# computational-cell-analytics/micro-sam

Measured on AMD Instinct MI355X. Metric: 1024^2 tiles/s embed+AMG (vit_b bf16), higher is better.
Workload: dtype bf16 image encoder (patch embedding + neck, 1.2 % of its flops, on hi+lo operand pairs of that type), fp16 mask decoder (16-bit MFMA operands, fp32 accumulation); 1 GPU; configs[1]: vit_b, 1024x1024 uint8 synthetic tiles, batched embedding precompute + AutomaticMaskGenerator (32x32 grid, multimask, default thresholds); encoder_batch=16, distinct_tiles_per_gpu=256, weights=seeded synthetic checkpoint (synthetic.py variant 'cells'), decode_lanes=3

## Files before the change

include/msam_hip.h:

```cpp
#ifndef MSAM_HIP_H
#define MSAM_HIP_H

#include <stdint.h>

#ifdef __cplusplus
extern "C" {
#endif

#define MSAM_MAX_BLOCKS 32
#define MSAM_F32 1
#define MSAM_BF16 2
#define MSAM_FP8 3
#define MSAM_F16 4
#define MSAM_U8 5
#define MSAM_U16 6
#define MSAM_ACT_NONE 0
#define MSAM_ACT_GELU 1
#define MSAM_ACT_RELU 2
#define MSAM_ACT_SIGMOID 3

const char* msam_last_error(void);
int msam_abi_version(void);


// ... 123 lines not shown
                  int32_t W, float thresh, int32_t intersection_over_min, uint64_t* mask_scratch, int32_t* keep_flags,
                  void* stream);

int64_t msam_amg_generate_workspace_bytes(int32_t N, int32_t H, int32_t W);
int msam_amg_generate_labels(const float* iou, const float* stability, const int32_t* boxes, const int32_t* area,
                             const uint32_t* bits, int32_t N, int32_t H, int32_t W, const int32_t* crop_box,
                             float pred_iou_thresh, float stability_score_thresh, float box_nms_thresh,
                             int32_t min_object_size, int32_t with_background, int32_t* labels, int32_t* flag,
                             void* workspace, int64_t workspace_bytes, void* stream);

int64_t msam_labels_from_masks_workspace_bytes(int32_t H, int32_t W);
int msam_labels_from_masks(const uint32_t* bits, const int32_t* order, int32_t K, const int32_t* k_dev, int32_t H, int32_t W,
                           int32_t min_object_size, int32_t with_background, int32_t* labels, int32_t* flag,
                           void* workspace, int64_t workspace_bytes, void* stream);

int msam_layernorm_backward(const float* x, const float* weight, const float* dy, float eps, int64_t rows, int32_t dim,
                            float* dx, float* dweight, float* dbias, void* stream);
int msam_attention_forward(const float* q, const float* k, const float* v, int32_t BH, int32_t Nq, int32_t Nk, int32_t D,
                           float scale, float* out, float* lse, void* stream);
int msam_attention_backward(const float* q, const float* k, const float* v, const float* out, const float* dout,
                            const float* lse, int32_t BH, int32_t Nq, int32_t Nk, int32_t D, float scale, float* dq, float* dk,
                            float* dv, float* delta, void* stream);

int msam_relpos_attention_forward(const float* q, const float* k, const float* v, const float* bias_h, const float* bias_w,
                                  int32_t BH, int32_t Gh, int32_t Gw, int32_t D, float scale, float* out, float* lse,
                                  void* stream);
int msam_relpos_attention_backward(const float* q, const float* k, const float* v, const float* bias_h, const float* bias_w,
                                   const float* out, const float* dout, const float* lse, int32_t BH, int32_t Gh, int32_t Gw,
                                   int32_t D, float scale, float* dq, float* dk, float* dv, float* dbias_h, float* dbias_w,
                                   float* delta, void* stream);

int msam_cast_transpose(const void* x, int32_t x_dtype, int64_t M, int32_t K, int64_t ldx, void* out16, void* outT, float* colsum,
                        void* stream);

int msam_layernorm(const float* x, const float* weight, const float* bias, float eps, int64_t rows, int32_t dim,
                   void* out, int32_t out_dtype, int32_t gelu, int32_t out_nchw_hw, void* stream);

int msam_layernorm_fp8(const float* x, const float* weight, const float* bias, float eps, int64_t rows, int32_t dim,
                       void* out_fp8, float* row_scale, void* stream);
int msam_quant_rows_fp8(const void* x_bf16, int64_t rows, int32_t dim, void* out_fp8, float* row_scale, void* stream);
int msam_patchify(const float* img, int32_t B, void* out_bf16, void* stream);
int msam_patchify16(const float* img, int32_t B, int32_t dtype16, void* out16, void* stream);
int msam_patchify_u8(const uint8_t* img, int32_t B, int32_t h, int32_t w, void* out_bf16, void* stream);
int msam_patchify_u8_16(const uint8_t* img, int32_t B, int32_t h, int32_t w, int32_t dtype16, void* out16, void* stream);
int msam_im2col3x3(const void* x_bf16, int32_t B, int32_t C, void* out_bf16, void* stream);
int msam_cast_f32_to_bf16(const float* x, void* out_bf16, int64_t n, void* stream);
int msam_cast_f32_to_16(const float* x, int32_t dtype16, void* out16, int64_t n, void* stream);
int msam_resample_u8(const uint8_t* in, int32_t B, int32_t H, int32_t W, int32_t C, int32_t axis, int32_t n_out,
                     const int32_t* bounds, const int32_t* coefs, int32_t ksize, uint8_t* out, void* stream);
int msam_patchify_split16(const float* img, int32_t B, int32_t dtype16, void* out16, void* stream);
int msam_patchify_u8_split16(const uint8_t* img, int32_t B, int32_t h, int32_t w, int32_t dtype16, void* out16, void* stream);
int msam_im2col3x3_split16(const float* x_f32, int32_t B, int32_t C, int32_t dtype16, void* out16, void* stream);
int msam_cast_f32_split16(const float* x, int32_t dtype16, void* out16, int64_t rows, int32_t dim, void* stream);

int msam_window_attention(const void* q, const void* k, const void* v, const void* rel_h, const void* rel_w,
                          const float* qkv_bias, int32_t B, int32_t heads, int32_t head_dim, float scale, void* out,
                          void* stream);
int msam_window_attention16(const void* q, const void* k, const void* v, const void* rel_h, const void* rel_w,
                            const float* qkv_bias, int32_t B, int32_t heads, int32_t head_dim, float scale, int32_t dtype16,
                            void* out, void* stream);
int msam_global_attention(const void* q, const void* k, const void* v, const void* rel_h, const void* rel_w,
                          int32_t B, int32_t heads, int32_t head_dim, float scale, void* out, void* stream);
int msam_global_attention16(const void* q, const void* k, const void* v, const void* rel_h, const void* rel_w, int32_t B,
                            int32_t heads, int32_t head_dim, float scale, int32_t dtype16, void* out, void* stream);

typedef struct {
    int32_t embed_dim, depth, heads;
    int32_t is_global[MSAM_MAX_BLOCKS];
    const void* patch_w; const float* patch_b;
    const float* pos_embed;
    const float* ln1_w[MSAM_MAX_BLOCKS]; const float* ln1_b[MSAM_MAX_BLOCKS];
    const void* qkv_w[MSAM_MAX_BLOCKS]; const float* qkv_b[MSAM_MAX_BLOCKS];
    const void* rel_h[MSAM_MAX_BLOCKS]; const void* rel_w[MSAM_MAX_BLOCKS];
    const void* proj_w[MSAM_MAX_BLOCKS]; const float* proj_b[MSAM_MAX_BLOCKS];
    const float* ln2_w[MSAM_MAX_BLOCKS]; const float* ln2_b[MSAM_MAX_BLOCKS];
    const void* lin1_w[MSAM_MAX_BLOCKS]; const float* lin1_b[MSAM_MAX_BLOCKS];
    const void* lin2_w[MSAM_MAX_BLOCKS]; const float* lin2_b[MSAM_MAX_BLOCKS];
    const void* neck0_w;
    const float* neck1_w; const float* neck1_b;
    const void* neck2_w;
    const float* neck3_w; const float* neck3_b;
    int32_t use_glds;
    int32_t head_dim_stored;
    int32_t fp8;
    const void* qkv_w8[MSAM_MAX_BLOCKS]; const float* qkv_cs[MSAM_MAX_BLOCKS];
    const void* proj_w8[MSAM_MAX_BLOCKS]; const float* proj_cs[MSAM_MAX_BLOCKS];
    const void* lin1_w8[MSAM_MAX_BLOCKS]; const float* lin1_cs[MSAM_MAX_BLOCKS];
    const void* lin2_w8[MSAM_MAX_BLOCKS]; const float* lin2_cs[MSAM_MAX_BLOCKS];
    int32_t dtype16;
    int32_t split_io;
    const void* adapter_wd[MSAM_MAX_BLOCKS]; const float* adapter_bd[MSAM_MAX_BLOCKS];
    const void* adapter_wu[MSAM_MAX_BLOCKS]; const float* adapter_bu[MSAM_MAX_BLOCKS];
    const float* adapter_alpha[MSAM_MAX_BLOCKS];
    int32_t adapter_dim;
} msam_encoder_t;

int64_t msam_encoder_workspace_bytes(const msam_encoder_t* enc, int32_t B);
int msam_encoder_forward(const msam_encoder_t* enc, const float* img_f32, const uint8_t* img_u8, int32_t h, int32_t w,
                         int32_t B, float* out, void* workspace, int64_t workspace_bytes,
                         float* tap, int32_t tap_block, void* stream);

int msam_adapter_bf16(const void* y16, int64_t ldy, const void* wd16, const float* bd, const void* wu16, const float* bu,
                      const float* alpha, float* x, int64_t ldx, int32_t R, int32_t D, int32_t P, int32_t dtype16, void* stream);

typedef struct {
    const void* q_w; const float* q_b; const void* k_w; const float* k_b;
    const void* v_w; const float* v_b; const void* o_w; const float* o_b;
} msam_attn_w_t;
typedef struct {
    msam_attn_w_t self_attn, t2i, i2t;
    const float *n1_w, *n1_b, *n2_w, *n2_b, *n3_w, *n3_b, *n4_w, *n4_b;
    const void* mlp1_w; const float* mlp1_b; const void* mlp2_w; const float* mlp2_b;
    const void* mlp1_ws; const void* mlp2_ws;
} msam_twoway_layer_t;
typedef struct {
    const float* pe_gauss;
    const float* point_embed;
    const float* not_a_point;
    const float* no_mask;
    const float* out_tokens;
    msam_twoway_layer_t layer[2];
    msam_attn_w_t final_attn; const float *nf_w, *nf_b;
    const void* up1_w; const float* up1_b;
    const float* up_ln_w; const float* up_ln_b;
    const void* up2_w; const float* up2_b;
    const void* hyp_w[4][3]; const float* hyp_b[4][3];
    const void* iou_w[3]; const float* iou_b[3];
    int32_t use_glds;
    int32_t low_res_dtype;
    int32_t up1_centred;
    float* low_res_range;
} msam_decoder_t;

int msam_decoder_dtype(void);
int64_t msam_decoder_const_bytes(void);
int msam_decoder_prepare_const(const msam_decoder_t* dec, void* consts, void* stream);
int64_t msam_decoder_image_bytes(void);
int msam_decoder_prepare_image(const msam_decoder_t* dec, const void* consts, const float* embedding ,
                               void* image_state, void* workspace, int64_t workspace_bytes, void* stream);
int64_t msam_decoder_workspace_bytes(int32_t P);
int msam_decoder_forward(const msam_decoder_t* dec, const void* consts, const void* image_state,
                         const float* points, const int32_t* labels, int32_t Np, const float* boxes, int32_t P,
                         int32_t multimask, float* low_res, float* iou,
                         void* workspace, int64_t workspace_bytes, void* stream);

typedef struct {
    const float *c1_w, *c1_b, *ln1_w, *ln1_b, *c2_w, *c2_b, *ln2_w, *ln2_b, *c3_w, *c3_b;
    int32_t exact_gelu;
} msam_mask_prompt_t;
int msam_decoder_forward_masks(const msam_decoder_t* dec, const msam_mask_prompt_t* mask_w, const void* consts,
                               const void* image_state, const float* points, const int32_t* labels, int32_t Np,
                               const float* boxes, const float* mask_input, int32_t P, int32_t multimask, float* low_res,
                               float* iou, void* workspace, int64_t workspace_bytes, void* stream);

int msam_prompt_encode(const msam_decoder_t* dec, const msam_mask_prompt_t* mask_w, const float* points,
                       const int32_t* labels, int32_t Np, const float* boxes, const float* mask_input, int32_t P,
                       float* sparse, float* dense, void* stream);
int msam_decoder_forward_embeddings(const msam_decoder_t* dec, const void* consts, const void* image_state,
                                    const float* sparse, int32_t Ns, const float* dense, const float* embedding,
                                    int32_t P, int32_t multimask, float* low_res, float* iou, void* workspace,
                                    int64_t workspace_bytes, void* stream);

int msam_postprocess_masks(const float* low_res, int32_t N, int32_t in_h, int32_t in_w, int32_t out_h, int32_t out_w,
                           float thr, float off, int32_t* counts, int32_t* boxes, uint32_t* bits, float* logits,
                           void* stream);
int msam_postprocess_masks16(const void* low_res, int32_t low_res_dtype, int32_t N, int32_t in_h, int32_t in_w, int32_t out_h,
                             int32_t out_w, float thr, float off, int32_t* counts, int32_t* boxes, uint32_t* bits, float* logits,
                             void* stream);
int msam_postprocess_masks_range(const float* low_res, const float* range, int32_t N, int32_t in_h, int32_t in_w, int32_t out_h,
                                 int32_t out_w, float thr, float off, int32_t* counts, int32_t* boxes, uint32_t* bits,
                                 void* stream);
int msam_uncrop_bits(const uint32_t* bits_crop, int32_t N, int32_t crop_h, int32_t crop_w, int32_t x0, int32_t y0,
                     int32_t out_h, int32_t out_w, uint32_t* bits_out, void* stream);

int msam_rle_run_counts(const uint32_t* bits, int32_t N, int32_t out_h, int32_t out_w, int32_t* n_runs, void* stream);
int msam_rle_encode(const uint32_t* bits, int32_t N, int32_t out_h, int32_t out_w, const int64_t* offsets,
                    int32_t* counts_out, void* stream);

int msam_box_nms(const float* boxes_sorted, int32_t K, float iou_threshold, uint64_t* mask_scratch, int32_t* keep_flags,
                 void* stream);

int msam_box_nms_valid(const float* boxes_sorted, const int32_t* valid_sorted, int32_t K, float iou_threshold,
                       uint64_t* mask_scratch, int32_t* keep_flags, void* stream);

int msam_paint_label_image(const uint32_t* bits, const int32_t* order, int32_t K, int32_t H, int32_t W, int32_t* label,
                           void* stream);
int msam_paint_label_image_dev(const uint32_t* bits, const int32_t* order, const int32_t* k_dev, int32_t H, int32_t W,
                               int32_t* label, void* stream);
int msam_label_components(const int32_t* seg, int32_t H, int32_t W, int32_t* roots, int32_t* changed_flag,
                          int32_t max_iters, int32_t* iters_done, void* stream);

int msam_component_sizes(const int32_t* roots, int32_t n, int32_t* sizes, int32_t* bg_count, void* stream);
int msam_label_components_async(const int32_t* seg, int32_t H, int32_t W, int32_t* roots, int32_t* changed_flag,
                                int32_t passes, void* stream);

#define MSAM_MATCH_MAX_THRESHOLDS 16
#define MSAM_MATCH_MAX_BATCH 65535
#define MSAM_MATCH_HEADER 4
#define MSAM_MATCH_ITEM 20
#define MSAM_MATCH_EDGE 6
int64_t msam_label_matching_workspace_bytes(int32_t B, int32_t capacity);
int msam_label_matching(const int32_t* pred, const int32_t* gt, int32_t B, int32_t G, int32_t H, int32_t W,
                        const double* thresholds, int32_t T, void* workspace, int64_t workspace_bytes, int32_t capacity,
                        int32_t* result, int32_t max_edges, void* stream);

int msam_slice_overlaps(const int32_t* labels, int32_t Z, int32_t H, int32_t W, uint64_t* table_keys, int32_t* table_counts,
                        int32_t capacity, int32_t* edges, int32_t max_edges, int32_t* n_edges, void* stream);

int msam_host_seeded_watershed(const float* image, const int32_t* markers, const uint8_t* mask, int32_t H, int32_t W, int32_t* out);

typedef struct {
    const float* A; int64_t lda;
    const float* A2; int64_t lda2; int64_t a2_rows;
    const float* W; int64_t ldw;
    int64_t M; int32_t N, K;
    const float* bias; int32_t act;
    const float* res; int64_t ldr; int64_t res_rows;
    float* out; int64_t ldc;
    const float* col_scale; const float* col_shift;
    int32_t conv_h, conv_w, conv_c;
    int32_t shuffle_h, shuffle_w, shuffle_c;
    int32_t a2_cols;
    int32_t split16;
    float a_scale, w_scale;
    const void* w_pairs;
} msam_sgemm_t;
int msam_strict_gemm(const msam_sgemm_t* p, void* stream);
int msam_strict_layernorm(const float* x, const float* weight, const float* bias, float eps, int64_t rows, int32_t dim, float* out,
                          int32_t gelu, int32_t out_nchw_hw, void* stream);
int msam_strict_relpos_attention(const float* qkv, const float* qkv_bias, const float* rel_h, const float* rel_w, int32_t B, int32_t heads,
                                 int32_t head_dim, int32_t grid, int32_t window, float scale, float* out, void* stream);
int msam_split16_relpos_attention(const float* qkv, const float* qkv_bias, const float* rel_h, const float* rel_w, int32_t B, int32_t heads,
                                  int32_t head_dim, int32_t grid, int32_t window, float scale, float* out, void* stream);
typedef struct msam_si2t {
    const float* keys; int64_t key_batch_stride;
    const float* pos;
    const float* wq; const float* bq;
    const float* tok_k; const float* tok_v; int64_t ld_tok, tok_batch_stride;
    const float* wo; const float* bo;
    const float* ln_weight; const float* ln_bias; float ln_eps; float denom;
    float* out;
    int32_t B, Tk;
    int32_t split16;
    float wq_scale, wo_scale;
    const void* wq_pairs; const void* wo_pairs;
} msam_si2t_t;
int msam_strict_i2t_block(const msam_si2t_t* p, void* stream);
int msam_strict_attention(const float* q, int64_t ldq, int64_t q_batch_stride, const float* k, int64_t ldk, int64_t k_batch_stride,
                          const float* v, int64_t ldv, int64_t v_batch_stride, int32_t B, int32_t H, int32_t Nq, int32_t Nk, int32_t D,
                          float denom, float* out, int64_t ldo, int64_t out_batch_stride, void* stream);
int msam_strict_patchify(const float* img, const uint8_t* img_u8, int32_t B, int32_t h, int32_t w, float* out, void* stream);
int msam_strict_im2col3x3(const float* x, int32_t B, int32_t C, float* out, void* stream);
int msam_strict_source(const float* embedding, const float* dense, int64_t dense_stride, int32_t P, float* src, void* stream);
int msam_strict_hyper_masks(const float* up, const float* hyper, int32_t hyper_ld, int32_t mask0, int32_t nmask, int64_t P, float* low_res,
                            void* stream);
int msam_split16_i2t_block(const msam_si2t_t* p, void* workspace, int64_t workspace_bytes, void* stream);
int msam_split16_prepare_pairs(const float* w, int64_t N, int32_t K, float scale, int32_t permute, void* out, void* stream);
typedef struct {
    const float* keys; int64_t key_batch_stride;
    const float* pos;
    const float* q; int64_t ldq;
    const float* wk; const float* wv; const float* bv;
    float denom;
    float* out; int64_t ldo;
    int32_t B, Tk;
    void* workspace; int64_t workspace_bytes;
} msam_st2i_t;
int msam_split16_t2i_attention(const msam_st2i_t* p, void* stream);
typedef struct {
    const float* u1;
    const float* ln_weight; const float* ln_bias; float ln_eps;
    const float* w2; const float* b2; float w_scale;
    const float* hyper; int32_t hyper_ld, mask0, nmask;
    float* low_res;
    int64_t P;
} msam_sup2_t;
int msam_strict_upscale2(const msam_sup2_t* p, void* stream);
int msam_strict_instance_norm(const float* x, int64_t ldx, int32_t B, int64_t HW, int32_t C, float eps, float* out, float* workspace,
                              int64_t workspace_floats, void* stream);
int msam_strict_resize_bilinear(const float* in, int32_t B, int32_t h, int32_t w, int32_t pitch_h, int32_t pitch_w, int64_t pixel_pitch, int32_t C,
                                int32_t H2, int32_t W2, float scale_h, float scale_w, int32_t out_nchw, float* out, void* stream);

#define MSAM_OBJFEAT_DESC 12
int msam_objfeat_gather(const int64_t* labels, const int64_t* desc, int32_t U, int32_t max_pixels, const int32_t* itab,
                        const int64_t* ids, int32_t n_ids, int64_t* keys, int32_t* area, void* stream);
int msam_objfeat_accumulate(const float* emb, const int64_t* desc, int32_t U, const int32_t* itab, const float* ftab,
                            const int64_t* sorted_keys, const int64_t* perm, const int32_t* chunk_start, const int64_t* pix_start,
                            const int32_t* area, int32_t n_ids, int32_t K, int32_t max_chunks, double* partial, void* stream);
int msam_objfeat_finish(const double* partial, const int32_t* chunk_start, const int32_t* area, int32_t n_ids, double* sums,
                        int64_t* area_total, int32_t out_f64, void* out, void* stream);
int msam_objfeat_project(const int64_t* labels, int64_t n, const int64_t* ids, int32_t n_ids, int32_t* index, void* stream);

#define MSAM_EDT_MAX_SIDE 32767
int64_t msam_edt_squared_workspace_bytes(int32_t H, int32_t W);
int msam_edt_squared(const void* mask, int32_t mask_is_int32, int32_t H, int32_t W, int32_t* out, void* workspace,
                     int64_t workspace_bytes, void* stream);
int64_t msam_label_props_workspace_bytes(int32_t H, int32_t W, int32_t N);
int msam_label_props(const int32_t* labels, int32_t H, int32_t W, const int32_t* ids, int32_t N, int32_t* area, int32_t* bbox,
                     int64_t* coord_sum, int32_t* center, void* workspace, int64_t workspace_bytes, void* stream);
int64_t msam_distance_targets_workspace_bytes(int32_t H, int32_t W, int32_t N);
int msam_distance_targets(const int32_t* labels, int32_t H, int32_t W, int32_t N, int32_t correct_centers, float fill, float* out,
                          int32_t* center, int32_t* dmax2, int32_t* bbox, void* workspace, int64_t workspace_bytes, void* stream);

#define MSAM_MASK_MAX_SIDE 32767
#define MSAM_MASK_MAX_OBJECTS 65535
int msam_mask_pack(const uint8_t* masks, int32_t P, int32_t H, int32_t W, uint32_t* bits, void* stream);
// ... 63 lines not shown
```

micro_sam_amd/_lib.py:

```python
from __future__ import annotations

import ctypes as C
import os
from typing import Optional

import torch

from . import build as _build

MSAM_MAX_BLOCKS = 32
F32, BF16, FP8, F16, U8, U16 = 1, 2, 3, 4, 5, 6
ACT_NONE, ACT_GELU, ACT_RELU, ACT_SIGMOID = 0, 1, 2, 3

_vp, _i32, _i64, _f32 = C.c_void_p, C.c_int32, C.c_int64, C.c_float
PROFILE_FAMILIES = 8


class GemmParams(C.Structure):
    _fields_ = [
        ("A", _vp), ("lda", _i64), ("W", _vp), ("ldw", _i64), ("M", _i32), ("N", _i32), ("K", _i32),
        ("bias", _vp), ("table", _vp), ("table_rows", _i32), ("table_cols", _i32), ("table_ld", _i64),
        ("resid", _vp), ("resid_dtype", _i32), ("resid_rows", _i32), ("ldr", _i64), ("act", _i32),
        ("out", _vp), ("out_dtype", _i32), ("ldc", _i64), ("out_mode", _i32),
        ("q", _vp), ("k", _vp), ("v", _vp), ("heads", _i32), ("head_dim", _i32), ("tokens", _i32),
        ("use_glds", _i32), ("ln_mode", _i32), ("ln_w", _vp), ("ln_b", _vp), ("ln_eps", _f32),
        ("a_dtype", _i32), ("row_scale", _vp), ("col_scale", _vp), ("split_k", _i32),
        ("ln_add", _vp), ("ln_out_a", _vp), ("ln_out_b", _vp),
    ]


class WsGemmParams(C.Structure):
    _fields_ = [
        ("A", _vp), ("W", _vp), ("M", _i32), ("N", _i32), ("K", _i32), ("bias", _vp),
        ("table", _vp), ("table_rows", _i32), ("table_cols", _i32), ("table_ld", _i64),
        ("resid", _vp), ("resid_rows", _i32), ("ldr", _i64),
        ("ln_mode", _i32), ("ln_w", _vp), ("ln_b", _vp), ("ln_eps", _f32),
        ("out", _vp), ("ldc", _i64), ("kv_split", _i32), ("k_out", _vp), ("vT_out", _vp), ("tokens", _i32),
        ("head_major", _i32),
    ]


class ImageLayerParams(C.Structure):
    _fields_ = [
        ("xin", _vp), ("q_shared", _vp), ("wq", _vp), ("bq", _vp), ("peq", _vp),
        ("wo", _vp), ("bo", _vp), ("ln_w", _vp), ("ln_b", _vp), ("ln_eps", _f32),
        ("ktok", _vp), ("vtok", _vp), ("Nt", _i32), ("out", _vp), ("rows", _i32),
    ]


_blk = _vp * MSAM_MAX_BLOCKS


class EncoderParams(C.Structure):
    _fields_ = [
        ("embed_dim", _i32), ("depth", _i32), ("heads", _i32), ("is_global", _i32 * MSAM_MAX_BLOCKS),
        ("patch_w", _vp), ("patch_b", _vp), ("pos_embed", _vp),
        ("ln1_w", _blk), ("ln1_b", _blk), ("qkv_w", _blk), ("qkv_b", _blk), ("rel_h", _blk), ("rel_w", _blk),
        ("proj_w", _blk), ("proj_b", _blk), ("ln2_w", _blk), ("ln2_b", _blk),
        ("lin1_w", _blk), ("lin1_b", _blk), ("lin2_w", _blk), ("lin2_b", _blk),
        ("neck0_w", _vp), ("neck1_w", _vp), ("neck1_b", _vp), ("neck2_w", _vp), ("neck3_w", _vp), ("neck3_b", _vp),
        ("use_glds", _i32), ("head_dim_stored", _i32), ("fp8", _i32),
        ("qkv_w8", _blk), ("qkv_cs", _blk), ("proj_w8", _blk), ("proj_cs", _blk),
        ("lin1_w8", _blk), ("lin1_cs", _blk), ("lin2_w8", _blk), ("lin2_cs", _blk),
        ("dtype16", _i32), ("split_io", _i32),
        ("adapter_wd", _blk), ("adapter_bd", _blk), ("adapter_wu", _blk), ("adapter_bu", _blk), ("adapter_alpha", _blk),
        ("adapter_dim", _i32),
    ]


class AttnW(C.Structure):
    _fields_ = [("q_w", _vp), ("q_b", _vp), ("k_w", _vp), ("k_b", _vp), ("v_w", _vp), ("v_b", _vp),
                ("o_w", _vp), ("o_b", _vp)]


class TwoWayLayer(C.Structure):
    _fields_ = [("self_attn", AttnW), ("t2i", AttnW), ("i2t", AttnW),
                ("n1_w", _vp), ("n1_b", _vp), ("n2_w", _vp), ("n2_b", _vp), ("n3_w", _vp), ("n3_b", _vp),
                ("n4_w", _vp), ("n4_b", _vp),
                ("mlp1_w", _vp), ("mlp1_b", _vp), ("mlp2_w", _vp), ("mlp2_b", _vp), ("mlp1_ws", _vp), ("mlp2_ws", _vp)]


class DecoderParams(C.Structure):
    _fields_ = [
        ("pe_gauss", _vp), ("point_embed", _vp), ("not_a_point", _vp), ("no_mask", _vp), ("out_tokens", _vp),
        ("layer", TwoWayLayer * 2), ("final_attn", AttnW), ("nf_w", _vp), ("nf_b", _vp),
        ("up1_w", _vp), ("up1_b", _vp), ("up_ln_w", _vp), ("up_ln_b", _vp), ("up2_w", _vp), ("up2_b", _vp),
        ("hyp_w", (_vp * 3) * 4), ("hyp_b", (_vp * 3) * 4), ("iou_w", _vp * 3), ("iou_b", _vp * 3),
        ("use_glds", _i32), ("low_res_dtype", _i32), ("up1_centred", _i32), ("low_res_range", _vp),
    ]


class SGemmParams(C.Structure):
    _fields_ = [("A", _vp), ("lda", _i64), ("A2", _vp), ("lda2", _i64), ("a2_rows", _i64), ("W", _vp), ("ldw", _i64),
                ("M", _i64), ("N", _i32), ("K", _i32), ("bias", _vp), ("act", _i32), ("res", _vp), ("ldr", _i64), ("res_rows", _i64),
                ("out", _vp), ("ldc", _i64), ("col_scale", _vp), ("col_shift", _vp), ("conv_h", _i32), ("conv_w", _i32), ("conv_c", _i32),
                ("shuffle_h", _i32), ("shuffle_w", _i32), ("shuffle_c", _i32), ("a2_cols", _i32), ("split16", _i32), ("a_scale", _f32), ("w_scale", _f32), ("w_pairs", _vp)]


class SI2TParams(C.Structure):
    _fields_ = [("keys", _vp), ("key_batch_stride", _i64), ("pos", _vp), ("wq", _vp), ("bq", _vp), ("tok_k", _vp), ("tok_v", _vp),
                ("ld_tok", _i64), ("tok_batch_stride", _i64), ("wo", _vp), ("bo", _vp), ("ln_weight", _vp), ("ln_bias", _vp),
                ("ln_eps", _f32), ("denom", _f32), ("out", _vp), ("B", _i32), ("Tk", _i32), ("split16", _i32), ("wq_scale", _f32), ("wo_scale", _f32), ("wq_pairs", _vp), ("wo_pairs", _vp)]


class ST2IParams(C.Structure):
    _fields_ = [("keys", _vp), ("key_batch_stride", _i64), ("pos", _vp), ("q", _vp), ("ldq", _i64), ("wk", _vp), ("wv", _vp), ("bv", _vp),
                ("denom", _f32), ("out", _vp), ("ldo", _i64), ("B", _i32), ("Tk", _i32), ("workspace", _vp), ("workspace_bytes", _i64)]


class SUp2Params(C.Structure):
    _fields_ = [("u1", _vp), ("ln_weight", _vp), ("ln_bias", _vp), ("ln_eps", _f32), ("w2", _vp), ("b2", _vp), ("w_scale", _f32),
                ("hyper", _vp), ("hyper_ld", _i32), ("mask0", _i32), ("nmask", _i32), ("low_res", _vp), ("P", _i64)]


class MaskPromptParams(C.Structure):
    _fields_ = [(n, _vp) for n in ("c1_w", "c1_b", "ln1_w", "ln1_b", "c2_w", "c2_b", "ln2_w", "ln2_b", "c3_w", "c3_b")] + [("exact_gelu", _i32)]


_PROTOS = {
    "msam_last_error": (C.c_char_p, []),
    "msam_abi_version": (_i32, []),
    "msam_gemm_bf16": (_i32, [C.POINTER(GemmParams), _vp]),
    "msam_wsgemm_bf16": (_i32, [C.POINTER(WsGemmParams), _vp]),
    "msam_decoder_image_layer": (_i32, [C.POINTER(ImageLayerParams), _vp]),
    "msam_t2i_fold_workspace_bytes": (_i64, [_i32]),
    "msam_t2i_fold_attention": (_i32, [_vp, _i32, _vp, _i32, _i32, _vp, _vp, _vp, _vp, _vp, _vp, _i64, _vp]),
    "msam_upscale_fused": (_i32, [_vp, _i32, _vp, _vp, _vp, _vp, _f32, _vp, _vp, _vp, _i32, _i32, _i32, _vp, _vp]),
    "msam_uncrop_bits": (_i32, [_vp, _i32, _i32, _i32, _i32, _i32, _i32, _i32, _vp, _vp]),
    "msam_decoder_forward_masks": (_i32, [C.POINTER(DecoderParams), C.POINTER(MaskPromptParams), _vp, _vp, _vp, _vp, _i32, _vp, _vp,
                                          _i32, _i32, _vp, _vp, _vp, _i64, _vp]),
    "msam_i2t_fold_workspace_bytes": (_i64, [_i32]),
    "msam_i2t_fold_layer": (_i32, [_vp, _i32, _vp, _vp, _i32, _i32, _vp, _vp, _vp, _vp, _vp, _vp, _f32, _vp, _vp, _i64, _vp]),
    "msam_profile_enable": (_i32, [_i32]),
    "msam_profile_collect": (_i32, [C.POINTER(_i32), C.POINTER(C.c_double), C.POINTER(C.c_double)]),
    "msam_profile_collect_family": (_i32, [_i32 * PROFILE_FAMILIES, C.c_double * PROFILE_FAMILIES, C.c_double * PROFILE_FAMILIES,
                                          C.c_double * PROFILE_FAMILIES]),
    "msam_layernorm": (_i32, [_vp, _vp, _vp, _f32, _i64, _i32, _vp, _i32, _i32, _i32, _vp]),
    "msam_layernorm_backward": (_i32, [_vp, _vp, _vp, _f32, _i64, _i32, _vp, _vp, _vp, _vp]),
    "msam_attention_forward": (_i32, [_vp, _vp, _vp, _i32, _i32, _i32, _i32, _f32, _vp, _vp, _vp]),
    "msam_attention_backward": (_i32, [_vp, _vp, _vp, _vp, _vp, _vp, _i32, _i32, _i32, _i32, _f32, _vp, _vp, _vp, _vp, _vp]),
    "msam_relpos_attention_forward": (_i32, [_vp, _vp, _vp, _vp, _vp, _i32, _i32, _i32, _i32, _f32, _vp, _vp, _vp]),
    "msam_relpos_attention_backward": (_i32, [_vp, _vp, _vp, _vp, _vp, _vp, _vp, _vp, _i32, _i32, _i32, _i32, _f32, _vp, _vp, _vp,
                                              _vp, _vp, _vp, _vp]),
    "msam_amg_generate_workspace_bytes": (_i64, [_i32, _i32, _i32]),
    "msam_amg_generate_labels": (_i32, [_vp, _vp, _vp, _vp, _vp, _i32, _i32, _i32, C.POINTER(_i32), _f32, _f32, _f32, _i32, _i32,
                                        _vp, _vp, _vp, _i64, _vp]),
    "msam_to_image": (_i32, [_vp, _i32, _i32, _i32, _i32, _vp, _vp, _vp]),
    "msam_patchify": (_i32, [_vp, _i32, _vp, _vp]),
    "msam_patchify_u8": (_i32, [_vp, _i32, _i32, _i32, _vp, _vp]),
    "msam_im2col3x3": (_i32, [_vp, _i32, _i32, _vp, _vp]),
    "msam_cast_f32_to_bf16": (_i32, [_vp, _vp, _i64, _vp]),
    "msam_cast_transpose": (_i32, [_vp, _i32, _i64, _i32, _i64, _vp, _vp, _vp, _vp]),
    "msam_gemm256_set_staging": (_i32, [_i32]),
    "msam_gemm_set_trace": (_i32, [_vp]),
    "msam_gemm_group_bf16": (_i32, [_vp, _i32, _vp]),
    "msam_fold_attn_set_dma": (_i32, [_i32]),
    "msam_tune_set": (_i32, [C.c_char_p, _i32]),
    "msam_tune_get": (_i32, [C.c_char_p, C.POINTER(_i32)]),
    "msam_i2t_fold_operand_bytes": (_i64, [_i32]),
    "msam_i2t_fold_operands": (_i32, [_vp, _vp, _i32, _i32, _vp, _vp, _vp, _i32, _vp, _vp]),
    "msam_i2t0_t2i_workspace_bytes": (_i64, [_i32]),
    "msam_i2t0_t2i_fused": (_i32, [_vp, _vp, _vp, _vp, _f32, _vp, _i32, _i32, _vp, _vp, _vp, _vp, _vp, _i64, _vp]),
    "msam_i2t01_fused": (_i32, [_vp, _vp, _vp, _vp, _vp, _vp, _vp, _f32, _i32, _i32, _vp, _vp]),
    "msam_chain_tables2_bytes": (_i64, []),
    "msam_chain_prepare_tables2": (_i32, [_vp, _vp, _vp, _vp, _vp, _vp, _vp, _vp, _vp, _vp]),
    "msam_chain_const2_bytes": (_i64, []),
    "msam_chain_prepare_const2": (_i32, [_vp, _vp, _vp, _vp, _vp, _vp, _vp, _vp, _vp]),
    "msam_chain_prepare_tables2_c": (_i32, [_vp, _vp, _vp, _vp]),
    "msam_t2i_fold_values_bytes": (_i64, [_i32]),
    "msam_t2i_fold_values": (_i32, [_vp, _i32, _i32, _vp, _vp, _vp]),
    "msam_i2t_fold_operands_values": (_i32, [_vp, _vp, _i32, _i32, _vp, _vp, _vp, _i32, _vp, _vp, _vp, _vp]),
    "msam_i2t0_t2i_v2_workspace_bytes": (_i64, [_i32]),
    "msam_i2t0_t2i_fused_v2": (_i32, [_vp, _vp, _vp, _vp, _vp, _f32, _vp, _i32, _i32, _vp, _vp, _vp, _i64, _vp]),
    "msam_chain_handover_bytes": (_i64, [_i32]),
    "msam_i2t0_t2i_fused_v2_handover": (_i32, [_vp, _vp, _vp, _vp, _vp, _f32, _vp, _i32, _i32, _vp, _vp, _vp, _i64, _vp, _vp]),
    "msam_i2t01_fused_handover": (_i32, [_vp, _vp, _vp, _vp, _vp, _vp, _vp, _f32, _i32, _i32, _vp, _vp, _vp]),
    "msam_chain_tables_bytes": (_i64, []),
    "msam_chain_prepare_tables": (_i32, [_vp, _vp, _vp, _vp, _vp, _vp]),
    "msam_upscale_fused_layout": (_i32, [_vp, _i32, _i32, _vp, _vp, _vp, _vp, _f32, _vp, _vp, _vp, _i32, _i32, _i32, _vp, _vp]),
    "msam_upscale_fused_out": (_i32, [_vp, _i32, _i32, _vp, _vp, _vp, _vp, _f32, _vp, _vp, _vp, _i32, _i32, _i32, _vp, _i32, _vp]),
    "msam_upscale_fused_range": (_i32, [_vp, _i32, _i32, _vp, _vp, _vp, _vp, _f32, _vp, _vp, _vp, _i32, _i32, _i32, _vp, _i32, _vp, _vp]),
    "msam_upscale_set_prio": (_i32, [_i32]),
    "msam_layernorm_fp8": (_i32, [_vp, _vp, _vp, _f32, _i64, _i32, _vp, _vp, _vp]),
    "msam_quant_rows_fp8": (_i32, [_vp, _i64, _i32, _vp, _vp, _vp]),
    "msam_debug_i2t_timing": (_i32, [_i32, _vp]),
    "msam_window_attention": (_i32, [_vp, _vp, _vp, _vp, _vp, _vp, _i32, _i32, _i32, C.c_float, _vp, _vp]),
    "msam_global_attention": (_i32, [_vp, _vp, _vp, _vp, _vp, _i32, _i32, _i32, C.c_float, _vp, _vp]),
    "msam_window_attention16": (_i32, [_vp, _vp, _vp, _vp, _vp, _vp, _i32, _i32, _i32, C.c_float, _i32, _vp, _vp]),
    "msam_global_attention16": (_i32, [_vp, _vp, _vp, _vp, _vp, _i32, _i32, _i32, C.c_float, _i32, _vp, _vp]),
    "msam_patchify16": (_i32, [_vp, _i32, _i32, _vp, _vp]),
    "msam_patchify_u8_16": (_i32, [_vp, _i32, _i32, _i32, _i32, _vp, _vp]),
    "msam_cast_f32_to_16": (_i32, [_vp, _i32, _vp, _i64, _vp]),
    "msam_resample_u8": (_i32, [_vp, _i32, _i32, _i32, _i32, _i32, _i32, _vp, _vp, _i32, _vp, _vp]),
    "msam_patchify_split16": (_i32, [_vp, _i32, _i32, _vp, _vp]),
    "msam_patchify_u8_split16": (_i32, [_vp, _i32, _i32, _i32, _i32, _vp, _vp]),
    "msam_im2col3x3_split16": (_i32, [_vp, _i32, _i32, _i32, _vp, _vp]),
    "msam_cast_f32_split16": (_i32, [_vp, _i32, _vp, _i64, _i32, _vp]),
    "msam_encoder_workspace_bytes": (_i64, [C.POINTER(EncoderParams), _i32]),
    "msam_encoder_forward": (_i32, [C.POINTER(EncoderParams), _vp, _vp, _i32, _i32, _i32, _vp, _vp, _i64, _vp, _i32, _vp]),
    "msam_decoder_dtype": (_i32, []),
    "msam_decoder_const_bytes": (_i64, []),
    "msam_decoder_prepare_const": (_i32, [C.POINTER(DecoderParams), _vp, _vp]),
    "msam_decoder_image_bytes": (_i64, []),
    "msam_decoder_prepare_image": (_i32, [C.POINTER(DecoderParams), _vp, _vp, _vp, _vp, _i64, _vp]),
    "msam_decoder_workspace_bytes": (_i64, [_i32]),
    "msam_prompt_encode": (_i32, [C.POINTER(DecoderParams), C.POINTER(MaskPromptParams), _vp, _vp, _i32, _vp, _vp, _i32, _vp, _vp, _vp]),
    "msam_decoder_forward_embeddings": (_i32, [C.POINTER(DecoderParams), _vp, _vp, _vp, _i32, _vp, _vp, _i32, _i32, _vp, _vp, _vp,
                                               _i64, _vp]),
    "msam_decoder_forward": (_i32, [C.POINTER(DecoderParams), _vp, _vp, _vp, _vp, _i32, _vp, _i32, _i32, _vp, _vp, _vp,
                                    _i64, _vp]),
    "msam_postprocess_masks": (_i32, [_vp, _i32, _i32, _i32, _i32, _i32, _f32, _f32, _vp, _vp, _vp, _vp, _vp]),
    "msam_postprocess_masks16": (_i32, [_vp, _i32, _i32, _i32, _i32, _i32, _i32, _f32, _f32, _vp, _vp, _vp, _vp, _vp]),
    "msam_postprocess_masks_range": (_i32, [_vp, _vp, _i32, _i32, _i32, _i32, _i32, _f32, _f32, _vp, _vp, _vp, _vp]),
    "msam_rle_run_counts": (_i32, [_vp, _i32, _i32, _i32, _vp, _vp]),
    "msam_rle_encode": (_i32, [_vp, _i32, _i32, _i32, _vp, _vp, _vp]),
    "msam_mask_nms": (_i32, [_vp, _vp, _vp, _vp, _i32, _i32, _i32, _f32, _i32, _vp, _vp, _vp]),
    "msam_box_nms": (_i32, [_vp, _i32, _f32, _vp, _vp, _vp]),
    "msam_box_nms_valid": (_i32, [_vp, _vp, _i32, _f32, _vp, _vp, _vp]),
    "msam_paint_label_image_dev": (_i32, [_vp, _vp, _vp, _i32, _i32, _vp, _vp]),
    "msam_label_components_async": (_i32, [_vp, _i32, _i32, _vp, _vp, _i32, _vp]),
    "msam_component_sizes": (_i32, [_vp, _i32, _vp, _vp, _vp]),
    "msam_labels_from_masks_workspace_bytes": (_i64, [_i32, _i32]),
    "msam_labels_from_masks": (_i32, [_vp, _vp, _i32, _vp, _i32, _i32, _i32, _i32, _vp, _vp, _vp, _i64, _vp]),
    "msam_host_seeded_watershed": (_i32, [_vp, _vp, _vp, _i32, _i32, _vp]),
    "msam_slice_overlaps": (_i32, [_vp, _i32, _i32, _i32, _vp, _vp, _i32, _vp, _i32, _vp, _vp]),
    "msam_paint_label_image": (_i32, [_vp, _vp, _i32, _i32, _i32, _vp, _vp]),
    "msam_label_components": (_i32, [_vp, _i32, _i32, _vp, _vp, _i32, C.POINTER(_i32), _vp]),
    "msam_strict_gemm": (_i32, [C.POINTER(SGemmParams), _vp]),
    "msam_strict_i2t_block": (_i32, [C.POINTER(SI2TParams), _vp]),
    "msam_strict_layernorm": (_i32, [_vp, _vp, _vp, _f32, _i64, _i32, _vp, _i32, _i32, _vp]),
    "msam_strict_relpos_attention": (_i32, [_vp, _vp, _vp, _vp, _i32, _i32, _i32, _i32, _i32, _f32, _vp, _vp]),
    "msam_split16_relpos_attention": (_i32, [_vp, _vp, _vp, _vp, _i32, _i32, _i32, _i32, _i32, _f32, _vp, _vp]),
    "msam_strict_attention": (_i32, [_vp, _i64, _i64, _vp, _i64, _i64, _vp, _i64, _i64, _i32, _i32, _i32, _i32, _i32, _f32, _vp, _i64,
                                     _i64, _vp]),
    "msam_strict_patchify": (_i32, [_vp, _vp, _i32, _i32, _i32, _vp, _vp]),
    "msam_strict_im2col3x3": (_i32, [_vp, _i32, _i32, _vp, _vp]),
    "msam_strict_source": (_i32, [_vp, _vp, _i64, _i32, _vp, _vp]),
    "msam_strict_hyper_masks": (_i32, [_vp, _vp, _i32, _i32, _i32, _i64, _vp, _vp]),
    "msam_strict_upscale2": (_i32, [C.POINTER(SUp2Params), _vp]),
    "msam_split16_t2i_attention": (_i32, [C.POINTER(ST2IParams), _vp]),
    "msam_split16_prepare_pairs": (_i32, [_vp, _i64, _i32, _f32, _i32, _vp, _vp]),
    "msam_split16_i2t_block": (_i32, [C.POINTER(SI2TParams), _vp, _i64, _vp]),
    "msam_strict_instance_norm": (_i32, [_vp, _i64, _i32, _i64, _i32, _f32, _vp, _vp, _i64, _vp]),
    "msam_strict_resize_bilinear": (_i32, [_vp, _i32, _i32, _i32, _i32, _i32, _i64, _i32, _i32, _i32, _f32, _f32, _i32, _vp, _vp]),
    "msam_objfeat_gather": (_i32, [_vp, _vp, _i32, _i32, _vp, _vp, _i32, _vp, _vp, _vp]),
    "msam_objfeat_accumulate": (_i32, [_vp, _vp, _i32, _vp, _vp, _vp, _vp, _vp, _vp, _vp, _i32, _i32, _i32, _vp, _vp]),
    "msam_objfeat_finish": (_i32, [_vp, _vp, _vp, _i32, _vp, _vp, _i32, _vp, _vp]),
    "msam_objfeat_project": (_i32, [_vp, _i64, _vp, _i32, _vp, _vp]),
    "msam_label_matching_workspace_bytes": (_i64, [_i32, _i32]),
    "msam_label_matching": (_i32, [_vp, _vp, _i32, _i32, _i32, _i32, C.POINTER(C.c_double), _i32, _vp, _i64, _i32, _vp, _i32, _vp]),
    "msam_edt_squared_workspace_bytes": (_i64, [_i32, _i32]),
    "msam_edt_squared": (_i32, [_vp, _i32, _i32, _i32, _vp, _vp, _i64, _vp]),
    "msam_label_props_workspace_bytes": (_i64, [_i32, _i32, _i32]),
    "msam_label_props": (_i32, [_vp, _i32, _i32, _vp, _i32, _vp, _vp, _vp, _vp, _vp, _i64, _vp]),
    "msam_distance_targets_workspace_bytes": (_i64, [_i32, _i32, _i32]),
    "msam_distance_targets": (_i32, [_vp, _i32, _i32, _i32, _i32, _f32, _vp, _vp, _vp, _vp, _vp, _i64, _vp]),
    "msam_mask_pack": (_i32, [_vp, _i32, _i32, _i32, _vp, _vp]),
    "msam_mask_iou_counts": (_i32, [_vp, _vp, _i32, _i32, _i32, C.c_double, _vp, _vp, _vp]),
    "msam_mask_box_prompts": (_i32, [_vp, _i32, _i32, _i32, C.c_double, _i32, _i32, _vp, _vp, _vp]),
    "msam_mask_logits": (_i32, [_vp, _i32, _i32, _i32, _vp, _vp]),
    "msam_paint_max": (_i32, [_vp, _vp, _vp, _i32, _i32, _i32, _vp, _vp]),
    "msam_pca_moments_workspace_bytes": (_i64, [_i32, _i32, _i32]),
    "msam_pca_moments": (_i32, [_vp, _i32, _i32, _i32, _vp, _vp, _vp, _i64, _vp]),
    "msam_pca_project": (_i32, [_vp, _vp, _vp, _i32, _i32, _i32, _i32, _vp, _vp, _vp]),
    "msam_pca_to_rgb": (_i32, [_vp, _vp, _i32, _i32, _vp, _vp]),
    "msam_semantic_loss_workspace_bytes": (_i64, [_i32, _i32, _i32]),
    "msam_semantic_loss_forward": (_i32, [_vp, _vp, _i32, _i32, _i32, _f32, _f32, _i32, C.c_double, _vp, _i64, _vp, _vp, _vp]),
    "msam_semantic_loss_backward": (_i32, [_vp, _vp, _i32, _i32, _i32, _f32, _f32, _i32, C.c_double, _vp, _vp, _vp, _vp]),
    "msam_depth_conv3_bf16": (_i32, [_vp, _i64, _vp, _vp, _vp, _i64, _i32, _i32, _i32, _i32, _i32, _vp]),
    "msam_conv3d_k3_bf16": (_i32, [_vp, _i64, _vp, _vp, _vp, _i64, _i32, _i32, _i32, _i32, _i32, _i32, _vp]),
    "msam_conv3d_k3_wgrad_workspace_bytes": (_i64, [_i32, _i32, _i32, _i32, _i32, _i32]),
    "msam_conv3d_k3_wgrad_bf16": (_i32, [_vp, _i64, _vp, _i64, _vp, _vp, _i64, _i32, _i32, _i32, _i32, _i32, _i32, _vp]),
    "msam_instance_norm_workspace_bytes": (_i64, [_i32, _i64, _i32]),
    "msam_instance_norm_stats": (_i32, [_vp, _i64, _i32, _i64, _i32, _vp, _vp, _i64, _vp]),
    "msam_instance_norm_apply": (_i32, [_vp, _i64, _vp, _vp, _i64, _vp, _i32, _i64, _i32, _f32, _f32, _i32, _vp, _i64, _vp, _i64, _vp]),
    "msam_instance_norm_backward": (_i32, [_vp, _i64, _vp, _i64, _vp, _vp, _i64, _vp, _i32, _i64, _i32, _f32, _f32, _i32, _vp, _i64, _vp, _i64,
                                           _vp, _vp, _i64, _vp]),
    "msam_column_sums_f32": (_i32, [_vp, _i64, _i64, _i32, _vp, _vp, _i64, _vp]),
    "msam_adapter_bf16": (_i32, [_vp, _i64, _vp, _vp, _vp, _vp, _vp, _vp, _i64, _i32, _i32, _i32, _i32, _vp]),
    "msam_tiled_mask_overlaps": (_i32, [_vp, _vp, _vp, _i32, _vp, _i32, _vp, _vp]),
    "msam_paint_tiled": (_i32, [_vp, _vp, _vp, _vp, _i32, _i32, _i32, _vp, _vp]),
    "msam_mask_moments": (_i32, [_vp, _i32, _i32, _i32, _vp, _vp]),
    "msam_mask_shift": (_i32, [_vp, _i32, _i32, _i32, _vp, _vp, _vp]),
# ... 76 lines not shown
```

micro_sam_amd/csrc/decfold.hip:

```cpp
#include "common.h"
#include "../../include/msam_hip.h"
#include <string>

void msam_set_error(const char* msg);
int msam_check_launch(const char* what);
void msam_profile_mark2(void* stream, int begin, double flops, double bytes, int family);

namespace {

constexpr int T = 4096, C = 256, CI = 128, TK = 32, NTHR = 256;
constexpr int SUBT = 1024 + 32;
constexpr int KEYS_BYTES = 16 * SUBT, TAB_BYTES = TK * CI * 2, BUF_BYTES = KEYS_BYTES + TAB_BYTES;
constexpr float NEG_BIG = -1.0e30f;
#ifndef FOLD_ATTN_DMA_DEFAULT
#define FOLD_ATTN_DMA_DEFAULT 0
#endif

typedef short s16x4_t __attribute__((ext_vector_type(4)));

MSAM_DEVINL uint2 lds_tr16(const unsigned char* p) {
    s16x4_t v = __builtin_amdgcn_ds_read_tr16_b64_v4i16((s16x4_t __attribute__((address_space(3)))*)p);
    return __builtin_bit_cast(uint2, v);
}

// ... 527 lines not shown
__global__ __launch_bounds__(256) void fold_v_kernel(const u16* __restrict__ vtok, const u16* __restrict__ wo, int Nt,
                                                     u16* __restrict__ vfoldT) {
    __shared__ float v[8][CI];
    const int p = blockIdx.x, c = threadIdx.x;
    for (int i = c; i < 8 * CI; i += 256) {
        const int t = i >> 7, d = i & (CI - 1);
        v[t][d] = t < Nt ? d2f(vtok[((long)p * Nt + t) * CI + d]) : 0.f;
    }
    __syncthreads();
    u16* dst = vfoldT + ((long)p * C + c) * 64;
    for (int h = 0; h < 8; ++h) {
        const uint4 w0 = *(const uint4*)(wo + (long)c * CI + h * 16), w1 = *(const uint4*)(wo + (long)c * CI + h * 16 + 8);
        const uint32_t ww[8] = {w0.x, w0.y, w0.z, w0.w, w1.x, w1.y, w1.z, w1.w};
        float wf[16];
#pragma unroll
        for (int x = 0; x < 8; ++x) { wf[2 * x] = d2f((u16)(ww[x] & 0xffff)); wf[2 * x + 1] = d2f((u16)(ww[x] >> 16)); }
        uint32_t pk[4];
#pragma unroll
        for (int t2 = 0; t2 < 4; ++t2) {
            float a0 = 0.f, a1 = 0.f;
#pragma unroll
            for (int d = 0; d < 16; ++d) { a0 = fmaf(wf[d], v[2 * t2][h * 16 + d], a0); a1 = fmaf(wf[d], v[2 * t2 + 1][h * 16 + d], a1); }
            pk[t2] = pack2d(a0, a1);
        }
        *(uint4*)(dst + h * 8) = make_uint4(pk[0], pk[1], pk[2], pk[3]);
    }
}

int key_splits(int P) {
    int ks = 1;
    while (P * ks < 512 && ks < 16) ks *= 2;
    return ks;
}

}

extern "C" int64_t msam_t2i_fold_workspace_bytes(int32_t P) {
    const long ks = key_splits(P);
    return (long)P * 64 * C * 2 + (long)P * ks * 64 * C * 4 + (long)P * ks * 64 * 2 * 4;
}

extern "C" int msam_t2i_fold_attention(const void* keys, int32_t kv_shared, const void* qtok, int32_t P, int32_t Nt,
                                       const void* wk, const void* tabk, const void* wv, const float* bv, void* out,
                                       void* workspace, int64_t workspace_bytes, void* stream) {
    if (!keys || !qtok || !wk || !tabk || !wv || !bv || !out || !workspace || P <= 0) {
        msam_set_error("msam_t2i_fold_attention: null argument");
        return 1;
    }
    if (Nt < 1 || Nt > 8) { msam_set_error("msam_t2i_fold_attention: 1 <= Nt <= 8 tokens per prompt"); return 1; }
    if (workspace_bytes < msam_t2i_fold_workspace_bytes(P)) { msam_set_error("msam_t2i_fold_attention: workspace too small"); return 1; }
    hipStream_t s = (hipStream_t)stream;
    const int KS = key_splits(P);
    char* wp = (char*)workspace;
    u16* qprime = (u16*)wp; wp += (long)P * 64 * C * 2;
    float* opart = (float*)wp; wp += (long)P * KS * 64 * C * 4;
    float* stats = (float*)wp;
    hipLaunchKernelGGL(fold_q_kernel, dim3(P * 8), dim3(256), 0, s, (const u16*)qtok, (const u16*)wk, Nt, qprime);
    if (int e = msam_check_launch("fold_q")) return e;
    FoldArgs a{};
    a.keys = (const u16*)keys; a.kv_shared = kv_shared & 1; a.blocked = (kv_shared >> 1) & 1; a.qprime = qprime; a.qtok = (const u16*)qtok; a.Nt = Nt;
    a.tabk = (const u16*)tabk; a.nitems = P * KS; a.KS = KS; a.opart = opart; a.stats = stats;
    a.wv = (const u16*)wv; a.bv = bv; a.out = (u16*)out;
    int dev = 0, cus = 256;
    (void)hipGetDevice(&dev);
    (void)hipDeviceGetAttribute(&cus, hipDeviceAttributeMultiprocessorCount, dev);
    const int grid = a.nitems < 2 * cus ? a.nitems : 2 * cus;
    const double flops = (double)P * T * (2.0 * 64 * C * 2 + 2.0 * 64 * 32);
    const double bytes = (double)((kv_shared & 1) ? 1 : P) * T * C * 2 + (KS > 1 ? (double)P * KS * 64 * C * 4 : 0.0);
    msam_profile_mark2(stream, 1, flops, bytes, 3);
    if (g_fold_attn_dma && !a.blocked) {
        const int grid3 = a.nitems < 3 * cus ? a.nitems : 3 * cus;
        hipLaunchKernelGGL(fold_attn_kernel<true>, dim3(grid3), dim3(NTHR), 0, s, a);
    } else {
        hipLaunchKernelGGL(fold_attn_kernel<false>, dim3(grid), dim3(NTHR), 0, s, a);
    }
    msam_profile_mark2(stream, 0, flops, bytes, 3);
    if (int e = msam_check_launch("fold_attn")) return e;
    if (KS == 1) return 0;
    hipLaunchKernelGGL(fold_finish_kernel, dim3(P * 8), dim3(128), 0, s, opart, stats, KS, Nt, (const u16*)wv, bv, (u16*)out);
    return msam_check_launch("fold_finish");
}

int64_t msam_i2t_tok_workspace_bytes(int32_t P);
int msam_i2t_tok_layer(const void* xin, int32_t x_shared, const void* ktok, const void* vtok, int32_t P, int32_t Nt,
                       const void* wq, const void* tabq, const void* wo, const float* bo, const float* ln_w,
                       const float* ln_b, float ln_eps, void* out, void* workspace, int KS, void* stream);
extern int g_tune_i2t_variant;

extern "C" int64_t msam_i2t_fold_workspace_bytes(int32_t P) {
    const int64_t a = (int64_t)P * 64 * C * 2 * 2, b = msam_i2t_tok_workspace_bytes(P);
    return a > b ? a : b;
}

extern "C" int msam_i2t_fold_layer(const void* xin, int32_t x_shared, const void* ktok, const void* vtok, int32_t P,
                                   int32_t Nt, const void* wq, const void* tabq, const void* wo, const float* bo,
                                   const float* ln_w, const float* ln_b, float ln_eps, void* out, void* workspace,
                                   int64_t workspace_bytes, void* stream) {
    if (!xin || !ktok || !vtok || !wq || !tabq || !wo || !bo || !ln_w || !ln_b || !out || !workspace || P <= 0) {
        msam_set_error("msam_i2t_fold_layer: null argument");
        return 1;
    }
    if (Nt < 1 || Nt > 8) { msam_set_error("msam_i2t_fold_layer: 1 <= Nt <= 8 tokens per prompt"); return 1; }
    if (workspace_bytes < msam_i2t_fold_workspace_bytes(P)) { msam_set_error("msam_i2t_fold_layer: workspace too small"); return 1; }
    if (g_tune_i2t_variant == 1)
        return msam_i2t_tok_layer(xin, x_shared, ktok, vtok, P, Nt, wq, tabq, wo, bo, ln_w, ln_b, ln_eps, out, workspace,
                                  key_splits(P), stream);
    hipStream_t s = (hipStream_t)stream;
    u16* kfold = (u16*)workspace;
    u16* vfoldT = kfold + (long)P * 64 * C;
    hipLaunchKernelGGL(fold_q_kernel, dim3(P * 8), dim3(256), 0, s, (const u16*)ktok, (const u16*)wq, Nt, kfold);
    if (int e = msam_check_launch("fold_k")) return e;
    hipLaunchKernelGGL(fold_v_kernel, dim3(P), dim3(256), 0, s, (const u16*)vtok, (const u16*)wo, Nt, vfoldT);
    if (int e = msam_check_launch("fold_v")) return e;
    I2tArgs a{};
    a.xin = (const u16*)xin; a.x_shared = x_shared; a.kfold = kfold; a.vfoldT = vfoldT; a.ktok = (const u16*)ktok; a.Nt = Nt;
    a.tabq = (const u16*)tabq; a.bo = bo; a.ln_w = ln_w; a.ln_b = ln_b; a.eps = ln_eps;
    a.KS = key_splits(P); a.nitems = P * a.KS; a.out = (u16*)out;
    int dev = 0, cus = 256;
    (void)hipGetDevice(&dev);
    (void)hipDeviceGetAttribute(&cus, hipDeviceAttributeMultiprocessorCount, dev);
    const int grid = a.nitems < 2 * cus ? a.nitems : 2 * cus;
    const double flops = (double)P * T * (2.0 * 64 * C * 2 + 2.0 * 64 * 32);
    const double bytes = (double)(x_shared ? 1 : P) * T * C * 2 + (double)P * T * C * 2;
    msam_profile_mark2(stream, 1, flops, bytes, 2);
    if (g_i2t_timing) hipLaunchKernelGGL(fold_i2t_kernel<true>, dim3(grid), dim3(NTHR), 0, s, a);
    else hipLaunchKernelGGL(fold_i2t_kernel<false>, dim3(grid), dim3(NTHR), 0, s, a);
    msam_profile_mark2(stream, 0, flops, bytes, 2);
    return msam_check_launch("fold_i2t");
}

extern "C" int msam_debug_i2t_timing(int32_t enable, uint64_t* host_out) {
    g_i2t_timing = enable;
    if (host_out) {
        if (hipDeviceSynchronize() != hipSuccess ||
            hipMemcpyFromSymbol(host_out, HIP_SYMBOL(g_i2t_stamps), sizeof(unsigned long long) * 64 * 12) != hipSuccess) {
            msam_set_error("msam_debug_i2t_timing: copy failed");
            return 2;
        }
    }
    return 0;
}

extern "C" int msam_fold_attn_set_dma(int32_t on) { g_fold_attn_dma = on; return 0; }

extern int g_tune_i2t_wg_per_cu, g_tune_chain_variant, g_tune_chain_tmask, g_tune_up_gelu16, g_tune_up_ln_two_pass, g_tune_up_centred;
void msam_gemm_set_dbg(int v);
void msam_gemm_set_gw(int delay, int cls);
void msam_gemm_set_g3(int delay);
void msam_gemm_set_g3_epi(int v);
extern int g_tune_tok_fuse;
extern int g_tune_chain_handover, g_tune_chain_handover_ring;
extern int g_tune_mlp_split_fused;
extern int g_tune_amg_range_map;
extern int g_tune_sgemm_bufs, g_tune_srel_mfma, g_tune_sgemm_small_below, g_tune_si2t_dbg, g_tune_si2t_late_us, g_tune_sattn_allh;
int g_tune_dec_chain = 1, g_tune_dec_chain_min_p = 128;
extern "C" int msam_tune_set(const char* key, int32_t value) {
    const std::string k = key ? key : "";
    if (k == "i2t_variant") g_tune_i2t_variant = value;
    else if (k == "i2t_wg_per_cu") g_tune_i2t_wg_per_cu = value;
    else if (k == "dec_chain") g_tune_dec_chain = value;
    else if (k == "chain_variant") g_tune_chain_variant = value;
    else if (k == "chain_tmask") g_tune_chain_tmask = value;
    else if (k == "chain_handover") g_tune_chain_handover = value;
    else if (k == "chain_handover_ring") g_tune_chain_handover_ring = value;
    else if (k == "up_gelu16") g_tune_up_gelu16 = value;
    else if (k == "up_ln_two_pass") g_tune_up_ln_two_pass = value;
    else if (k == "up_centred") g_tune_up_centred = value;
    else if (k == "amg_range_map") g_tune_amg_range_map = value;
    else if (k == "gemm_dbg") msam_gemm_set_dbg(value);
    else if (k == "gw_delay") msam_gemm_set_gw(value, -1);
    else if (k == "gw_class") msam_gemm_set_gw(-2, value);
    else if (k == "g3_delay") msam_gemm_set_g3(value);
    else if (k == "g3_epi") msam_gemm_set_g3_epi(value);
    else if (k == "tok_fuse") g_tune_tok_fuse = value;
    else if (k == "mlp_split_fused") g_tune_mlp_split_fused = value;
    else if (k == "dec_chain_min_p") g_tune_dec_chain_min_p = value;
    else if (k == "sgemm_bufs") g_tune_sgemm_bufs = value;
    else if (k == "srel_mfma") g_tune_srel_mfma = value;
    else if (k == "sattn_allh") g_tune_sattn_allh = value;
    else if (k == "sgemm_small_below") g_tune_sgemm_small_below = value;
    else if (k == "si2t_dbg") g_tune_si2t_dbg = value;
    else if (k == "si2t_late_us") g_tune_si2t_late_us = value;
    else { msam_set_error("msam_tune_set: unknown key"); return 1; }
    return 0;
}
extern "C" int msam_tune_get(const char* key, int32_t* value) {
    const std::string k = key ? key : "";
    if (!value || k != "amg_range_map") { msam_set_error("msam_tune_get: unknown key"); return 1; }
    *value = g_tune_amg_range_map;
    return 0;
}
```

micro_sam_amd/csrc/decoder.hip:

```cpp
#include <stdlib.h>
#include "common.h"
#include "../../include/msam_hip.h"

void msam_set_error(const char* msg);
int msam_check_launch(const char* what);

namespace {

constexpr int T = 4096;
constexpr int C = 256;
constexpr int CI = 128;
constexpr float NEG_BIG = -1.0e30f;
constexpr float TWO_PI = 6.283185307179586f;


MSAM_DEVINL void pe_encode(const float* __restrict__ G, float cx, float cy, int j, float& s, float& c) {
    const float x = 2.f * cx - 1.f, y = 2.f * cy - 1.f;
    const float v = TWO_PI * (x * G[j] + y * G[128 + j]);
    s = sinf(v); c = cosf(v);
}

__global__ __launch_bounds__(256) void dense_pe_kernel(const float* __restrict__ G, float* __restrict__ pos_f32,
                                                       u16* __restrict__ pos_bf16) {
    const int idx = blockIdx.x * 256 + threadIdx.x;
// ... 183 lines not shown
            float s, co;
            pe_encode(G, bx / 1024.f, by / 1024.f, j, s, co);
            tp[row * C + c] = (c < 128 ? s : co) + point_embed[(2 + k) * C + c];
        }
    }
}

__global__ __launch_bounds__(256) void add_cast_kernel(const float* __restrict__ a, const float* __restrict__ b,
                                                       u16* __restrict__ out, long n4) {
    for (long i = (long)blockIdx.x * 256 + threadIdx.x; i < n4; i += (long)gridDim.x * 256) {
        float4 x = *(const float4*)(a + i * 4);
        if (b) { float4 y = *(const float4*)(b + i * 4); x.x += y.x; x.y += y.y; x.z += y.z; x.w += y.w; }
        uint2 pk; pk.x = pack2d(x.x, x.y); pk.y = pack2d(x.z, x.w);
        *(uint2*)(out + i * 4) = pk;
    }
}

__global__ __launch_bounds__(256) void add_cast2_kernel(const float* __restrict__ a, const float* __restrict__ b,
                                                        u16* __restrict__ out_a, u16* __restrict__ out_b, long n4) {
    for (long i = (long)blockIdx.x * 256 + threadIdx.x; i < n4; i += (long)gridDim.x * 256) {
        const float4 x = *(const float4*)(a + i * 4), y = *(const float4*)(b + i * 4);
        uint2 pa, pb;
        pa.x = pack2d(x.x + y.x, x.y + y.y); pa.y = pack2d(x.z + y.z, x.w + y.w);
        pb.x = pack2d(x.x, x.y); pb.y = pack2d(x.z, x.w);
        *(uint2*)(out_a + i * 4) = pa;
        *(uint2*)(out_b + i * 4) = pb;
    }
}

__global__ __launch_bounds__(128) void token_self_attn_kernel(const u16* __restrict__ q, const u16* __restrict__ k,
                                                              const u16* __restrict__ v, int Nt, u16* __restrict__ out) {
    const int p = blockIdx.x, head = threadIdx.x >> 4, i = threadIdx.x & 15;
    if (i >= Nt) return;
    const long base = (long)p * Nt * C + head * 32;
    float qv[32];
#pragma unroll
    for (int c4 = 0; c4 < 4; ++c4) {
        uint4 w = *(const uint4*)(q + base + (long)i * C + c4 * 8);
        const uint32_t ww[4] = {w.x, w.y, w.z, w.w};
#pragma unroll
        for (int x = 0; x < 4; ++x) { qv[c4 * 8 + 2 * x] = d2f((u16)(ww[x] & 0xffff)); qv[c4 * 8 + 2 * x + 1] = d2f((u16)(ww[x] >> 16)); }
    }
    float s[16];
    float m = NEG_BIG;
#pragma unroll
    for (int j = 0; j < 16; ++j) {
        float acc = 0.f;
        if (j < Nt) {
#pragma unroll
            for (int c4 = 0; c4 < 4; ++c4) {
                uint4 w = *(const uint4*)(k + base + (long)j * C + c4 * 8);
                const uint32_t ww[4] = {w.x, w.y, w.z, w.w};
#pragma unroll
                for (int x = 0; x < 4; ++x) {
                    acc += qv[c4 * 8 + 2 * x] * d2f((u16)(ww[x] & 0xffff));
                    acc += qv[c4 * 8 + 2 * x + 1] * d2f((u16)(ww[x] >> 16));
                }
            }
            acc *= 0.17677669529663687f;
        } else acc = NEG_BIG;
        s[j] = acc; m = fmaxf(m, acc);
    }
    float l = 0.f;
#pragma unroll
    for (int j = 0; j < 16; ++j) { s[j] = __expf(s[j] - m); l += s[j]; }
    float o[32];
#pragma unroll
    for (int d = 0; d < 32; ++d) o[d] = 0.f;
#pragma unroll
    for (int j = 0; j < 16; ++j) {
        if (j < Nt) {
#pragma unroll
            for (int c4 = 0; c4 < 4; ++c4) {
                uint4 w = *(const uint4*)(v + base + (long)j * C + c4 * 8);
                const uint32_t ww[4] = {w.x, w.y, w.z, w.w};
#pragma unroll
                for (int x = 0; x < 4; ++x) {
                    o[c4 * 8 + 2 * x] += s[j] * d2f((u16)(ww[x] & 0xffff));
                    o[c4 * 8 + 2 * x + 1] += s[j] * d2f((u16)(ww[x] >> 16));
                }
            }
        }
    }
    const float inv = 1.f / l;
#pragma unroll
    for (int c4 = 0; c4 < 4; ++c4) {
        uint4 pk;
        pk.x = pack2d(o[c4 * 8 + 0] * inv, o[c4 * 8 + 1] * inv); pk.y = pack2d(o[c4 * 8 + 2] * inv, o[c4 * 8 + 3] * inv);
        pk.z = pack2d(o[c4 * 8 + 4] * inv, o[c4 * 8 + 5] * inv); pk.w = pack2d(o[c4 * 8 + 6] * inv, o[c4 * 8 + 7] * inv);
        *(uint4*)(out + base + (long)i * C + c4 * 8) = pk;
    }
}

__global__ __launch_bounds__(256) void t2i_attn_kernel(const u16* __restrict__ qtok, const u16* __restrict__ kimg,
                                                       const u16* __restrict__ vT, int kv_shared, int Nt,
                                                       u16* __restrict__ out) {
    __shared__ float red[4][16][20];
    const int p = blockIdx.x >> 3, head = blockIdx.x & 7;
    const int tid = threadIdx.x, lane = tid & 63, wave = tid >> 6, fr = lane & 15, fg = lane >> 4;
    const int pk = kv_shared ? 0 : p;
    const u16* kb = kimg + ((long)pk * 8 + head) * T * 16;
    const u16* vb = vT + ((long)pk * CI + head * 16 + fr) * T;
    uint4 qf = make_uint4(0, 0, 0, 0);
    if (fg < 2 && fr < Nt) qf = *(const uint4*)(qtok + ((long)p * Nt + fr) * CI + head * 16 + fg * 8);
    f32x4_t o = {0.f, 0.f, 0.f, 0.f};
    float m = NEG_BIG, l = 0.f;
    const int t_begin = wave * (T / 4), t_end = t_begin + T / 4;
    for (int t0 = t_begin; t0 < t_end; t0 += 32) {
        uint4 ka0 = make_uint4(0, 0, 0, 0), ka1 = ka0;
        if (fg < 2) {
            ka0 = *(const uint4*)(kb + (long)(t0 + fr) * 16 + fg * 8);
            ka1 = *(const uint4*)(kb + (long)(t0 + 16 + fr) * 16 + fg * 8);
        }
        const uint2 v0 = *(const uint2*)(vb + t0 + fg * 4), v1 = *(const uint2*)(vb + t0 + 16 + fg * 4);
        f32x4_t s0 = {0.f, 0.f, 0.f, 0.f}, s1 = s0;
        s0 = mfma16d(ka0, qf, s0);
        s1 = mfma16d(ka1, qf, s1);
        float mt = NEG_BIG;
#pragma unroll
        for (int r = 0; r < 4; ++r) { s0[r] *= 0.25f; s1[r] *= 0.25f; mt = fmaxf(mt, fmaxf(s0[r], s1[r])); }
        mt = fmaxf(mt, __shfl_xor(mt, 16)); mt = fmaxf(mt, __shfl_xor(mt, 32));
        const float mn = fmaxf(m, mt), alpha = __expf(m - mn);
        m = mn;
        float ps = 0.f;
#pragma unroll
        for (int r = 0; r < 4; ++r) { s0[r] = __expf(s0[r] - mn); s1[r] = __expf(s1[r] - mn); ps += s0[r] + s1[r]; }
        l = l * alpha + ps;
        uint4 pb;
        pb.x = pack2d(s0[0], s0[1]); pb.y = pack2d(s0[2], s0[3]); pb.z = pack2d(s1[0], s1[1]); pb.w = pack2d(s1[2], s1[3]);
        o[0] *= alpha; o[1] *= alpha; o[2] *= alpha; o[3] *= alpha;
        o = mfma16d(make_uint4(v0.x, v0.y, v1.x, v1.y), pb, o);
    }
    l += __shfl_xor(l, 16); l += __shfl_xor(l, 32);
    if (fg == 0) { red[wave][fr][0] = m; red[wave][fr][1] = l; }
#pragma unroll
    for (int r = 0; r < 4; ++r) red[wave][fr][2 + fg * 4 + r] = o[r];
    __syncthreads();
    if (wave == 0 && fr < Nt) {
        float mm = fmaxf(fmaxf(red[0][fr][0], red[1][fr][0]), fmaxf(red[2][fr][0], red[3][fr][0]));
        float ll = 0.f, oo[4] = {0.f, 0.f, 0.f, 0.f};
#pragma unroll
        for (int w = 0; w < 4; ++w) {
            const float a = __expf(red[w][fr][0] - mm);
            ll += a * red[w][fr][1];
#pragma unroll
            for (int r = 0; r < 4; ++r) oo[r] += a * red[w][fr][2 + fg * 4 + r];
        }
        const float inv = 1.f / ll;
        uint2 pkd; pkd.x = pack2d(oo[0] * inv, oo[1] * inv); pkd.y = pack2d(oo[2] * inv, oo[3] * inv);
        *(uint2*)(out + ((long)p * Nt + fr) * CI + head * 16 + fg * 4) = pkd;
    }
}

__global__ __launch_bounds__(256) void t2i_shared4_kernel(const u16* __restrict__ qtok, const u16* __restrict__ kimg,
                                                          const u16* __restrict__ vT, int P, int Nt, u16* __restrict__ out) {
    __shared__ float red[4][32][20];
    const int pg = blockIdx.x >> 3, head = blockIdx.x & 7;
    const int tid = threadIdx.x, lane = tid & 63, wave = tid >> 6, fr = lane & 15, fg = lane >> 4;
    const u16* kb = kimg + (long)head * T * 16;
    const u16* vb = vT + ((long)head * 16 + fr) * T;
    const int tk = fr & 7;
    uint4 qf[2];
#pragma unroll
    for (int n = 0; n < 2; ++n) {
        const int p = pg * 4 + n * 2 + (fr >> 3);
        qf[n] = make_uint4(0, 0, 0, 0);
        if (fg < 2 && tk < Nt && p < P) qf[n] = *(const uint4*)(qtok + ((long)p * Nt + tk) * CI + head * 16 + fg * 8);
    }
    f32x4_t o[2] = {{0.f, 0.f, 0.f, 0.f}, {0.f, 0.f, 0.f, 0.f}};
    float m[2] = {NEG_BIG, NEG_BIG}, l[2] = {0.f, 0.f};
    const int t_begin = wave * (T / 4), t_end = t_begin + T / 4;
    for (int t0 = t_begin; t0 < t_end; t0 += 32) {
        uint4 ka0 = make_uint4(0, 0, 0, 0), ka1 = ka0;
        if (fg < 2) {
            ka0 = *(const uint4*)(kb + (long)(t0 + fr) * 16 + fg * 8);
            ka1 = *(const uint4*)(kb + (long)(t0 + 16 + fr) * 16 + fg * 8);
        }
        const uint2 v0 = *(const uint2*)(vb + t0 + fg * 4), v1 = *(const uint2*)(vb + t0 + 16 + fg * 4);
        const uint4 va = make_uint4(v0.x, v0.y, v1.x, v1.y);
#pragma unroll
        for (int n = 0; n < 2; ++n) {
            f32x4_t s0 = {0.f, 0.f, 0.f, 0.f}, s1 = s0;
            s0 = mfma16d(ka0, qf[n], s0);
            s1 = mfma16d(ka1, qf[n], s1);
            float mt = NEG_BIG;
#pragma unroll
            for (int r = 0; r < 4; ++r) { s0[r] *= 0.25f; s1[r] *= 0.25f; mt = fmaxf(mt, fmaxf(s0[r], s1[r])); }
            mt = fmaxf(mt, __shfl_xor(mt, 16)); mt = fmaxf(mt, __shfl_xor(mt, 32));
            const float mn = fmaxf(m[n], mt), alpha = __expf(m[n] - mn);
            m[n] = mn;
            float ps = 0.f;
#pragma unroll
            for (int r = 0; r < 4; ++r) { s0[r] = __expf(s0[r] - mn); s1[r] = __expf(s1[r] - mn); ps += s0[r] + s1[r]; }
            l[n] = l[n] * alpha + ps;
            uint4 pb;
            pb.x = pack2d(s0[0], s0[1]); pb.y = pack2d(s0[2], s0[3]); pb.z = pack2d(s1[0], s1[1]); pb.w = pack2d(s1[2], s1[3]);
            o[n][0] *= alpha; o[n][1] *= alpha; o[n][2] *= alpha; o[n][3] *= alpha;
            o[n] = mfma16d(va, pb, o[n]);
        }
    }
#pragma unroll
    for (int n = 0; n < 2; ++n) {
        float ln = l[n];
        ln += __shfl_xor(ln, 16); ln += __shfl_xor(ln, 32);
        if (fg == 0) { red[wave][n * 16 + fr][0] = m[n]; red[wave][n * 16 + fr][1] = ln; }
#pragma unroll
        for (int r = 0; r < 4; ++r) red[wave][n * 16 + fr][2 + fg * 4 + r] = o[n][r];
    }
    __syncthreads();
    if (wave < 2) {
        const int n = wave, c = n * 16 + fr, p = pg * 4 + n * 2 + (fr >> 3);
        if (tk < Nt && p < P) {
            const float mm = fmaxf(fmaxf(red[0][c][0], red[1][c][0]), fmaxf(red[2][c][0], red[3][c][0]));
            float ll = 0.f, oo[4] = {0.f, 0.f, 0.f, 0.f};
#pragma unroll
            for (int w = 0; w < 4; ++w) {
                const float a = __expf(red[w][c][0] - mm);
                ll += a * red[w][c][1];
#pragma unroll
                for (int r = 0; r < 4; ++r) oo[r] += a * red[w][c][2 + fg * 4 + r];
            }
            const float inv = 1.f / ll;
            uint2 pkd; pkd.x = pack2d(oo[0] * inv, oo[1] * inv); pkd.y = pack2d(oo[2] * inv, oo[3] * inv);
            *(uint2*)(out + ((long)p * Nt + tk) * CI + head * 16 + fg * 4) = pkd;
        }
    }
}

inline int grid_for(long items) { long g = (items + 255) / 256; return (int)(g < 1 ? 1 : (g > 8192 ? 8192 : g)); }


struct Ctx { hipStream_t s; int use_glds; };

msam_gemm_t mk_gemm(const void* A, long lda, const void* W, int M, int N, int K, const float* bias, void* out, int out_dtype,
                    long ldc, int act = 0) {
    msam_gemm_t g{};
    g.A = A; g.lda = lda; g.W = W; g.ldw = K; g.M = M; g.N = N; g.K = K; g.bias = bias;
    g.act = act; g.out = out; g.out_dtype = out_dtype; g.ldc = ldc; g.a_dtype = MSAM_D16;
    return g;
}

int gemm(const Ctx& cx, const void* A, long lda, const void* W, int M, int N, int K, const float* bias, void* out,
         int out_dtype, long ldc, int act = 0, const void* resid = nullptr, int resid_dtype = 0, long ldr = 0,
         int resid_rows = 0, const float* table = nullptr, int table_cols = 0, int ln_mode = 0,
         const float* ln_w = nullptr, const float* ln_b = nullptr, float ln_eps = 1e-5f) {
    msam_gemm_t g{};
    g.ln_mode = ln_mode; g.ln_w = ln_w; g.ln_b = ln_b; g.ln_eps = ln_eps;
    g.A = A; g.lda = lda; g.W = W; g.ldw = K; g.M = M; g.N = N; g.K = K; g.bias = bias;
    g.table = table; g.table_rows = T; g.table_cols = table_cols; g.table_ld = CI;
    g.resid = resid; g.resid_dtype = resid_dtype; g.resid_rows = resid_rows; g.ldr = ldr;
    g.act = act; g.out = out; g.out_dtype = out_dtype; g.ldc = ldc; g.out_mode = 0; g.a_dtype = MSAM_D16;
    g.use_glds = MSAM_DEC_F16 ? 0 : cx.use_glds;
    return msam_gemm_bf16(&g, cx.s);
}

int gemm_ln_tok(const Ctx& cx, const void* A, long lda, const void* W, int M, int K, const float* bias, const float* resid,
                const float* ln_w, const float* ln_b, float* queries, const float* add, void* out_a, void* out_b) {
    msam_gemm_t g{};
    g.A = A; g.lda = lda; g.W = W; g.ldw = K; g.M = M; g.N = C; g.K = K; g.bias = bias;
    g.resid = resid; g.resid_dtype = resid ? MSAM_F32 : 0; g.ldr = C;
    g.out = queries; g.out_dtype = MSAM_F32; g.ldc = C; g.a_dtype = MSAM_D16;
    g.ln_mode = 1; g.ln_w = ln_w; g.ln_b = ln_b; g.ln_eps = 1e-5f;
    g.ln_add = add; g.ln_out_a = out_a; g.ln_out_b = out_b;
    return msam_gemm_bf16(&g, cx.s);
}

int wsgemm_kv(const Ctx& cx, const void* x, const u16* wkv, const float* bkv, const float* pek, int rows, void* k_out,
              void* vT_out) {
    {
        msam_wsgemm_t k{};
        k.A = x; k.W = wkv; k.M = rows; k.N = CI; k.K = C; k.bias = bkv;
        k.table = pek; k.table_rows = T; k.table_cols = CI; k.table_ld = CI;
        k.out = k_out; k.ldc = CI; k.head_major = 1; k.tokens = T;
        if (int e = msam_wsgemm_bf16(&k, cx.s)) return e;
    }
    msam_wsgemm_t g{};
    g.A = x; g.W = wkv + (long)CI * C; g.M = rows; g.N = CI; g.K = C; g.bias = bkv + CI;
    g.kv_split = 1; g.vT_out = vT_out; g.tokens = T;
    return msam_wsgemm_bf16(&g, cx.s);
}

struct Consts {
    float* pos_f32; u16* pos_bf16; float* pe_k[3]; float* pe_q[2]; u16* wkv[3]; float* bkv[3];
    u16* tab_k[3];
    u16* tab_q[2];
    void* chain2;
};
constexpr long CONST2_BYTES = 128L * 128 * 4 + 4 * 512 + (long)CI * C * 2;
constexpr long CONST_BYTES = (long)T * C * 4 + (long)T * C * 2 + 5L * T * CI * 4 + 3L * C * C * 2 + 3L * C * 4 + 5L * T * CI * 2 + CONST2_BYTES;

Consts carve_consts(void* base) {
    Consts c; char* p = (char*)base;
    c.pos_f32 = (float*)p; p += (long)T * C * 4;
    c.pos_bf16 = (u16*)p; p += (long)T * C * 2;
    for (int i = 0; i < 3; ++i) { c.pe_k[i] = (float*)p; p += (long)T * CI * 4; }
    for (int i = 0; i < 2; ++i) { c.pe_q[i] = (float*)p; p += (long)T * CI * 4; }
    for (int i = 0; i < 3; ++i) { c.wkv[i] = (u16*)p; p += (long)C * C * 2; }
    for (int i = 0; i < 3; ++i) { c.bkv[i] = (float*)p; p += (long)C * 4; }
    for (int i = 0; i < 3; ++i) { c.tab_k[i] = (u16*)p; p += (long)T * CI * 2; }
    for (int i = 0; i < 2; ++i) { c.tab_q[i] = (u16*)p; p += (long)T * CI * 2; }
    c.chain2 = p;
    return c;
}

struct ImageState { float* src_f32; u16* src_bf16; u16* k0; u16* vT0; u16* q0; };
constexpr long IMAGE_BYTES = (long)T * C * 4 + (long)T * C * 2 + 3L * T * CI * 2;

ImageState carve_image(void* base) {
    ImageState s; char* p = (char*)base;
    s.src_f32 = (float*)p; p += (long)T * C * 4;
    s.src_bf16 = (u16*)p; p += (long)T * C * 2;
    s.k0 = (u16*)p; p += (long)T * CI * 2;
    s.vT0 = (u16*)p; p += (long)T * CI * 2;
    s.q0 = (u16*)p; p += (long)T * CI * 2;
    return s;
}

inline long align256(long x) { return (x + 255) & ~255L; }

}

extern "C" int64_t msam_decoder_const_bytes(void) { return CONST_BYTES; }
extern "C" int msam_decoder_dtype(void) { return MSAM_D16; }
extern "C" int64_t msam_decoder_image_bytes(void) { return IMAGE_BYTES; }

extern "C" int msam_decoder_prepare_const(const msam_decoder_t* dec, void* consts, void* stream) {
    if (!dec || !consts) { msam_set_error("msam_decoder_prepare_const: null argument"); return 1; }
    Ctx cx{(hipStream_t)stream, dec->use_glds};
    Consts c = carve_consts(consts);
    hipLaunchKernelGGL(dense_pe_kernel, dim3(T * 128 / 256), dim3(256), 0, cx.s, dec->pe_gauss, c.pos_f32, c.pos_bf16);
    if (int e = msam_check_launch("dense_pe")) return e;
    const msam_attn_w_t* t2i[3] = {&dec->layer[0].t2i, &dec->layer[1].t2i, &dec->final_attn};
    for (int i = 0; i < 3; ++i) {
        hipMemcpyAsync(c.wkv[i], t2i[i]->k_w, (size_t)CI * C * 2, hipMemcpyDeviceToDevice, cx.s);
        hipMemcpyAsync(c.wkv[i] + (long)CI * C, t2i[i]->v_w, (size_t)CI * C * 2, hipMemcpyDeviceToDevice, cx.s);
        hipMemcpyAsync(c.bkv[i], t2i[i]->k_b, CI * 4, hipMemcpyDeviceToDevice, cx.s);
        hipMemcpyAsync(c.bkv[i] + CI, t2i[i]->v_b, CI * 4, hipMemcpyDeviceToDevice, cx.s);
        if (int e = gemm(cx, c.pos_bf16, C, t2i[i]->k_w, T, CI, C, nullptr, c.pe_k[i], MSAM_F32, CI)) return e;
        if (int e = gemm(cx, c.pos_bf16, C, t2i[i]->k_w, T, CI, C, t2i[i]->k_b, c.tab_k[i], MSAM_D16, CI)) return e;
    }
    for (int i = 0; i < 2; ++i) {
        if (int e = gemm(cx, c.pos_bf16, C, dec->layer[i].i2t.q_w, T, CI, C, nullptr, c.pe_q[i], MSAM_F32, CI)) return e;
        if (int e = gemm(cx, c.pos_bf16, C, dec->layer[i].i2t.q_w, T, CI, C, dec->layer[i].i2t.q_b, c.tab_q[i], MSAM_D16, CI))
            return e;
    }
    if (msam_chain_const2_bytes() != CONST2_BYTES) { msam_set_error("msam_decoder_prepare_const: const2 size mismatch"); return 2; }
    return msam_chain_prepare_const2(dec->layer[1].t2i.v_w, dec->layer[1].t2i.v_b, dec->layer[1].t2i.k_w, dec->layer[0].n4_w,
                                     dec->layer[0].n4_b, dec->layer[0].i2t.o_w, dec->layer[0].i2t.o_b, c.chain2, stream);
}

extern "C" int msam_decoder_prepare_image(const msam_decoder_t* dec, const void* consts, const float* embedding,
                                          void* image_state, void* workspace, int64_t workspace_bytes, void* stream) {
    (void)workspace; (void)workspace_bytes;
    if (!dec || !consts || !embedding || !image_state) { msam_set_error("msam_decoder_prepare_image: null argument"); return 1; }
    Ctx cx{(hipStream_t)stream, dec->use_glds};
    Consts c = carve_consts((void*)consts);
    ImageState im = carve_image(image_state);
    hipLaunchKernelGGL(src_prepare_kernel, dim3(T / 32, C / 32), dim3(256), 0, cx.s, embedding, dec->no_mask, im.src_f32,
                       im.src_bf16);
    if (int e = msam_check_launch("src_prepare")) return e;
    if (int e = wsgemm_kv(cx, im.src_bf16, c.wkv[0], c.bkv[0], c.pe_k[0], T, im.k0, im.vT0)) return e;
    return gemm(cx, im.src_bf16, C, dec->layer[0].i2t.q_w, T, CI, C, dec->layer[0].i2t.q_b, im.q0, MSAM_D16, CI, 0,
                nullptr, 0, 0, 0, c.pe_q[0], CI);
}

extern int g_tune_dec_chain, g_tune_dec_chain_min_p, g_tune_chain_variant, g_tune_chain_handover;
int g_tune_tok_fuse = 0;
int g_tune_mlp_split_fused = 1;
namespace {
struct Work {
    float *qpe, *queries, *tmp; u16 *a, *b, *qs, *ks, *vs, *attn_tok, *mlp_h;
    u16 *keys, *kimg, *vT, *qimg, *attn_img, *up1; float* pre;
    u16 *hh0, *hh1; float *hyper, *iou_full;
    void* hand;
};
long work_bytes(int P, int Nt) {
    const long M = (long)P * Nt, R = (long)P * T;
    long b = 0;
    b += 3 * align256(M * C * 4);
    b += 6 * align256(M * C * 2);
    b += align256(M * 2048 * 2);
    b += align256(R * C * 2);
    b += 4 * align256(R * CI * 2);
    b += align256(R * C * 2);
    b += align256(R * C * 4);
    b += 2 * align256(5L * P * C * 2);
    b += align256((long)P * 4 * 128 * 4) + align256((long)P * 128 * 4);
    b += align256(msam_chain_handover_bytes(P));
    return b;
}
Work carve_work(void* base, int P, int Nt) {
    const long M = (long)P * Nt, R = (long)P * T;
    Work w; char* p = (char*)base;
    auto take = [&](long bytes) { char* r = p; p += align256(bytes); return r; };
    w.qpe = (float*)take(M * C * 4); w.queries = (float*)take(M * C * 4); w.tmp = (float*)take(M * C * 4);
    w.a = (u16*)take(M * C * 2); w.b = (u16*)take(M * C * 2); w.qs = (u16*)take(M * C * 2); w.ks = (u16*)take(M * C * 2);
    w.vs = (u16*)take(M * C * 2); w.attn_tok = (u16*)take(M * C * 2);
    w.mlp_h = (u16*)take(M * 2048 * 2);
    w.keys = (u16*)take(R * C * 2);
    w.kimg = (u16*)take(R * CI * 2); w.vT = (u16*)take(R * CI * 2); w.qimg = (u16*)take(R * CI * 2);
    w.attn_img = (u16*)take(R * CI * 2);
    w.up1 = (u16*)take(R * C * 2);
    w.pre = (float*)take(R * C * 4);
    w.hh0 = (u16*)take(5L * P * C * 2); w.hh1 = (u16*)take(5L * P * C * 2);
    w.hyper = (float*)take((long)P * 4 * 128 * 4); w.iou_full = (float*)take((long)P * 128 * 4);
    w.hand = take(msam_chain_handover_bytes(P));
    return w;
}

int t2i_stream(const Ctx& cx, const Work& w, const Consts& c, int idx, const msam_attn_w_t& aw, int P, int Nt, bool blocked = false) {
    const long R = (long)P * T;
    if (Nt <= 8) {
        const int64_t avail = (int64_t)((char*)w.up1 - (char*)w.kimg);
        return msam_t2i_fold_attention(w.keys, blocked ? 2 : 0, w.qs, P, Nt, aw.k_w, c.tab_k[idx], aw.v_w, aw.v_b, w.attn_tok, w.kimg,
                                       avail, cx.s);
    }
    if (int e = wsgemm_kv(cx, w.keys, c.wkv[idx], c.bkv[idx], c.pe_k[idx], (int)R, w.kimg, w.vT)) return e;
    hipLaunchKernelGGL(t2i_attn_kernel, dim3(P * 8), dim3(256), 0, cx.s, w.qs, w.kimg, w.vT, 0, Nt, w.attn_tok);
    return msam_check_launch("t2i_attn");
}

__global__ void gather_iou_kernel(const float* __restrict__ iou_full, int P, int c0, int nc, float* __restrict__ iou) {
    const int i = blockIdx.x * 256 + threadIdx.x;
    if (i < P * nc) iou[i] = iou_full[(long)(i / nc) * 128 + c0 + (i % nc)];
}
}

extern "C" int64_t msam_decoder_workspace_bytes(int32_t P) { return work_bytes(P, 16); }

extern "C" int msam_decoder_forward(const msam_decoder_t* dec, const void* consts, const void* image_state,
                                    const float* points, const int32_t* labels, int32_t Np, const float* boxes, int32_t P,
                                    int32_t multimask, float* low_res, float* iou, void* workspace, int64_t workspace_bytes,
                                    void* stream) {
    return msam_decoder_forward_masks(dec, nullptr, consts, image_state, points, labels, Np, boxes, nullptr, P, multimask,
                                      low_res, iou, workspace, workspace_bytes, stream);
}

namespace {
int decoder_run(const msam_decoder_t* dec, const msam_mask_prompt_t* mask_w, const void* consts,
                const void* image_state, const float* points, const int32_t* labels, int32_t Np,
                const float* boxes, const float* mask_input, const float* sparse, int32_t Ns, const float* dense,
                const float* embedding, int32_t P, int32_t multimask,
                float* low_res, float* iou, void* workspace, int64_t workspace_bytes, void* stream);
}

extern "C" int msam_decoder_forward_masks(const msam_decoder_t* dec, const msam_mask_prompt_t* mask_w, const void* consts,
                                          const void* image_state, const float* points, const int32_t* labels, int32_t Np,
                                          const float* boxes, const float* mask_input, int32_t P, int32_t multimask,
                                          float* low_res, float* iou, void* workspace, int64_t workspace_bytes, void* stream) {
    return decoder_run(dec, mask_w, consts, image_state, points, labels, Np, boxes, mask_input, nullptr, 0, nullptr, nullptr, P,
                       multimask, low_res, iou, workspace, workspace_bytes, stream);
}

extern "C" int msam_decoder_forward_embeddings(const msam_decoder_t* dec, const void* consts, const void* image_state,
                                               const float* sparse, int32_t Ns, const float* dense, const float* embedding,
                                               int32_t P, int32_t multimask, float* low_res, float* iou, void* workspace,
                                               int64_t workspace_bytes, void* stream) {
    if (!sparse && Ns != 0) { msam_set_error("msam_decoder_forward_embeddings: Ns > 0 needs the sparse embeddings"); return 1; }
    if (Ns < 0 || Ns > 11) { msam_set_error("msam_decoder_forward_embeddings: 0 .. 11 sparse tokens per prompt"); return 1; }
    if (dense && !embedding) { msam_set_error("msam_decoder_forward_embeddings: a dense embedding needs the image embedding"); return 1; }
    return decoder_run(dec, nullptr, consts, image_state, nullptr, nullptr, 0, nullptr, nullptr, sparse ? sparse : (const float*)consts,
                       Ns, dense, embedding, P, multimask, low_res, iou, workspace, workspace_bytes, stream);
}

extern "C" int msam_prompt_encode(const msam_decoder_t* dec, const msam_mask_prompt_t* mask_w, const float* points,
                                  const int32_t* labels, int32_t Np, const float* boxes, const float* mask_input, int32_t P,
                                  float* sparse, float* dense, void* stream) {
    if (!dec || P <= 0) { msam_set_error("msam_prompt_encode: null argument"); return 1; }
    if (!points) Np = 0;
    const int Ns = Np + (boxes ? 2 : (Np > 0 ? 1 : 0));
    if (Ns > 0) {
        if (!sparse) { msam_set_error("msam_prompt_encode: null sparse output"); return 1; }
        hipLaunchKernelGGL(sparse_embed_kernel, dim3(P), dim3(256), 0, (hipStream_t)stream, dec->pe_gauss, dec->point_embed,
                           dec->not_a_point, points, labels, Np, boxes, P, Ns, sparse);
        if (int e = msam_check_launch("sparse_embed")) return e;
    }
    if (mask_input) {
        if (!mask_w || !dense) { msam_set_error("msam_prompt_encode: mask prompts need the mask_downscaling weights and a dense output"); return 1; }
        hipLaunchKernelGGL(mask_src_kernel, dim3(64, P), dim3(256), 0, (hipStream_t)stream, mask_input, *mask_w, (const float*)nullptr,
                           dec->no_mask, (u16*)nullptr, dense);
        if (int e = msam_check_launch("mask_dense")) return e;
    }
    return 0;
}

namespace {
int decoder_run(const msam_decoder_t* dec, const msam_mask_prompt_t* mask_w, const void* consts,
                const void* image_state, const float* points, const int32_t* labels, int32_t Np,
                const float* boxes, const float* mask_input, const float* sparse, int32_t Ns, const float* dense,
                const float* embedding, int32_t P, int32_t multimask,
                float* low_res, float* iou, void* workspace, int64_t workspace_bytes, void* stream) {
    if (!dec || !consts || !image_state || !low_res || !iou || !workspace || P <= 0) {
        msam_set_error("msam_decoder_forward: null argument");
        return 1;
    }
    if (!sparse && (!points || Np <= 0) && !boxes && !mask_input && !dense) {
        msam_set_error("msam_decoder_forward: need points, boxes and / or a mask prompt");
        return 1;
    }
    if (mask_input && !mask_w) { msam_set_error("msam_decoder_forward: mask prompts need the mask_downscaling weights"); return 1; }
    const bool own_src = mask_input != nullptr || dense != nullptr;
    if (!points) Np = 0;
    const int Nt = sparse ? 5 + Ns : 5 + Np + (boxes ? 2 : (Np > 0 ? 1 : 0));
    if (Nt > 16) { msam_set_error("msam_decoder_forward: at most 16 tokens per prompt (<= 10 points)"); return 1; }
    if (workspace_bytes < work_bytes(P, Nt)) { msam_set_error("msam_decoder_forward: workspace too small"); return 1; }
    Ctx cx{(hipStream_t)stream, dec->use_glds};
    Consts c = carve_consts((void*)consts);
    ImageState im = carve_image((void*)image_state);
    Work w = carve_work(workspace, P, Nt);
    const int M = P * Nt;
    const long R = (long)P * T;
    const long n4 = (long)M * C / 4;
    int e;
#define CHECK(x) do { if ((e = (x))) return e; } while (0)
#define ADD_CAST(a_, b_, out_) do { hipLaunchKernelGGL(add_cast_kernel, dim3(grid_for(n4)), dim3(256), 0, cx.s, a_, b_, out_, n4); \
                                     CHECK(msam_check_launch("add_cast")); } while (0)
#define ADD_CAST2(a_, b_, outa_, outb_) do { hipLaunchKernelGGL(add_cast2_kernel, dim3(grid_for(n4)), dim3(256), 0, cx.s, a_, b_, outa_, \
                                                                 outb_, n4); CHECK(msam_check_launch("add_cast2")); } while (0)
#define LN(x_, w_, b_, rows_, out_, dt_) CHECK(msam_layernorm(x_, w_, b_, 1e-5f, rows_, C, out_, dt_, 0, 0, cx.s))

    if (dense) {
        hipLaunchKernelGGL(dense_src_kernel, dim3(T / 32, C / 32, P), dim3(256), 0, cx.s, embedding, dense, w.keys);
        CHECK(msam_check_launch("dense_src"));
    } else if (own_src) {
        hipLaunchKernelGGL(mask_src_kernel, dim3(64, P), dim3(256), 0, cx.s, mask_input, *mask_w, im.src_f32, dec->no_mask, w.keys,
                           (float*)nullptr);
        CHECK(msam_check_launch("mask_src"));
    }
    if (sparse) {
        hipLaunchKernelGGL(tokens_from_sparse_kernel, dim3(P), dim3(256), 0, cx.s, dec->out_tokens, sparse, Ns, P, Nt, w.qpe,
                           w.queries, w.a);
        CHECK(msam_check_launch("tokens_from_sparse"));
    } else {
        hipLaunchKernelGGL(prompt_tokens_kernel, dim3(P), dim3(256), 0, cx.s, dec->pe_gauss, dec->point_embed, dec->not_a_point,
                           dec->out_tokens, points, labels, Np, boxes, P, Nt, w.qpe, w.queries, w.a);
        CHECK(msam_check_launch("prompt_tokens"));
    }

    const char* dbg = getenv("MSAM_DEBUG_DEC_LAYERS");
    const int nlayers = dbg ? atoi(dbg) : 2;
    const bool chain = g_tune_dec_chain && !own_src && !dbg && Nt <= 8 && P >= g_tune_dec_chain_min_p;
    const bool fuse_tok = g_tune_tok_fuse != 0 && !dbg;
    void* const oper0 = w.qimg; void* const oper1 = w.attn_img;
    void* const tables = (char*)w.vT + (int64_t)R * CI * 2 - msam_chain_tables_bytes();
    if (chain) CHECK(msam_chain_prepare_tables(im.src_bf16, im.q0, c.tab_k[1], c.tab_q[1], tables, cx.s));
    const bool chain2 = chain && g_tune_chain_variant == 9;
    void* const tables2 = (char*)tables - msam_chain_tables2_bytes();
    void* const mfrag = (char*)oper0 + msam_i2t_fold_operand_bytes(P);
    if (chain2) CHECK(msam_chain_prepare_tables2_c(im.src_bf16, c.chain2, tables2, cx.s));
    const bool handover = chain2 && g_tune_chain_handover != 0;
    for (int li = 0; li < nlayers && li < 2; ++li) {
        const msam_twoway_layer_t& L = dec->layer[li];
        const u16* sv = w.a;
        if (li > 0) {
            if (!fuse_tok) ADD_CAST2(w.queries, w.qpe, w.a, w.b);
            sv = w.b;
        }
        {
            const msam_gemm_t qkv[3] = {mk_gemm(w.a, C, L.self_attn.q_w, M, C, C, L.self_attn.q_b, w.qs, MSAM_D16, C),
                                        mk_gemm(w.a, C, L.self_attn.k_w, M, C, C, L.self_attn.k_b, w.ks, MSAM_D16, C),
                                        mk_gemm(sv, C, L.self_attn.v_w, M, C, C, L.self_attn.v_b, w.vs, MSAM_D16, C)};
            CHECK(msam_gemm_group_bf16(qkv, 3, cx.s));
        }
        hipLaunchKernelGGL(token_self_attn_kernel, dim3(P), dim3(128), 0, cx.s, w.qs, w.ks, w.vs, Nt, w.attn_tok);
        CHECK(msam_check_launch("token_self_attn"));
        if (fuse_tok) {
            CHECK(gemm_ln_tok(cx, w.attn_tok, C, L.self_attn.o_w, M, C, L.self_attn.o_b, li == 0 ? nullptr : w.queries, L.n1_w, L.n1_b,
                              w.queries, w.qpe, w.a, nullptr));
        } else {
        CHECK(gemm(cx, w.attn_tok, C, L.self_attn.o_w, M, C, C, L.self_attn.o_b, w.tmp, MSAM_F32, C, 0,
                   li == 0 ? nullptr : w.queries, li == 0 ? 0 : MSAM_F32, C));
        LN(w.tmp, L.n1_w, L.n1_b, M, w.queries, MSAM_F32);
        ADD_CAST(w.queries, w.qpe, w.a);
        }
        CHECK(gemm(cx, w.a, C, L.t2i.q_w, M, CI, C, L.t2i.q_b, w.qs, MSAM_D16, CI));
        if (li == 0 && !own_src) {
            if (Nt <= 8)
                hipLaunchKernelGGL(t2i_shared4_kernel, dim3(((P + 3) / 4) * 8), dim3(256), 0, cx.s, w.qs, im.k0, im.vT0, P, Nt,
                                   w.attn_tok);
            else
                hipLaunchKernelGGL(t2i_attn_kernel, dim3(P * 8), dim3(256), 0, cx.s, w.qs, im.k0, im.vT0, 1, Nt, w.attn_tok);
            CHECK(msam_check_launch("t2i_attn"));
        } else if (chain) {
            const msam_twoway_layer_t& L0 = dec->layer[0];
            const int64_t avail = (int64_t)R * CI * 2 - msam_chain_tables_bytes() - msam_chain_tables2_bytes();
            if (handover)
                CHECK(msam_i2t0_t2i_fused_v2_handover(tables, tables2, oper0, mfrag, L0.n4_w, 1e-5f, w.qs, P, Nt, L.t2i.k_w, w.attn_tok,
                                                      w.vT, avail, w.hand, cx.s));
            else if (chain2)
                CHECK(msam_i2t0_t2i_fused_v2(tables, tables2, oper0, mfrag, L0.n4_w, 1e-5f, w.qs, P, Nt, L.t2i.k_w, w.attn_tok, w.vT,
                                             avail, cx.s));
            else
                CHECK(msam_i2t0_t2i_fused(tables, oper0, L0.n4_w, L0.n4_b, 1e-5f, w.qs, P, Nt, L.t2i.k_w, L.t2i.v_w, L.t2i.v_b,
                                          w.attn_tok, w.vT, avail, cx.s));
        } else {
            CHECK(t2i_stream(cx, w, c, li, L.t2i, P, Nt));
        }
        if (fuse_tok) {
            CHECK(gemm_ln_tok(cx, w.attn_tok, CI, L.t2i.o_w, M, CI, L.t2i.o_b, w.queries, L.n2_w, L.n2_b, w.queries, nullptr, w.a, nullptr));
        } else {
        CHECK(gemm(cx, w.attn_tok, CI, L.t2i.o_w, M, C, CI, L.t2i.o_b, w.tmp, MSAM_F32, C, 0, w.queries, MSAM_F32, C));
        LN(w.tmp, L.n2_w, L.n2_b, M, w.queries, MSAM_F32);
        if (!(L.mlp1_ws != nullptr && L.mlp2_ws != nullptr)) ADD_CAST(w.queries, nullptr, w.a);
        }
        const bool mlp_split = L.mlp1_ws != nullptr && L.mlp2_ws != nullptr;
        const void* mlp_h = w.mlp_h; const void* mlp2_w = L.mlp2_w; int mlp2_k = 2048;
        if (mlp_split) {
            u16* a3 = (u16*)w.pre;
            float* h32 = (float*)((char*)a3 + align256((long)M * 3 * C * 2));
            u16* h3 = (u16*)((char*)h32 + align256((long)M * 2048 * 4));
            CHECK(msam_cast_f32_split16(w.queries, MSAM_D16, a3, M, C, cx.s));
            if (g_tune_mlp_split_fused) {
                msam_gemm_t g1 = mk_gemm(a3, 3 * C, L.mlp1_ws, M, 2048, 3 * C, L.mlp1_b, h3, MSAM_D16, 3 * 2048, MSAM_ACT_RELU);
                g1.out_mode = 3;
                CHECK(msam_gemm_bf16(&g1, cx.s));
            } else {
                CHECK(gemm(cx, a3, 3 * C, L.mlp1_ws, M, 2048, 3 * C, L.mlp1_b, h32, MSAM_F32, 2048, MSAM_ACT_RELU));
                CHECK(msam_cast_f32_split16(h32, MSAM_D16, h3, M, 2048, cx.s));
            }
            mlp_h = h3; mlp2_w = L.mlp2_ws; mlp2_k = 3 * 2048;
        } else {
        CHECK(gemm(cx, w.a, C, L.mlp1_w, M, 2048, C, L.mlp1_b, w.mlp_h, MSAM_D16, 2048, MSAM_ACT_RELU));
        }
        if (fuse_tok) {
            CHECK(gemm_ln_tok(cx, mlp_h, mlp2_k, mlp2_w, M, mlp2_k, L.mlp2_b, w.queries, L.n3_w, L.n3_b, w.queries, w.qpe, w.a, w.b));
        } else {
        CHECK(gemm(cx, mlp_h, mlp2_k, mlp2_w, M, C, mlp2_k, L.mlp2_b, w.tmp, MSAM_F32, C, 0, w.queries, MSAM_F32, C));
        LN(w.tmp, L.n3_w, L.n3_b, M, w.queries, MSAM_F32);
        ADD_CAST2(w.queries, w.qpe, w.a, w.b);
        }
        {
            const msam_gemm_t kv[2] = {mk_gemm(w.a, C, L.i2t.k_w, M, CI, C, L.i2t.k_b, w.ks, MSAM_D16, CI),
                                       mk_gemm(w.b, C, L.i2t.v_w, M, CI, C, L.i2t.v_b, w.vs, MSAM_D16, CI)};
            CHECK(msam_gemm_group_bf16(kv, 2, cx.s));
        }
        if (chain) {
            if (li == 0 && chain2)
                CHECK(msam_i2t_fold_operands_values(w.ks, w.vs, P, Nt, L.i2t.q_w, L.i2t.o_w, L.i2t.o_b, 0, tables2, oper0, mfrag, cx.s));
            else
                CHECK(msam_i2t_fold_operands(w.ks, w.vs, P, Nt, L.i2t.q_w, L.i2t.o_w, L.i2t.o_b, li, li == 0 ? oper0 : oper1, cx.s));
            if (li == 1) {
                const msam_twoway_layer_t& L0 = dec->layer[0];
                if (handover)
                    CHECK(msam_i2t01_fused_handover(tables, oper0, L0.n4_w, L0.n4_b, oper1, L.n4_w, L.n4_b, 1e-5f, P, Nt, w.hand, w.keys, cx.s));
                else
                    CHECK(msam_i2t01_fused(tables, oper0, L0.n4_w, L0.n4_b, oper1, L.n4_w, L.n4_b, 1e-5f, P, Nt, w.keys, cx.s));
            }
        } else if (Nt <= 8) {
            const bool shared = li == 0 && !own_src;
            CHECK(msam_i2t_fold_layer(shared ? (const void*)im.src_bf16 : (const void*)w.keys, shared, w.ks, w.vs, P, Nt,
                                      L.i2t.q_w, c.tab_q[li], L.i2t.o_w, L.i2t.o_b, L.n4_w, L.n4_b, 1e-5f, w.keys, w.qimg,
                                      (int64_t)((char*)w.up1 - (char*)w.qimg), cx.s));
        } else {
            msam_image_layer_t g{};
            g.wo = L.i2t.o_w; g.bo = L.i2t.o_b; g.ln_w = L.n4_w; g.ln_b = L.n4_b; g.ln_eps = 1e-5f;
            g.ktok = w.ks; g.vtok = w.vs; g.Nt = Nt; g.out = w.keys; g.rows = (int)R;
            if (li == 0 && !own_src) { g.xin = im.src_bf16; g.q_shared = im.q0; }
            else { g.xin = w.keys; g.wq = L.i2t.q_w; g.bq = L.i2t.q_b; g.peq = c.pe_q[li]; }
            CHECK(msam_decoder_image_layer(&g, cx.s));
        }
    }
    if (dbg) return 0;
    if (!fuse_tok) ADD_CAST(w.queries, w.qpe, w.a);
    CHECK(gemm(cx, w.a, C, dec->final_attn.q_w, M, CI, C, dec->final_attn.q_b, w.qs, MSAM_D16, CI));
    CHECK(t2i_stream(cx, w, c, 2, dec->final_attn, P, Nt, chain));
    if (fuse_tok) {
        CHECK(gemm_ln_tok(cx, w.attn_tok, CI, dec->final_attn.o_w, M, CI, dec->final_attn.o_b, w.queries, dec->nf_w, dec->nf_b, w.queries,
                          nullptr, w.a, nullptr));
    } else {
    CHECK(gemm(cx, w.attn_tok, CI, dec->final_attn.o_w, M, C, CI, dec->final_attn.o_b, w.tmp, MSAM_F32, C, 0, w.queries,
               MSAM_F32, C));
    LN(w.tmp, dec->nf_w, dec->nf_b, M, w.queries, MSAM_F32);

    ADD_CAST(w.queries, nullptr, w.a);
    }
    {
        msam_gemm_t h[5];
        const long PC = (long)P * C;
        for (int i = 0; i < 5; ++i) {
            const void* wt = i == 0 ? dec->iou_w[0] : dec->hyp_w[i - 1][0];
            const float* bs = i == 0 ? dec->iou_b[0] : dec->hyp_b[i - 1][0];
            h[i] = mk_gemm(w.a + (long)i * C, (long)Nt * C, wt, P, C, C, bs, w.hh0 + i * PC, MSAM_D16, C, MSAM_ACT_RELU);
        }
        CHECK(msam_gemm_group_bf16(h, 5, cx.s));
        for (int i = 0; i < 5; ++i) {
            const void* wt = i == 0 ? dec->iou_w[1] : dec->hyp_w[i - 1][1];
            const float* bs = i == 0 ? dec->iou_b[1] : dec->hyp_b[i - 1][1];
            h[i] = mk_gemm(w.hh0 + i * PC, C, wt, P, C, C, bs, w.hh1 + i * PC, MSAM_D16, C, MSAM_ACT_RELU);
        }
        CHECK(msam_gemm_group_bf16(h, 5, cx.s));
        h[0] = mk_gemm(w.hh1, C, dec->iou_w[2], P, 128, C, dec->iou_b[2], w.iou_full, MSAM_F32, 128);
        for (int i = 1; i < 5; ++i)
            h[i] = mk_gemm(w.hh1 + i * PC, C, dec->hyp_w[i - 1][2], P, 128, C, dec->hyp_b[i - 1][2], w.hyper + (long)(i - 1) * 128,
                           MSAM_F32, 4 * 128);
        CHECK(msam_gemm_group_bf16(h, 5, cx.s));
    }
    const int mask0 = multimask ? 1 : 0, nmask = multimask ? 3 : 1;
    hipLaunchKernelGGL(gather_iou_kernel, dim3((P * nmask + 255) / 256), dim3(256), 0, cx.s, w.iou_full, P, mask0, nmask, iou);
    CHECK(msam_check_launch("gather_iou"));

    CHECK(msam_upscale_fused_range(w.keys, (chain ? 1 : 0) | (dec->up1_centred ? 2 : 0), P, dec->up1_w, dec->up1_b, dec->up_ln_w, dec->up_ln_b, 1e-6f, dec->up2_w,
                                   dec->up2_b, w.hyper, 128, mask0, nmask, low_res, dec->low_res_dtype == MSAM_F16 ? MSAM_F16 : MSAM_F32,
                                   dec->low_res_range, cx.s));
#undef CHECK
#undef ADD_CAST
#undef ADD_CAST2
#undef LN
    return 0;
}
}
```

micro_sam_amd/instance_segmentation.py:

```python
from __future__ import annotations

from abc import ABC
from copy import deepcopy
from typing import Any, Dict, List, Optional, Union

import numpy as np
import torch

from . import amg_utils, ops, util
from .predictor import SamPredictor


class DeviceMaskData(amg_utils.MaskData):

    def __init__(self, mask_size=None, crop_box=None, full_size=None, **kwargs) -> None:
        super().__init__(**kwargs)
        self.mask_size = mask_size
        self.crop_box = crop_box
        self.full_size = full_size

    def _is_cropped(self) -> bool:
        return self.crop_box is not None and self.full_size is not None and tuple(self.mask_size) != tuple(self.full_size)

    def full_bits(self, bits: Optional[torch.Tensor] = None) -> torch.Tensor:
        bits = self._stats["bits"] if bits is None else bits
        if not self._is_cropped():
            return bits
        return ops.uncrop_bits(bits.contiguous(), self.crop_box, self.full_size[0], self.full_size[1])

    def __getitem__(self, key: str):
        if key == "rles" and "rles" not in self._stats and "bits" in self._stats:
            self._stats["rles"] = self._encode_rles()
        return self._stats[key]

    def _encode_rles(self):
        bits = self._stats["bits"]
        if bits.shape[0] == 0:
            return []
        if not self._is_cropped():
            h, w = self.mask_size
            counts, offsets = ops.rle_encode(bits.contiguous(), h, w)
            return ops.rles_to_list(counts, offsets, h, w, as_list=False)
        h, w = self.full_size
        out = []
        for s in range(0, bits.shape[0], 256):
            counts, offsets = ops.rle_encode(self.full_bits(bits[s:s + 256]), h, w)
            out.extend(ops.rles_to_list(counts, offsets, h, w, as_list=False))
        return out

    def shallow_copy(self) -> "DeviceMaskData":
        out = DeviceMaskData(mask_size=self.mask_size, crop_box=self.crop_box, full_size=self.full_size)
        out._stats = dict(self._stats)
        return out

    def cat(self, new_stats) -> None:
        new_cropped = isinstance(new_stats, DeviceMaskData) and new_stats._is_cropped()
        same_crop = new_cropped and self.crop_box is not None and list(self.crop_box) == list(new_stats.crop_box)
        if "rles" in self._stats and "rles" not in new_stats._stats and "bits" in new_stats._stats:
            new_stats["rles"]
        if new_cropped and not same_crop:
            items = dict(new_stats.items())
            if "bits" in items:
                items["bits"] = new_stats.full_bits()
            self.mask_size, self.crop_box = tuple(new_stats.full_size), None
            self.full_size = tuple(new_stats.full_size)
        else:
            items = dict(new_stats.items())
            if getattr(new_stats, "mask_size", None) is not None:
                self.mask_size = new_stats.mask_size
                if same_crop or (isinstance(new_stats, DeviceMaskData) and "bits" not in self._stats):
                    self.crop_box, self.full_size = new_stats.crop_box, new_stats.full_size
        for k, v in items.items():
            cur = self._stats.get(k)
            if cur is None:
                self._stats[k] = v
            elif isinstance(v, torch.Tensor):
                self._stats[k] = torch.cat([cur, v.to(cur.device)], dim=0)
            elif isinstance(v, np.ndarray):
                self._stats[k] = np.concatenate([cur, v], axis=0)
            else:
                self._stats[k] = cur + list(v)

    def __len__(self) -> int:
        return int(self._stats["iou_preds"].shape[0]) if "iou_preds" in self._stats else 0

    def __getstate__(self):
        stats = {}
        for k, v in self._stats.items():
            if k == "bits":
                continue
            stats[k] = v.cpu() if torch.is_tensor(v) else v
        if "bits" in self._stats:
            stats["rles"] = self["rles"]
        size = self.full_size if self._is_cropped() else self.mask_size
        return {"_stats": stats, "mask_size": size}

    def __setstate__(self, state):
        self._stats = state["_stats"]
        self.mask_size = state["mask_size"]
        self.crop_box = None
        self.full_size = state["mask_size"]


DEFAULT_SEGMENTATION_MODE_WITH_DECODER = "ais"


class AMGBase(ABC):
    def __init__(self):
        self._is_initialized = False
        self._crop_list = None
        self._crop_boxes = None
        self._original_size = None

    @property
    def is_initialized(self):
        return self._is_initialized

    @property
    def crop_list(self):
        return self._crop_list

    @property
    def crop_boxes(self):
        return self._crop_boxes

    @property
    def original_size(self):
        return self._original_size

    def _postprocess_batch(self, data, crop_box, original_size, pred_iou_thresh, stability_score_thresh, box_nms_thresh):
        orig_h, orig_w = original_size
        keep = ~amg_utils.is_box_near_crop_edge(data["boxes"], crop_box, [0, 0, orig_w, orig_h])
        if pred_iou_thresh > 0.0:
            keep = keep & (data["iou_preds"] > pred_iou_thresh).to(keep.device)
        if stability_score_thresh > 0.0:
            keep = keep & (data["stability_score"] >= stability_score_thresh).to(keep.device)
        idx = torch.nonzero(keep).squeeze(1)
        boxes, scores = data["boxes"][idx], data["iou_preds"][idx]
        if boxes.is_cuda:
            keep_by_nms = ops.box_nms(boxes, scores, box_nms_thresh)
        else:
            keep_by_nms = amg_utils.batched_nms(boxes.float(), scores, torch.zeros_like(boxes[:, 0]), iou_threshold=box_nms_thresh)
        data.filter(idx[keep_by_nms.to(idx.device)])
        data["boxes"] = amg_utils.uncrop_boxes_xyxy(data["boxes"], crop_box)
        data["crop_boxes"] = torch.tensor([crop_box for _ in range(int(data["iou_preds"].shape[0]))])
        try:
            data["points"] = amg_utils.uncrop_points(data["points"], crop_box)
        except KeyError:
            pass
        return data

    def _postprocess_batch_prepare(self, data, crop_box, original_size, pred_iou_thresh, stability_score_thresh, box_nms_thresh):
        orig_h, orig_w = original_size
        keep = ~amg_utils.is_box_near_crop_edge(data["boxes"], crop_box, [0, 0, orig_w, orig_h])
        if pred_iou_thresh > 0.0:
            keep = keep & (data["iou_preds"] > pred_iou_thresh)
        if stability_score_thresh > 0.0:
            keep = keep & (data["stability_score"] >= stability_score_thresh)
        scores = data["iou_preds"].float()
        flags = ops.box_nms_flags(data["boxes"], scores, keep, box_nms_thresh)
        order = torch.sort(torch.where(flags, scores, torch.full_like(scores, float("-inf"))), descending=True, stable=True).indices
        return order, flags.sum()

    def _postprocess_batch_finish(self, data, crop_box, order, count: int):
        data.filter(order[:count])
        data["boxes"] = amg_utils.uncrop_boxes_xyxy(data["boxes"], crop_box)
        data["crop_boxes"] = torch.tensor([crop_box for _ in range(int(data["iou_preds"].shape[0]))])
        try:
            data["points"] = amg_utils.uncrop_points(data["points"], crop_box)
        except KeyError:
            pass
        return data

    def _postprocess_small_regions(self, mask_data, min_area, nms_thresh):
        from ._vendored import batched_mask_to_box
        rles = list(mask_data["rles"])
        if len(rles) == 0:
            return mask_data
        for k in ("bits", "area"):
            if k in mask_data:
                del mask_data[k]
        mask_data["rles"] = rles
        new_masks, scores = [], []
        for rle in rles:
            mask = amg_utils.rle_to_mask(rle)
            mask, changed = amg_utils.remove_small_regions(mask, min_area, mode="holes")
            unchanged = not changed
            mask, changed = amg_utils.remove_small_regions(mask, min_area, mode="islands")
            unchanged = unchanged and not changed
            new_masks.append(torch.as_tensor(mask, dtype=torch.int).unsqueeze(0))
            scores.append(float(unchanged))
        masks = torch.cat(new_masks, dim=0)
        boxes = batched_mask_to_box(masks.to(torch.bool))
        keep_by_nms = amg_utils.batched_nms(boxes.float(), torch.as_tensor(scores, dtype=torch.float),
                                            torch.zeros_like(boxes[:, 0]), iou_threshold=nms_thresh)
        box_col = torch.as_tensor(mask_data["boxes"]).clone()
        for i_mask in keep_by_nms.tolist():
            if scores[i_mask] == 0.0:
                mask_data["rles"][i_mask] = amg_utils.mask_to_rle_numpy(masks[i_mask].numpy().astype(bool))
                box_col[i_mask] = boxes[i_mask].to(box_col.dtype)
        mask_data["boxes"] = box_col.numpy() if isinstance(mask_data["boxes"], np.ndarray) else box_col
        mask_data.filter(keep_by_nms)
        return mask_data

    def _postprocess_masks(self, mask_data, min_mask_region_area, box_nms_thresh, crop_nms_thresh, output_mode):
        if min_mask_region_area > 0:
            mask_data = self._postprocess_small_regions(mask_data, min_mask_region_area, max(box_nms_thresh, crop_nms_thresh))
        if output_mode == "coco_rle":
            mask_data["segmentations"] = [amg_utils.coco_encode_rle(rle) for rle in mask_data["rles"]]
        elif output_mode in ("binary_mask", "instance_segmentation"):
            if "bits" in mask_data:
                h, w = mask_data.mask_size
                dense = ops.unpack_bits(torch.as_tensor(mask_data["bits"]), h).cpu().numpy()
                mask_data["segmentations"] = [m for m in dense]
            else:
                mask_data["segmentations"] = [amg_utils.rle_to_mask(rle) for rle in mask_data["rles"]]
        elif output_mode == "rle":
            mask_data["segmentations"] = [{"size": r["size"], "counts": np.asarray(r["counts"]).tolist()}
                                          for r in mask_data["rles"]]
        else:
            raise ValueError(f"Invalid output mode {output_mode}.")
        curr_anns = []
        for idx in range(len(mask_data["segmentations"])):
            ann = {
                "segmentation": mask_data["segmentations"][idx],
                "area": int(mask_data["area"][idx]) if "area" in mask_data else amg_utils.area_from_rle(mask_data["rles"][idx]),
                "bbox": amg_utils.box_xyxy_to_xywh(mask_data["boxes"][idx]).tolist(),
                "predicted_iou": mask_data["iou_preds"][idx].item(),
                "stability_score": mask_data["stability_score"][idx].item(),
                "crop_box": amg_utils.box_xyxy_to_xywh(mask_data["crop_boxes"][idx]).tolist(),
            }
            try:
                ann["point_coords"] = [mask_data["points"][idx].tolist()]
            except KeyError:
                pass
            curr_anns.append(ann)
        return curr_anns

    def _to_mask_data_device(self, iou_preds, post, crop_box, original_size, points=None):
        orig_h, orig_w = original_size
        x0, y0, x1, y1 = crop_box
        full_image = (x0 == 0 and y0 == 0 and x1 == orig_w and y1 == orig_h)
        n_masks_per_prompt = iou_preds.shape[1]
        data = DeviceMaskData(mask_size=(orig_h, orig_w) if full_image else (y1 - y0, x1 - x0),
                              crop_box=None if full_image else list(crop_box), full_size=(orig_h, orig_w),
                              iou_preds=iou_preds.flatten(0, 1))
        if points is not None:
            data["points"] = torch.as_tensor(points.repeat(n_masks_per_prompt, axis=0), dtype=torch.float)
        counts = post["counts"]
        data["stability_score"] = counts[:, 0] / counts[:, 1]
        data["boxes"] = post["boxes"]
        data["area"] = counts[:, 2]
        data["bits"] = post["bits"]
        return data

    def get_state(self) -> Dict[str, Any]:
        if not self.is_initialized:
            raise RuntimeError("The state has not been computed yet. Call initialize first.")
        return {"crop_list": self.crop_list, "crop_boxes": self.crop_boxes, "original_size": self.original_size}

    def set_state(self, state: Dict[str, Any]) -> None:
        self._crop_list = state["crop_list"]
        self._crop_boxes = state["crop_boxes"]
        self._original_size = state["original_size"]
        self._is_initialized = True

    def clear_state(self):
        self._crop_list = None
        self._crop_boxes = None
        self._original_size = None
        self._is_initialized = False


class AutomaticMaskGenerator(AMGBase):

    def __init__(self, predictor: SamPredictor, points_per_side: Optional[int] = 32, points_per_batch: Optional[int] = None,
                 crop_n_layers: int = 0, crop_overlap_ratio: float = 512 / 1500, crop_n_points_downscale_factor: int = 1,
                 point_grids: Optional[List[np.ndarray]] = None, stability_score_offset: float = 1.0,
                 device_chunk: int = 1024):
        super().__init__()
        self._device_chunk = int(device_chunk)
        if points_per_side is not None:
            self.point_grids = amg_utils.build_all_layer_point_grids(points_per_side, crop_n_layers,
                                                                     crop_n_points_downscale_factor)
        elif point_grids is not None:
            self.point_grids = point_grids
        else:
            raise ValueError("Can't have both points_per_side and point_grid be None or not None.")
        self._predictor = predictor
        self._points_per_side = points_per_side
        self._points_per_batch = 64 if points_per_batch is None else points_per_batch
        self._crop_n_layers = crop_n_layers
        self._crop_overlap_ratio = crop_overlap_ratio
        self._crop_n_points_downscale_factor = crop_n_points_downscale_factor
        self._stability_score_offset = stability_score_offset

    def _lane_clone(self, lane_predictor: Optional[SamPredictor] = None) -> "AutomaticMaskGenerator":
        import copy
        clone = copy.copy(self)
        clone._predictor = lane_predictor if lane_predictor is not None else SamPredictor(self._predictor.model.lane_view())
        clone._prompt_cache = {}
        clone._lanes = clone._post_stream = None
        clone.clear_state()
        return clone

    def _decode_lanes(self, n: int):
        dev = self._predictor.device
        pool = getattr(self._predictor, "_lane_pool", None) or []
        if pool and (pool[0][0].device != dev or pool[0][0].model.mask_decoder is not self._predictor.model.mask_decoder):
            pool = []
        while len(pool) < n:
            pool.append((SamPredictor(self._predictor.model.lane_view()), torch.cuda.Stream(device=dev)))
        self._predictor._lane_pool = pool
        main = self._predictor.model
        for lp, _ in pool[:n]:
            lm, stale = lp.model, False
            for k in ("precision", "split_token_mlp", "use_glds", "amg_low_res_dtype"):
                if getattr(lm, k, None) != getattr(main, k, None):
                    setattr(lm, k, getattr(main, k))
                    stale = stale or k in ("split_token_mlp", "use_glds")
            if stale:
                lm._dec = None
                lm._img_state = None
        lanes = getattr(self, "_lanes", None) or []
        if lanes and any(l[0]._predictor is not p for l, (p, _) in zip(lanes, pool)):
            lanes = []
        while len(lanes) < n:
            lp, st = pool[len(lanes)]
            lanes.append((self._lane_clone(lp), st))
        self._lanes = lanes
        for clone, _ in lanes[:n]:
            for k in ("point_grids", "_points_per_side", "_points_per_batch", "_crop_n_layers", "_crop_overlap_ratio",
                      "_crop_n_points_downscale_factor", "_stability_score_offset", "_device_chunk"):
                setattr(clone, k, getattr(self, k))
        return lanes[:n]

    def _process_batch(self, points, im_size, crop_box, original_size):
        key = (points.shape, tuple(im_size), float(points[0, 0]), float(points[-1, -1]))
        cached = self._prompt_cache.get(key) if hasattr(self, "_prompt_cache") else None
        if cached is None or cached[0].device != self._predictor.device or not np.array_equal(cached[2], points):
            transformed_points = self._predictor.transform.apply_coords(points, im_size)
            in_points = torch.as_tensor(transformed_points, device=self._predictor.device, dtype=torch.float)
            in_labels = torch.ones(in_points.shape[0], dtype=torch.int, device=in_points.device)
            if not hasattr(self, "_prompt_cache"):
                self._prompt_cache = {}
            if len(self._prompt_cache) > 64:
                self._prompt_cache.clear()
            self._prompt_cache[key] = (in_points, in_labels, np.array(points, copy=True))
        else:
            in_points, in_labels = cached[0], cached[1]
        iou_preds, post = self._predictor.predict_masks_device(
            in_points[:, None, :], in_labels[:, None], multimask_output=True,
            stability_score_offset=self._stability_score_offset)
        return self._to_mask_data_device(iou_preds, post, crop_box, original_size, points=points)

    def _process_crop(self, image, crop_box, crop_layer_idx, precomputed_embeddings, pbar_init=None, pbar_update=None):
        x0, y0, x1, y1 = crop_box
        cropped_im = image[y0:y1, x0:x1, :]
        cropped_im_size = cropped_im.shape[:2]
        if not precomputed_embeddings:
            self._predictor.set_image(cropped_im)
        points_scale = np.array(cropped_im_size)[None, ::-1]
        points_for_image = self.point_grids[crop_layer_idx] * points_scale
        full_image = (x0 == 0 and y0 == 0 and (y1, x1) == tuple(self.original_size))
        data = DeviceMaskData(mask_size=tuple(self.original_size) if full_image else tuple(cropped_im_size),
                              crop_box=None if full_image else list(crop_box), full_size=tuple(self.original_size))
        n_batches = len(points_for_image) // self._points_per_batch + \
            int(len(points_for_image) % self._points_per_batch != 0)
        if pbar_init is not None:
            pbar_init(n_batches, "Predict masks for point grid prompts")
        chunk = max(self._device_chunk, self._points_per_batch)
        for (points,) in amg_utils.batch_iterator(chunk, points_for_image):
            batch_data = self._process_batch(points, cropped_im_size, crop_box, self.original_size)
            data.cat(batch_data)
            del batch_data
            if pbar_update is not None:
                pbar_update(int(np.ceil(len(points) / self._points_per_batch)))
        if not precomputed_embeddings:
            self._predictor.reset_image()
        return data

    @torch.no_grad()
    def initialize(self, image: np.ndarray, image_embeddings=None, i: Optional[int] = None, verbose: bool = False,
                   pbar_init: Optional[callable] = None, pbar_update: Optional[callable] = None) -> None:
        original_size = image.shape[:2]
        self._original_size = original_size
        crop_boxes, layer_idxs = amg_utils.generate_crop_boxes(original_size, self._crop_n_layers,
                                                               self._crop_overlap_ratio)
        if len(crop_boxes) == 1:
            if image_embeddings is None:
                image_embeddings = util.precompute_image_embeddings(self._predictor, image, verbose=verbose)
            util.set_precomputed(self._predictor, image_embeddings, i=i)
            precomputed_embeddings = True
        else:
            precomputed_embeddings = False
        if precomputed_embeddings:
            image = np.broadcast_to(np.zeros((1, 1, 1), dtype=np.uint8), tuple(original_size) + (3,))
        else:
            image = util._to_image(image)
        _, pbar_init, pbar_update, pbar_close = util.handle_pbar(verbose, pbar_init, pbar_update)
        crop_list = []
        for crop_box, layer_idx in zip(crop_boxes, layer_idxs):
            crop_list.append(self._process_crop(image, crop_box, layer_idx, precomputed_embeddings=precomputed_embeddings,
                                                pbar_init=pbar_init, pbar_update=pbar_update))
        pbar_close()
        self._is_initialized = True
        self._crop_list = crop_list
        self._crop_boxes = crop_boxes

    @torch.no_grad()
    def generate_device(self, pred_iou_thresh: float = 0.88, stability_score_thresh: float = 0.95,
                        box_nms_thresh: float = 0.7, with_background: bool = True, min_object_size: int = 0,
                        stream: Optional["torch.cuda.Stream"] = None):
        if not self.is_initialized:
            raise RuntimeError("AutomaticMaskGenerator has not been initialized. Call initialize first.")
        if len(self.crop_list) != 1 or "bits" not in self.crop_list[0]:
            raise RuntimeError("generate_device needs the single-crop device state produced by initialize()")
        if stream is not None:
            stream.wait_stream(torch.cuda.current_stream(stream.device))
            for k in ("iou_preds", "stability_score", "boxes", "area", "bits"):
                self.crop_list[0][k].record_stream(stream)
            with torch.cuda.stream(stream):
                return self.generate_device(pred_iou_thresh, stability_score_thresh, box_nms_thresh, with_background,
                                            min_object_size)
        data, crop_box = self.crop_list[0], self.crop_boxes[0]
        orig_h, orig_w = self.original_size
        if 0 < len(data) <= 4096 and tuple(crop_box) == (0, 0, orig_w, orig_h) and not getattr(self, "_torch_glue_generate", False):
            return ops.amg_generate_labels(data["iou_preds"], data["stability_score"], data["boxes"], data["area"], data["bits"],
                                           self.original_size, crop_box, pred_iou_thresh, stability_score_thresh, box_nms_thresh,
                                           min_object_size=min_object_size, with_background=with_background)
        valid = torch.ones_like(data["iou_preds"], dtype=torch.bool)
        if pred_iou_thresh > 0.0:
            valid &= data["iou_preds"] > pred_iou_thresh
        if stability_score_thresh > 0.0:
            valid &= data["stability_score"] >= stability_score_thresh
        valid &= ~amg_utils.is_box_near_crop_edge(data["boxes"], crop_box, [0, 0, orig_w, orig_h])
        keep = ops.box_nms_flags(data["boxes"], data["iou_preds"], valid, box_nms_thresh)
        return util.masks_to_segmentation_device(data["bits"], data["area"], keep, self.original_size,
                                                 min_object_size=min_object_size, with_background=with_background)

    @torch.no_grad()
    def generate(self, pred_iou_thresh: float = 0.88, stability_score_thresh: float = 0.95, box_nms_thresh: float = 0.7,
                 crop_nms_thresh: float = 0.7, min_mask_region_area: int = 0, output_mode: str = "instance_segmentation",
                 with_background: bool = True) -> Union[List[Dict[str, Any]], np.ndarray]:
        if not self.is_initialized:
            raise RuntimeError("AutomaticMaskGenerator has not been initialized. Call initialize first.")
        if (output_mode == "instance_segmentation" and min_mask_region_area == 0 and len(self.crop_list) == 1
                and isinstance(self.crop_list[0], DeviceMaskData) and "bits" in self.crop_list[0]
                and 0 < len(self.crop_list[0]) <= 4096
                and tuple(self.crop_boxes[0]) == (0, 0, self.original_size[1], self.original_size[0])
                and not getattr(self, "_general_generate", False)):
            labels, flag = self.generate_device(pred_iou_thresh, stability_score_thresh, box_nms_thresh, with_background)
            out = util.fetch_to_host(torch.cat([labels.reshape(-1), flag]), tag="labels")
            if out[-1] == 0:
                return out[:-1].reshape(self.original_size).view(np.uint32)
        data = DeviceMaskData()
        on_device = len(self.crop_list) > 1 and all(
            isinstance(d, DeviceMaskData) and len(d) > 0 and all(torch.is_tensor(d[k]) and d[k].is_cuda for k in ("boxes", "iou_preds", "stability_score"))
            for d in self.crop_list)
        if on_device:
            prepared = [self._postprocess_batch_prepare(d, cb, self.original_size, pred_iou_thresh, stability_score_thresh, box_nms_thresh)
                        for d, cb in zip(self.crop_list, self.crop_boxes)]
            counts = torch.stack([c for _, c in prepared]).tolist()
            for data_, crop_box, (order, _), n in zip(self.crop_list, self.crop_boxes, prepared, counts):
                data.cat(self._postprocess_batch_finish(data_.shallow_copy(), crop_box, order, int(n)))
        else:
            for data_, crop_box in zip(self.crop_list, self.crop_boxes):
                crop_data = self._postprocess_batch(
                    data=data_.shallow_copy() if isinstance(data_, DeviceMaskData) else deepcopy(data_),
                    crop_box=crop_box, original_size=self.original_size,
                    pred_iou_thresh=pred_iou_thresh, stability_score_thresh=stability_score_thresh,
                    box_nms_thresh=box_nms_thresh)
                data.cat(crop_data)
        if len(self.crop_boxes) > 1 and len(data["crop_boxes"]) > 0:
            scores = 1 / amg_utils.box_area(data["crop_boxes"])
            scores = scores.to(data["boxes"].device)
            keep_by_nms = amg_utils.batched_nms(data["boxes"].float(), scores, torch.zeros_like(data["boxes"][:, 0]),
                                                iou_threshold=crop_nms_thresh)
            data.filter(keep_by_nms)
        if output_mode == "instance_segmentation" and min_mask_region_area == 0 and "bits" in data:
            return util.mask_data_to_segmentation_device(data["bits"], data["area"], self.original_size,
                                                         with_background=with_background)
        bits = data["bits"] if "bits" in data else None
        if bits is not None:
            del data["bits"]
        data.to_numpy()
        if bits is not None:
            data["bits"] = bits
        masks = self._postprocess_masks(data, min_mask_region_area, box_nms_thresh, crop_nms_thresh, output_mode)
        if output_mode == "instance_segmentation":
            shape = next(iter(masks))["segmentation"].shape if len(masks) > 0 else self.original_size
            masks = util.mask_data_to_segmentation(masks, shape=shape, with_background=with_background,
                                                   merge_exclusively=False)
        return masks


def _process_tiled_embeddings(predictor, image, image_embeddings, tile_shape, halo, verbose, batch_size, mask, i):
    if image_embeddings is None:
        if tile_shape is None or halo is None:
            raise ValueError("To compute tiled embeddings the parameters tile_shape and halo have to be passed.")
        image_embeddings = util.precompute_image_embeddings(predictor, image, tile_shape=tile_shape, halo=halo,
                                                            verbose=verbose, batch_size=batch_size, mask=mask)
    feats = image_embeddings["features"]
    tile_shape_, halo_ = tuple(feats.attrs["tile_shape"]), tuple(feats.attrs["halo"])
    if tile_shape is None:
        tile_shape = tile_shape_
# ... 367 lines not shown
```

micro_sam_amd/modeling.py:

```python
from __future__ import annotations

import ctypes as C
import os
from typing import List, Optional, Tuple, Union

import torch
import torch.nn as nn
import torch.nn.functional as F

from . import _lib

VIT_CONFIGS = {
    "vit_b": dict(embed_dim=768, depth=12, num_heads=12, global_attn_indexes=(2, 5, 8, 11)),
    "vit_l": dict(embed_dim=1024, depth=24, num_heads=16, global_attn_indexes=(5, 11, 17, 23)),
    "vit_h": dict(embed_dim=1280, depth=32, num_heads=16, global_attn_indexes=(7, 15, 23, 31)),
}
IMG_SIZE, PATCH, GRID, WINDOW, PROMPT_DIM = 1024, 16, 64, 14, 256


def _bf16(t: torch.Tensor) -> torch.Tensor:
    return t.detach().to(torch.bfloat16).contiguous()


def _d16(t: torch.Tensor) -> torch.Tensor:
# ... 515 lines not shown
        up = md.output_upscaling
        w1 = up[0].weight.detach().float().permute(2, 3, 1, 0).reshape(4, 64, PROMPT_DIM)
        b1 = up[0].bias.detach().float()
        centred = os.environ.get("MSAM_UP_CENTRED", "1") != "0"
        if centred:
            w1 = w1 - w1.mean(dim=1, keepdim=True)
            b1 = b1 - b1.mean()
        p.up1_w = k(_d16(w1.reshape(4 * 64, PROMPT_DIM)))
        p.up1_b = k(_f32(b1.repeat(4)))
        p.up1_centred = 1 if centred else 0
        p.up_ln_w, p.up_ln_b = k(_f32(up[1].weight)), k(_f32(up[1].bias))
        p.up2_w = k(_d16(up[3].weight.permute(2, 3, 1, 0).reshape(4 * 32, 64)))
        p.up2_b = k(_f32(up[3].bias))

        def pad_rows(wt, bs, rows=128):
            wp = torch.zeros((rows, wt.shape[1]), dtype=wt.dtype, device=wt.device)
            wp[: wt.shape[0]] = wt
            bp = torch.zeros((rows,), dtype=bs.dtype, device=bs.device)
            bp[: bs.shape[0]] = bs
            return wp, bp

        for i, mlp in enumerate(md.output_hypernetworks_mlps):
            for j, lin in enumerate(mlp.layers):
                wt, bs = lin.weight.detach(), lin.bias.detach()
                if j == 2:
                    wt, bs = pad_rows(wt, bs)
                p.hyp_w[i][j], p.hyp_b[i][j] = k(_d16(wt)), k(_f32(bs))
        for j, lin in enumerate(md.iou_prediction_head.layers):
            wt, bs = lin.weight.detach(), lin.bias.detach()
            if j == 2:
                wt, bs = pad_rows(wt, bs)
            p.iou_w[j], p.iou_b[j] = k(_d16(wt)), k(_f32(bs))
        p.use_glds = int(self.use_glds)
        ds = pe.mask_downscaling
        mp = _lib.MaskPromptParams()
        mp.c1_w, mp.c1_b = k(_f32(ds[0].weight.reshape(-1))), k(_f32(ds[0].bias))
        mp.ln1_w, mp.ln1_b = k(_f32(ds[1].weight)), k(_f32(ds[1].bias))
        mp.c2_w, mp.c2_b = k(_f32(ds[3].weight.reshape(-1))), k(_f32(ds[3].bias))
        mp.ln2_w, mp.ln2_b = k(_f32(ds[4].weight)), k(_f32(ds[4].bias))
        mp.c3_w, mp.c3_b = k(_f32(ds[6].weight.reshape(PROMPT_DIM, 16))), k(_f32(ds[6].bias))
        mp.exact_gelu = 1 if self.reference_formulation else 0
        self._mask_params = mp
        lib = _lib.load()
        consts = torch.empty(lib.msam_decoder_const_bytes(), dtype=torch.uint8, device=dev)
        _lib.check(lib.msam_decoder_prepare_const(C.byref(p), consts.data_ptr(), _lib.stream_ptr()),
                   "msam_decoder_prepare_const")
        self._dec = (p, keep, consts)
        self._dec_versions = self._watch.key()
        return self._dec

    def _dense_pe(self) -> torch.Tensor:
        _, _, consts = self._prepare_decoder()
        pos = consts[: GRID * GRID * PROMPT_DIM * 4].view(torch.float32).reshape(GRID * GRID, PROMPT_DIM)
        return pos.t().reshape(1, PROMPT_DIM, GRID, GRID).contiguous()

    def _image_state(self, features: torch.Tensor, prepared=None) -> torch.Tensor:
        key = (features.data_ptr(), features._version, tuple(features.shape))
        p, _, consts = prepared if prepared is not None else self._prepare_decoder()
        if self._img_state is not None and self._img_state[0] == key and self._img_state[3] is features:
            return self._img_state[1]
        lib = _lib.load()
        feats = features.to(device=self.device, dtype=torch.float32).reshape(PROMPT_DIM, GRID * GRID).contiguous()
        state = torch.empty(lib.msam_decoder_image_bytes(), dtype=torch.uint8, device=self.device)
        _lib.check(lib.msam_decoder_prepare_image(C.byref(p), consts.data_ptr(), feats.data_ptr(), state.data_ptr(),
                                                  None, 0, _lib.stream_ptr()), "msam_decoder_prepare_image")
        self._img_state = (key, state, feats, features)
        return state

    def _workspace(self, P: int) -> torch.Tensor:
        need = _lib.load().msam_decoder_workspace_bytes(P)
        if self._dec_ws is None or self._dec_ws.numel() < need or self._dec_ws.device != self.device:
            self._dec_ws = None
            self._dec_ws = torch.empty(need, dtype=torch.uint8, device=self.device)
        return self._dec_ws

    @torch.no_grad()
    def _prompt_encode(self, points, boxes, masks):
        p, _, _ = self._prepare_decoder()
        dev = self.device
        pts = lbl = bx = msk = None
        if points is not None:
            pts = points[0].to(device=dev, dtype=torch.float32).contiguous()
            lbl = points[1].to(device=dev, dtype=torch.int32).contiguous()
            B, Np = pts.shape[0], pts.shape[1]
        else:
            Np = 0
            B = boxes.shape[0] if boxes is not None else (masks.shape[0] if masks is not None else 1)
        if boxes is not None:
            bx = boxes.to(device=dev, dtype=torch.float32).reshape(-1, 4).contiguous()
        if masks is not None:
            msk = masks.to(device=dev, dtype=torch.float32).reshape(-1, 4 * GRID, 4 * GRID).contiguous()
            if msk.shape[0] != B:
                raise ValueError(f"masks holds {msk.shape[0]} masks for {B} prompts")
        Ns = Np + (2 if boxes is not None else (1 if Np > 0 else 0))
        sparse = torch.empty((B, Ns, PROMPT_DIM), dtype=torch.float32, device=dev)
        dense = torch.empty((B, PROMPT_DIM, GRID, GRID), dtype=torch.float32, device=dev) if msk is not None else None
        if Ns > 0 or msk is not None:
            self._mask_params.exact_gelu = 1 if self.reference_formulation else 0
            _lib.check(_lib.load().msam_prompt_encode(
                C.byref(p), C.byref(self._mask_params), _lib.ptr(pts), _lib.ptr(lbl), Np, _lib.ptr(bx), _lib.ptr(msk), B,
                _lib.ptr(sparse) if Ns > 0 else None, _lib.ptr(dense), _lib.stream_ptr()), "msam_prompt_encode")
        if dense is None:
            dense = self.prompt_encoder.no_mask_embed.weight.detach().to(dev).reshape(1, -1, 1, 1).expand(B, -1, GRID, GRID)
        return sparse, dense

    @torch.no_grad()
    def _decode_embeddings(self, image_embeddings, image_pe, sparse, dense, multimask_output: bool):
        if image_embeddings.numel() != PROMPT_DIM * GRID * GRID:
            raise NotImplementedError("micro_sam_amd: mask_decoder takes ONE image embedding [1,256,64,64] per call "
                                      f"(got {tuple(image_embeddings.shape)})")
        p, _, consts = self._prepare_decoder()
        dev = self.device
        if self.reference_formulation:
            nm = self.prompt_encoder.no_mask_embed.weight.detach().to(dev).reshape(1, -1, 1, 1)
            dn = dense.to(device=dev, dtype=torch.float32)
            no_mask = (dn.stride(-1) == 0 and dn.stride(-2) == 0 and torch.equal(dn[:, :, :1, :1], nm.expand(dn.shape[0], -1, 1, 1))) \
                or bool(torch.equal(dn, nm.expand_as(dn)))
            return self._decode_strict(image_embeddings, sparse.to(device=dev, dtype=torch.float32), None if no_mask else dn,
                                       multimask_output)
        own_pe = self._dense_pe()
        if image_pe is not None and (tuple(image_pe.shape) != tuple(own_pe.shape) or
                                     not torch.allclose(image_pe.to(device=dev, dtype=torch.float32), own_pe, atol=1e-5)):
            raise NotImplementedError("micro_sam_amd: mask_decoder needs image_pe == prompt_encoder.get_dense_pe() "
                                      "(the positional projections are precomputed tables)")
        state = self._image_state(image_embeddings)
        sp = sparse.to(device=dev, dtype=torch.float32).contiguous()
        P, Ns = sp.shape[0], sp.shape[1]
        if Ns > 11:
            raise ValueError(f"at most 11 sparse prompt tokens per prompt, got {Ns}")
        nm = self.prompt_encoder.no_mask_embed.weight.detach().to(dev).reshape(1, -1, 1, 1)
        dn = dense.to(device=dev, dtype=torch.float32)
        is_no_mask = (dn.stride(-1) == 0 and dn.stride(-2) == 0 and torch.equal(dn[:, :, :1, :1], nm.expand(dn.shape[0], -1, 1, 1))) \
            or bool(torch.equal(dn, nm.expand_as(dn)))
        dptr = eptr = None
        if not is_no_mask:
            if dn.shape[0] != P:
                raise ValueError(f"dense_prompt_embeddings holds {dn.shape[0]} entries for {P} prompts")
            dn = dn.contiguous()
            emb = image_embeddings.to(device=dev, dtype=torch.float32).reshape(PROMPT_DIM, GRID * GRID).contiguous()
            dptr, eptr = dn.data_ptr(), emb.data_ptr()
        nc = 3 if multimask_output else 1
        low = torch.empty((P, nc, 256, 256), dtype=torch.float32, device=dev)
        iou = torch.empty((P, nc), dtype=torch.float32, device=dev)
        ws = self._workspace(P)
        p.low_res_dtype = _lib.F32
        p.low_res_range = None
        _lib.check(_lib.load().msam_decoder_forward_embeddings(
            C.byref(p), consts.data_ptr(), state.data_ptr(), sp.data_ptr() if Ns > 0 else None, Ns, dptr, eptr, P,
            1 if multimask_output else 0, low.data_ptr(), iou.data_ptr(), ws.data_ptr(), ws.numel(), _lib.stream_ptr()),
            "msam_decoder_forward_embeddings")
        return low, iou

    @torch.no_grad()
    def decode(self, features: torch.Tensor, point_coords: Optional[torch.Tensor], point_labels: Optional[torch.Tensor],
               boxes: Optional[torch.Tensor] = None, mask_input: Optional[torch.Tensor] = None,
               multimask_output: bool = True, low_res_dtype: torch.dtype = torch.float32,
               range_map: Union[bool, torch.Tensor] = False) -> Tuple[torch.Tensor, ...]:
        want_range = range_map is not False and range_map is not None
        if want_range and (low_res_dtype != torch.float32 or self.reference_formulation or mask_input is not None):
            raise ValueError("range_map goes with float32 low-res logits of the kernel path, without a mask prompt")
        if low_res_dtype not in (torch.float32, torch.float16):
            raise ValueError("low_res_dtype is torch.float32 or torch.float16")
        if features.numel() != PROMPT_DIM * GRID * GRID:
            raise ValueError(f"expected one image embedding [1,256,64,64], got {tuple(features.shape)}")
        if self.reference_formulation:
            if point_coords is None and boxes is None and mask_input is None:
                raise ValueError("micro_sam_amd: a prompt needs points, a box and / or a mask input")
            pts = None if point_coords is None else (point_coords, point_labels)
            msk = None if mask_input is None else mask_input.reshape(-1, 1, 4 * GRID, 4 * GRID)
            sparse, dense = self._prompt_encode(pts, None if boxes is None else boxes.reshape(-1, 4), msk)
            low, iou = self._decode_strict(features, sparse, dense if mask_input is not None else None, multimask_output)
            return (low if low_res_dtype == torch.float32 else low.to(low_res_dtype)), iou
        prepared = self._prepare_decoder()
        p, _, consts = prepared
        state = self._image_state(features, prepared)
        lib = _lib.load()
        dev = self.device
        if point_coords is not None:
            pts = point_coords.to(device=dev, dtype=torch.float32).contiguous()
            lbl = point_labels.to(device=dev, dtype=torch.int32).contiguous()
            P, Np = pts.shape[0], pts.shape[1]
        else:
            if boxes is None and mask_input is None:
                raise ValueError("micro_sam_amd: a prompt needs points, a box and / or a mask input")
            pts = lbl = None
            P, Np = (boxes.shape[0] if boxes is not None else mask_input.reshape(-1, 4 * GRID, 4 * GRID).shape[0]), 0
        bx = None if boxes is None else boxes.to(device=dev, dtype=torch.float32).reshape(-1, 4).contiguous()
        nc = 3 if multimask_output else 1
        low = torch.empty((P, nc, 256, 256), dtype=low_res_dtype, device=dev)
        iou = torch.empty((P, nc), dtype=torch.float32, device=dev)
        p.low_res_dtype = _lib.F16 if low_res_dtype == torch.float16 else _lib.F32
        rng = None
        if want_range:
            rng = range_map if isinstance(range_map, torch.Tensor) else torch.empty((P, nc, 256, 4, 2), dtype=torch.float32, device=dev)
            if rng.dtype != torch.float32 or tuple(rng.shape) != (P, nc, 256, 4, 2) or not rng.is_contiguous() or rng.device != low.device:
                raise ValueError(f"range_map must be a contiguous float32 tensor [{P},{nc},256,4,2] on {low.device}")
        p.low_res_range = _lib.ptr(rng)
        need = lib.msam_decoder_workspace_bytes(P)
        if self._dec_ws is None or self._dec_ws.numel() < need or self._dec_ws.device != dev:
            self._dec_ws = None
            self._dec_ws = torch.empty(need, dtype=torch.uint8, device=dev)
        msk = None
        if mask_input is not None:
            msk = mask_input.to(device=dev, dtype=torch.float32).reshape(-1, 4 * GRID, 4 * GRID).contiguous()
            if msk.shape[0] != P:
                raise ValueError(f"mask_input holds {msk.shape[0]} masks for {P} prompts")
        _lib.check(lib.msam_decoder_forward_masks(
            C.byref(p), C.byref(self._mask_params), consts.data_ptr(), state.data_ptr(), _lib.ptr(pts), _lib.ptr(lbl), Np,
            _lib.ptr(bx), _lib.ptr(msk), P, 1 if multimask_output else 0, low.data_ptr(), iou.data_ptr(),
            self._dec_ws.data_ptr(), self._dec_ws.numel(), _lib.stream_ptr()), "msam_decoder_forward")
        if want_range:
            return low, iou, rng
        return low, iou


def build_sam(model_type: str = "vit_b", num_multimask_outputs: int = 3) -> Sam:
    key = model_type[:5]
    if key == "vit_t":
        from .models.tiny_vit import TinyViT
        sam = Sam(TinyViT(), PromptEncoder(), MaskDecoder(num_multimask_outputs))
        sam.eval()
        return sam
    if key not in VIT_CONFIGS:
        raise ValueError(f"Invalid model_type: {model_type}. Expect one of {tuple(VIT_CONFIGS) + ('vit_t',)}")
    cfg = VIT_CONFIGS[key]
    sam = Sam(ImageEncoderViT(cfg["embed_dim"], cfg["depth"], cfg["num_heads"], cfg["global_attn_indexes"]),
              PromptEncoder(), MaskDecoder(num_multimask_outputs))
    sam.eval()
    return sam


sam_model_registry = {
    "vit_b": lambda **kw: build_sam("vit_b", **kw),
    "vit_l": lambda **kw: build_sam("vit_l", **kw),
    "vit_h": lambda **kw: build_sam("vit_h", **kw),
    "vit_t": lambda **kw: build_sam("vit_t", **kw),
}
```

micro_sam_amd/predictor.py:

```python
from __future__ import annotations

from typing import Optional, Tuple

import numpy as np
import torch

from .modeling import Sam
from .transforms import ResizeLongestSide


class SamPredictor:
    def __init__(self, sam_model: Sam) -> None:
        self.model = sam_model
        self.transform = ResizeLongestSide(sam_model.image_encoder.img_size)
        self.reset_image()

    @property
    def device(self) -> torch.device:
        return self.model.device

    def set_precision(self, mode: str) -> None:
        self.model.set_precision(mode)

    def reset_image(self) -> None:
        self.model._img_state = None
        self.is_image_set = False
        self.features = None
        self.orig_h = self.orig_w = self.input_h = self.input_w = None
        self.original_size = None
        self.input_size = None

    def set_image(self, image: np.ndarray, image_format: str = "RGB") -> None:
        assert image_format in ["RGB", "BGR"], f"image_format must be in ['RGB', 'BGR'], is {image_format}."
        if image_format != self.model.image_format:
            image = image[..., ::-1]
        input_image = self.transform.apply_image(image)
        self.reset_image()
        self.original_size = tuple(image.shape[:2])
        self.input_size = tuple(input_image.shape[:2])
        u8 = torch.as_tensor(np.ascontiguousarray(input_image), device=self.device)[None]
        self.features = self.model.image_encoder.forward_u8(u8)
        self.is_image_set = True

    @torch.no_grad()
    def set_torch_image(self, transformed_image: torch.Tensor, original_image_size: Tuple[int, ...]) -> None:
        assert (len(transformed_image.shape) == 4 and transformed_image.shape[1] == 3
                and max(*transformed_image.shape[2:]) == self.model.image_encoder.img_size), \
            f"set_torch_image input must be BCHW with long side {self.model.image_encoder.img_size}."
        self.reset_image()
        self.original_size = tuple(original_image_size)
        self.input_size = tuple(transformed_image.shape[-2:])
        input_image = self.model.preprocess(transformed_image.to(self.device).float())
        self.features = self.model.image_encoder(input_image)
        self.is_image_set = True

    def get_image_embedding(self) -> torch.Tensor:
        if not self.is_image_set:
            raise RuntimeError("An image must be set with .set_image(...) to generate an embedding.")
        assert self.features is not None, "Features must exist if an image has been set."
        return self.features

    def predict(self, point_coords: Optional[np.ndarray] = None, point_labels: Optional[np.ndarray] = None,
                box: Optional[np.ndarray] = None, mask_input: Optional[np.ndarray] = None,
                multimask_output: bool = True, return_logits: bool = False):
        if not self.is_image_set:
            raise RuntimeError("An image must be set with .set_image(...) before mask prediction.")
        coords_torch = labels_torch = box_torch = mask_input_torch = None
        if point_coords is not None:
            assert point_labels is not None, "point_labels must be supplied if point_coords is supplied."
            point_coords = self.transform.apply_coords(point_coords, self.original_size)
            coords_torch = torch.as_tensor(point_coords, dtype=torch.float, device=self.device)[None, :, :]
            labels_torch = torch.as_tensor(point_labels, dtype=torch.int, device=self.device)[None, :]
        if box is not None:
            box = self.transform.apply_boxes(box, self.original_size)
            box_torch = torch.as_tensor(box, dtype=torch.float, device=self.device)[None, :]
        if mask_input is not None:
            mask_input_torch = torch.as_tensor(mask_input, dtype=torch.float, device=self.device)[None, :, :, :]
        masks, iou, low = self.predict_torch(coords_torch, labels_torch, box_torch, mask_input_torch, multimask_output,
                                             return_logits=return_logits)
        return masks[0].detach().cpu().numpy(), iou[0].detach().cpu().numpy(), low[0].detach().cpu().numpy()

    @torch.no_grad()
    def predict_torch(self, point_coords: Optional[torch.Tensor], point_labels: Optional[torch.Tensor],
                      boxes: Optional[torch.Tensor] = None, mask_input: Optional[torch.Tensor] = None,
                      multimask_output: bool = True, return_logits: bool = False):
        if not self.is_image_set:
            raise RuntimeError("An image must be set with .set_image(...) before mask prediction.")
        low, iou = self.model.decode(self.features, point_coords, point_labels, boxes, mask_input, multimask_output)
        from .ops import postprocess_masks, unpack_bits
        b, c = low.shape[:2]
        res = postprocess_masks(low.reshape(b * c, 256, 256), self.input_size, self.original_size,
                                self.model.mask_threshold, 1.0, want_logits=return_logits)
        if return_logits:
            masks = res["logits"].reshape(b, c, *self.original_size)
        else:
            masks = unpack_bits(res["bits"], self.original_size[0]).reshape(b, c, *self.original_size)
        return masks, iou, low

    @torch.no_grad()
    def predict_masks_device(self, point_coords, point_labels, boxes=None, multimask_output: bool = True,
                             stability_score_offset: float = 1.0):
        if not self.is_image_set:
            raise RuntimeError("An image must be set with .set_image(...) before mask prediction.")
        from . import _lib
        dt = self.model.amg_low_res_dtype
        with_map = (dt == torch.float32 and not self.model.reference_formulation
                    and tuple(int(v) for v in self.input_size) == (1024, 1024)
                    and tuple(int(v) for v in self.original_size) == (1024, 1024) and _lib.tune_get("amg_range_map") == 1)
        out = self.model.decode(self.features, point_coords, point_labels, boxes, None, multimask_output, low_res_dtype=dt,
                                range_map=with_map)
        low, iou = out[0], out[1]
        from .ops import postprocess_masks
        b, c = low.shape[:2]
        res = postprocess_masks(low.reshape(b * c, 256, 256), self.input_size, self.original_size,
                                self.model.mask_threshold, stability_score_offset, want_logits=False,
                                range_map=out[2].reshape(b * c, 256, 4, 2) if with_map else None)
        return iou, res
```

Before: 185.9 tiles/s.

## Cache image-independent prompt-token prefix across tiles and generalise shared t2i kernel

Adds a prompt-prefix path: the image-independent part of the mask decoder (point/box token embeddings, initial queries and the first token-to-image query projection) is computed once per point grid and kept in a small host-side cache keyed on the points. Later decoder calls for other tiles with the same grid reuse it instead of recomputing it. The shared token-to-image attention kernel is also templated on group size, and its K/V loads are software-prefetched one step ahead. In exchange there is extra prefix memory and cache bookkeeping, and a risk of stale prefixes if the weights or settings change, which the code guards with an owner and constants check.

```diff
diff --git a/include/msam_hip.h b/include/msam_hip.h
--- a/include/msam_hip.h
+++ b/include/msam_hip.h
@@ -299,6 +299,15 @@
                                const void* image_state, const float* points, const int32_t* labels, int32_t Np,
                                const float* boxes, const float* mask_input, int32_t P, int32_t multimask, float* low_res,
                                float* iou, void* workspace, int64_t workspace_bytes, void* stream);
+
+int64_t msam_decoder_prompt_prefix_bytes(int32_t P, int32_t Nt);
+int msam_decoder_prompt_prefix(const msam_decoder_t* dec, const float* points, const int32_t* labels, int32_t Np,
+                               const float* boxes, int32_t P, void* prefix, void* workspace, int64_t workspace_bytes, void* stream);
+int msam_decoder_forward_masks_prefixed(const msam_decoder_t* dec, const msam_mask_prompt_t* mask_w, const void* consts,
+                                        const void* image_state, const float* points, const int32_t* labels, int32_t Np,
+                                        const float* boxes, const float* mask_input, const void* prefix, int32_t P,
+                                        int32_t multimask, float* low_res, float* iou, void* workspace, int64_t workspace_bytes,
+                                        void* stream);
 
 int msam_prompt_encode(const msam_decoder_t* dec, const msam_mask_prompt_t* mask_w, const float* points,
                        const int32_t* labels, int32_t Np, const float* boxes, const float* mask_input, int32_t P,
diff --git a/micro_sam_amd/_lib.py b/micro_sam_amd/_lib.py
--- a/micro_sam_amd/_lib.py
+++ b/micro_sam_amd/_lib.py
@@ -129,6 +129,10 @@
     "msam_uncrop_bits": (_i32, [_vp, _i32, _i32, _i32, _i32, _i32, _i32, _i32, _vp, _vp]),
     "msam_decoder_forward_masks": (_i32, [C.POINTER(DecoderParams), C.POINTER(MaskPromptParams), _vp, _vp, _vp, _vp, _i32, _vp, _vp,
                                           _i32, _i32, _vp, _vp, _vp, _i64, _vp]),
+    "msam_decoder_prompt_prefix_bytes": (_i64, [_i32, _i32]),
+    "msam_decoder_prompt_prefix": (_i32, [C.POINTER(DecoderParams), _vp, _vp, _i32, _vp, _i32, _vp, _vp, _i64, _vp]),
+    "msam_decoder_forward_masks_prefixed": (_i32, [C.POINTER(DecoderParams), C.POINTER(MaskPromptParams), _vp, _vp, _vp, _vp, _i32, _vp,
+                                                   _vp, _vp, _i32, _i32, _vp, _vp, _vp, _i64, _vp]),
     "msam_i2t_fold_workspace_bytes": (_i64, [_i32]),
     "msam_i2t_fold_layer": (_i32, [_vp, _i32, _vp, _vp, _i32, _i32, _vp, _vp, _vp, _vp, _vp, _vp, _f32, _vp, _vp, _i64, _vp]),
     "msam_profile_enable": (_i32, [_i32]),
diff --git a/micro_sam_amd/_prompt_prefix.py b/micro_sam_amd/_prompt_prefix.py
--- /dev/null
+++ b/micro_sam_amd/_prompt_prefix.py
@@ -0,0 +1,35 @@
+from collections import OrderedDict
+from typing import Any, Callable, Hashable, Optional, Tuple
+
+import numpy as np
+
+MAX_ENTRIES = 8
+
+
+class PromptPrefixCache:
+
+    def __init__(self, max_entries: int = MAX_ENTRIES):
+        self.max_entries = int(max_entries)
+        self._owner = None
+        self._entries: "OrderedDict[Hashable, Tuple[np.ndarray, Any]]" = OrderedDict()
+
+    def __len__(self) -> int:
+        return len(self._entries)
+
+    def clear(self) -> None:
+        self._entries.clear()
+        self._owner = None
+
+    def get(self, key: Hashable, points_host: np.ndarray, owner: Any, make: Callable[[np.ndarray], Any]):
+        if owner is not self._owner:
+            self._entries.clear()
+            self._owner = owner
+        hit: Optional[Tuple[np.ndarray, Any]] = self._entries.get(key)
+        if hit is not None and np.array_equal(hit[0], points_host):
+            return hit[1]
+        value = make(points_host)
+        self._entries.pop(key, None)
+        while len(self._entries) >= self.max_entries:
+            self._entries.popitem(last=False)
+        self._entries[key] = (np.array(points_host, copy=True), value)
+        return value
diff --git a/micro_sam_amd/csrc/decfold.hip b/micro_sam_amd/csrc/decfold.hip
--- a/micro_sam_amd/csrc/decfold.hip
+++ b/micro_sam_amd/csrc/decfold.hip
@@ -703,6 +703,7 @@
 extern int g_tune_chain_handover, g_tune_chain_handover_ring;
 extern int g_tune_mlp_split_fused;
 extern int g_tune_amg_range_map;
+extern int g_tune_t2i_shared_group, g_tune_prompt_prefix;
 extern int g_tune_sgemm_bufs, g_tune_srel_mfma, g_tune_sgemm_small_below, g_tune_si2t_dbg, g_tune_si2t_late_us, g_tune_sattn_allh;
 int g_tune_dec_chain = 1, g_tune_dec_chain_min_p = 128;
 extern "C" int msam_tune_set(const char* key, int32_t value) {
@@ -718,6 +719,8 @@
     else if (k == "up_ln_two_pass") g_tune_up_ln_two_pass = value;
     else if (k == "up_centred") g_tune_up_centred = value;
     else if (k == "amg_range_map") g_tune_amg_range_map = value;
+    else if (k == "t2i_shared_group") g_tune_t2i_shared_group = value;
+    else if (k == "prompt_prefix") g_tune_prompt_prefix = value;
     else if (k == "gemm_dbg") msam_gemm_set_dbg(value);
     else if (k == "gw_delay") msam_gemm_set_gw(value, -1);
     else if (k == "gw_class") msam_gemm_set_gw(-2, value);
@@ -737,7 +740,7 @@
 }
 extern "C" int msam_tune_get(const char* key, int32_t* value) {
     const std::string k = key ? key : "";
-    if (!value || k != "amg_range_map") { msam_set_error("msam_tune_get: unknown key"); return 1; }
-    *value = g_tune_amg_range_map;
+    if (!value || (k != "amg_range_map" && k != "prompt_prefix")) { msam_set_error("msam_tune_get: unknown key"); return 1; }
+    *value = k == "prompt_prefix" ? g_tune_prompt_prefix : g_tune_amg_range_map;
     return 0;
 }
diff --git a/micro_sam_amd/csrc/decoder.hip b/micro_sam_amd/csrc/decoder.hip
--- a/micro_sam_amd/csrc/decoder.hip
+++ b/micro_sam_amd/csrc/decoder.hip
@@ -359,34 +359,47 @@
     }
 }
 
-__global__ __launch_bounds__(256) void t2i_shared4_kernel(const u16* __restrict__ qtok, const u16* __restrict__ kimg,
-                                                          const u16* __restrict__ vT, int P, int Nt, u16* __restrict__ out) {
-    __shared__ float red[4][32][20];
+template <int G>
+__global__ __launch_bounds__(256, 2) void t2i_shared_kernel(const u16* __restrict__ qtok, const u16* __restrict__ kimg,
+                                                         const u16* __restrict__ vT, int P, int Nt, u16* __restrict__ out) {
+    constexpr int NT = G / 2;
+    __shared__ float red[4][NT * 16][20];
     const int pg = blockIdx.x >> 3, head = blockIdx.x & 7;
     const int tid = threadIdx.x, lane = tid & 63, wave = tid >> 6, fr = lane & 15, fg = lane >> 4;
     const u16* kb = kimg + (long)head * T * 16;
     const u16* vb = vT + ((long)head * 16 + fr) * T;
     const int tk = fr & 7;
-    uint4 qf[2];
-#pragma unroll
-    for (int n = 0; n < 2; ++n) {
-        const int p = pg * 4 + n * 2 + (fr >> 3);
+    const int left = P - pg * G;
+    const int nt = left >= G ? NT : (left + 1) >> 1;
+    uint4 qf[NT];
+#pragma unroll
+    for (int n = 0; n < NT; ++n) {
+        const int p = pg * G + n * 2 + (fr >> 3);
         qf[n] = make_uint4(0, 0, 0, 0);
         if (fg < 2 && tk < Nt && p < P) qf[n] = *(const uint4*)(qtok + ((long)p * Nt + tk) * CI + head * 16 + fg * 8);
     }
-    f32x4_t o[2] = {{0.f, 0.f, 0.f, 0.f}, {0.f, 0.f, 0.f, 0.f}};
-    float m[2] = {NEG_BIG, NEG_BIG}, l[2] = {0.f, 0.f};
+    f32x4_t o[NT];
+    float m[NT], l[NT];
+#pragma unroll
+    for (int n = 0; n < NT; ++n) { o[n] = f32x4_t{0.f, 0.f, 0.f, 0.f}; m[n] = NEG_BIG; l[n] = 0.f; }
     const int t_begin = wave * (T / 4), t_end = t_begin + T / 4;
+    uint4 ka0 = make_uint4(0, 0, 0, 0), ka1 = ka0, kn0 = ka0, kn1 = ka0;
+    if (fg < 2) {
+        kn0 = *(const uint4*)(kb + (long)(t_begin + fr) * 16 + fg * 8);
+        kn1 = *(const uint4*)(kb + (long)(t_begin + 16 + fr) * 16 + fg * 8);
+    }
+    uint2 vn0 = *(const uint2*)(vb + t_begin + fg * 4), vn1 = *(const uint2*)(vb + t_begin + 16 + fg * 4);
     for (int t0 = t_begin; t0 < t_end; t0 += 32) {
-        uint4 ka0 = make_uint4(0, 0, 0, 0), ka1 = ka0;
+        ka0 = kn0; ka1 = kn1;
+        const uint4 va = make_uint4(vn0.x, vn0.y, vn1.x, vn1.y);
+        const int tn = t0 + 32 < t_end ? t0 + 32 : t0;
         if (fg < 2) {
-            ka0 = *(const uint4*)(kb + (long)(t0 + fr) * 16 + fg * 8);
-            ka1 = *(const uint4*)(kb + (long)(t0 + 16 + fr) * 16 + fg * 8);
-        }
-        const uint2 v0 = *(const uint2*)(vb + t0 + fg * 4), v1 = *(const uint2*)(vb + t0 + 16 + fg * 4);
-        const uint4 va = make_uint4(v0.x, v0.y, v1.x, v1.y);
-#pragma unroll
-        for (int n = 0; n < 2; ++n) {
+            kn0 = *(const uint4*)(kb + (long)(tn + fr) * 16 + fg * 8);
+            kn1 = *(const uint4*)(kb + (long)(tn + 16 + fr) * 16 + fg * 8);
+        }
+        vn0 = *(const uint2*)(vb + tn + fg * 4); vn1 = *(const uint2*)(vb + tn + 16 + fg * 4);
+#pragma unroll
+        for (int n = 0; n < NT; ++n) {
             f32x4_t s0 = {0.f, 0.f, 0.f, 0.f}, s1 = s0;
             s0 = mfma16d(ka0, qf[n], s0);
             s1 = mfma16d(ka1, qf[n], s1);
@@ -407,7 +420,7 @@
         }
     }
 #pragma unroll
-    for (int n = 0; n < 2; ++n) {
+    for (int n = 0; n < NT; ++n) {
         float ln = l[n];
         ln += __shfl_xor(ln, 16); ln += __shfl_xor(ln, 32);
         if (fg == 0) { red[wave][n * 16 + fr][0] = m[n]; red[wave][n * 16 + fr][1] = ln; }
@@ -415,8 +428,8 @@
         for (int r = 0; r < 4; ++r) red[wave][n * 16 + fr][2 + fg * 4 + r] = o[n][r];
     }
     __syncthreads();
-    if (wave < 2) {
-        const int n = wave, c = n * 16 + fr, p = pg * 4 + n * 2 + (fr >> 3);
+    for (int n = wave; n < nt; n += 4) {
+        const int c = n * 16 + fr, p = pg * G + n * 2 + (fr >> 3);
         if (tk < Nt && p < P) {
             const float mm = fmaxf(fmaxf(red[0][c][0], red[1][c][0]), fmaxf(red[2][c][0], red[3][c][0]));
             float ll = 0.f, oo[4] = {0.f, 0.f, 0.f, 0.f};
@@ -574,7 +587,17 @@
 extern int g_tune_dec_chain, g_tune_dec_chain_min_p, g_tune_chain_variant, g_tune_chain_handover;
 int g_tune_tok_fuse = 0;
 int g_tune_mlp_split_fused = 1;
+int g_tune_t2i_shared_group = 4;
+int g_tune_prompt_prefix = 1;
 namespace {
+struct Prefix { float* qpe; float* queries; u16* q; };
+long prefix_bytes(int P, int Nt) { const long M = (long)P * Nt; return 2 * ((M * C * 4 + 255) & ~255L) + ((M * CI * 2 + 255) & ~255L); }
+Prefix carve_prefix(void* base, int P, int Nt) {
+    const long M = (long)P * Nt, f = (M * C * 4 + 255) & ~255L;
+    Prefix x; char* p = (char*)base;
+    x.qpe = (float*)p; x.queries = (float*)(p + f); x.q = (u16*)(p + 2 * f);
+    return x;
+}
 struct Work {
     float *qpe, *queries, *tmp; u16 *a, *b, *qs, *ks, *vs, *attn_tok, *mlp_h;
     u16 *keys, *kimg, *vT, *qimg, *attn_img, *up1; float* pre;
@@ -615,15 +638,15 @@
     return w;
 }
 
-int t2i_stream(const Ctx& cx, const Work& w, const Consts& c, int idx, const msam_attn_w_t& aw, int P, int Nt, bool blocked = false) {
+int t2i_stream(const Ctx& cx, const Work& w, const Consts& c, int idx, const msam_attn_w_t& aw, int P, int Nt, bool blocked, const u16* qs) {
     const long R = (long)P * T;
     if (Nt <= 8) {
         const int64_t avail = (int64_t)((char*)w.up1 - (char*)w.kimg);
-        return msam_t2i_fold_attention(w.keys, blocked ? 2 : 0, w.qs, P, Nt, aw.k_w, c.tab_k[idx], aw.v_w, aw.v_b, w.attn_tok, w.kimg,
+        return msam_t2i_fold_attention(w.keys, blocked ? 2 : 0, qs, P, Nt, aw.k_w, c.tab_k[idx], aw.v_w, aw.v_b, w.attn_tok, w.kimg,
                                        avail, cx.s);
     }
     if (int e = wsgemm_kv(cx, w.keys, c.wkv[idx], c.bkv[idx], c.pe_k[idx], (int)R, w.kimg, w.vT)) return e;
-    hipLaunchKernelGGL(t2i_attn_kernel, dim3(P * 8), dim3(256), 0, cx.s, w.qs, w.kimg, w.vT, 0, Nt, w.attn_tok);
+    hipLaunchKernelGGL(t2i_attn_kernel, dim3(P * 8), dim3(256), 0, cx.s, qs, w.kimg, w.vT, 0, Nt, w.attn_tok);
     return msam_check_launch("t2i_attn");
 }
 
@@ -648,7 +671,8 @@
                 const void* image_state, const float* points, const int32_t* labels, int32_t Np,
                 const float* boxes, const float* mask_input, const float* sparse, int32_t Ns, const float* dense,
                 const float* embedding, int32_t P, int32_t multimask,
-                float* low_res, float* iou, void* workspace, int64_t workspace_bytes, void* stream);
+                float* low_res, float* iou, void* workspace, int64_t workspace_bytes, void* stream,
+                const Prefix* pf_in = nullptr, const Prefix* pf_out = nullptr);
 }
 
 extern "C" int msam_decoder_forward_masks(const msam_decoder_t* dec, const msam_mask_prompt_t* mask_w, const void* consts,
@@ -657,6 +681,35 @@
                                           float* low_res, float* iou, void* workspace, int64_t workspace_bytes, void* stream) {
     return decoder_run(dec, mask_w, consts, image_state, points, labels, Np, boxes, mask_input, nullptr, 0, nullptr, nullptr, P,
                        multimask, low_res, iou, workspace, workspace_bytes, stream);
+}
+
+extern "C" int64_t msam_decoder_prompt_prefix_bytes(int32_t P, int32_t Nt) { return P > 0 && Nt > 0 ? prefix_bytes(P, Nt) : 0; }
+
+namespace {
+int prefix_tokens(const float* points, int32_t Np, const float* boxes) {
+    if (!points) Np = 0;
+    return 5 + Np + (boxes ? 2 : (Np > 0 ? 1 : 0));
+}
+}
+
+extern "C" int msam_decoder_prompt_prefix(const msam_decoder_t* dec, const float* points, const int32_t* labels, int32_t Np,
+                                          const float* boxes, int32_t P, void* prefix, void* workspace, int64_t workspace_bytes,
+                                          void* stream) {
+    if (!prefix || P <= 0) { msam_set_error("msam_decoder_prompt_prefix: null argument"); return 1; }
+    const Prefix pf = carve_prefix(prefix, P, prefix_tokens(points, Np, boxes));
+    return decoder_run(dec, nullptr, nullptr, nullptr, points, labels, Np, boxes, nullptr, nullptr, 0, nullptr, nullptr, P, 1, nullptr,
+                       nullptr, workspace, workspace_bytes, stream, nullptr, &pf);
+}
+
+extern "C" int msam_decoder_forward_masks_prefixed(const msam_decoder_t* dec, const msam_mask_prompt_t* mask_w, const void* consts,
+                                                   const void* image_state, const float* points, const int32_t* labels, int32_t Np,
+                                                   const float* boxes, const float* mask_input, const void* prefix, int32_t P,
+                                                   int32_t multimask, float* low_res, float* iou, void* workspace,
+                                                   int64_t workspace_bytes, void* stream) {
+    if (!prefix || P <= 0) { msam_set_error("msam_decoder_forward_masks_prefixed: null argument"); return 1; }
+    const Prefix pf = carve_prefix((void*)prefix, P, prefix_tokens(points, Np, boxes));
+    return decoder_run(dec, mask_w, consts, image_state, points, labels, Np, boxes, mask_input, nullptr, 0, nullptr, nullptr, P,
+                       multimask, low_res, iou, workspace, workspace_bytes, stream, &pf, nullptr);
 }
 
 extern "C" int msam_decoder_forward_embeddings(const msam_decoder_t* dec, const void* consts, const void* image_state,
@@ -696,8 +749,9 @@
                 const void* image_state, const float* points, const int32_t* labels, int32_t Np,
                 const float* boxes, const float* mask_input, const float* sparse, int32_t Ns, const float* dense,
                 const float* embedding, int32_t P, int32_t multimask,
-                float* low_res, float* iou, void* workspace, int64_t workspace_bytes, void* stream) {
-    if (!dec || !consts || !image_state || !low_res || !iou || !workspace || P <= 0) {
+                float* low_res, float* iou, void* workspace, int64_t workspace_bytes, void* stream,
+                const Prefix* pf_in, const Prefix* pf_out) {
+    if (!dec || !workspace || P <= 0 || (!pf_out && (!consts || !image_state || !low_res || !iou))) {
         msam_set_error("msam_decoder_forward: null argument");
         return 1;
     }
@@ -712,9 +766,16 @@
     if (Nt > 16) { msam_set_error("msam_decoder_forward: at most 16 tokens per prompt (<= 10 points)"); return 1; }
     if (workspace_bytes < work_bytes(P, Nt)) { msam_set_error("msam_decoder_forward: workspace too small"); return 1; }
     Ctx cx{(hipStream_t)stream, dec->use_glds};
-    Consts c = carve_consts((void*)consts);
-    ImageState im = carve_image((void*)image_state);
+    Consts c{}; ImageState im{};
+    if (consts) c = carve_consts((void*)consts);
+    if (image_state) im = carve_image((void*)image_state);
     Work w = carve_work(workspace, P, Nt);
+    const char* dbg = getenv("MSAM_DEBUG_DEC_LAYERS");
+    if (dbg) pf_in = nullptr;
+    if (pf_in) w.qpe = pf_in->qpe;
+    if (pf_out) w.qpe = pf_out->qpe;
+    float* const q_n1 = pf_out ? pf_out->queries : w.queries;
+    u16* const qs_0 = pf_out ? pf_out->q : w.qs;
     const int M = P * Nt;
     const long R = (long)P * T;
     const long n4 = (long)M * C / 4;
@@ -738,55 +799,65 @@
         hipLaunchKernelGGL(tokens_from_sparse_kernel, dim3(P), dim3(256), 0, cx.s, dec->out_tokens, sparse, Ns, P, Nt, w.qpe,
                            w.queries, w.a);
         CHECK(msam_check_launch("tokens_from_sparse"));
-    } else {
+    } else if (!pf_in) {
         hipLaunchKernelGGL(prompt_tokens_kernel, dim3(P), dim3(256), 0, cx.s, dec->pe_gauss, dec->point_embed, dec->not_a_point,
                            dec->out_tokens, points, labels, Np, boxes, P, Nt, w.qpe, w.queries, w.a);
         CHECK(msam_check_launch("prompt_tokens"));
     }
 
-    const char* dbg = getenv("MSAM_DEBUG_DEC_LAYERS");
     const int nlayers = dbg ? atoi(dbg) : 2;
     const bool chain = g_tune_dec_chain && !own_src && !dbg && Nt <= 8 && P >= g_tune_dec_chain_min_p;
     const bool fuse_tok = g_tune_tok_fuse != 0 && !dbg;
     void* const oper0 = w.qimg; void* const oper1 = w.attn_img;
     void* const tables = (char*)w.vT + (int64_t)R * CI * 2 - msam_chain_tables_bytes();
-    if (chain) CHECK(msam_chain_prepare_tables(im.src_bf16, im.q0, c.tab_k[1], c.tab_q[1], tables, cx.s));
+    if (chain && !pf_out) CHECK(msam_chain_prepare_tables(im.src_bf16, im.q0, c.tab_k[1], c.tab_q[1], tables, cx.s));
     const bool chain2 = chain && g_tune_chain_variant == 9;
     void* const tables2 = (char*)tables - msam_chain_tables2_bytes();
     void* const mfrag = (char*)oper0 + msam_i2t_fold_operand_bytes(P);
-    if (chain2) CHECK(msam_chain_prepare_tables2_c(im.src_bf16, c.chain2, tables2, cx.s));
+    if (chain2 && !pf_out) CHECK(msam_chain_prepare_tables2_c(im.src_bf16, c.chain2, tables2, cx.s));
     const bool handover = chain2 && g_tune_chain_handover != 0;
+    const bool merge = !dbg;
+    u16* const ks_1 = (u16*)w.tmp; u16* const vs_1 = ks_1 + (long)M * C;
     for (int li = 0; li < nlayers && li < 2; ++li) {
         const msam_twoway_layer_t& L = dec->layer[li];
-        const u16* sv = w.a;
-        if (li > 0) {
-            if (!fuse_tok) ADD_CAST2(w.queries, w.qpe, w.a, w.b);
-            sv = w.b;
-        }
-        {
+        const bool have_qkv = li > 0 && merge;
+        const bool have_prefix = li == 0 && pf_in != nullptr;
+        u16* const ks_s = have_qkv ? ks_1 : w.ks; u16* const vs_s = have_qkv ? vs_1 : w.vs;
+        if (!have_qkv && !have_prefix) {
+            const u16* sv = li > 0 ? w.b : w.a;
             const msam_gemm_t qkv[3] = {mk_gemm(w.a, C, L.self_attn.q_w, M, C, C, L.self_attn.q_b, w.qs, MSAM_D16, C),
                                         mk_gemm(w.a, C, L.self_attn.k_w, M, C, C, L.self_attn.k_b, w.ks, MSAM_D16, C),
                                         mk_gemm(sv, C, L.self_attn.v_w, M, C, C, L.self_attn.v_b, w.vs, MSAM_D16, C)};
             CHECK(msam_gemm_group_bf16(qkv, 3, cx.s));
         }
-        hipLaunchKernelGGL(token_self_attn_kernel, dim3(P), dim3(128), 0, cx.s, w.qs, w.ks, w.vs, Nt, w.attn_tok);
+        float* const n1_out = li == 0 ? q_n1 : w.queries;
+        const float* const n1_res = have_prefix ? pf_in->queries : n1_out;
+        const u16* const qs_l = have_prefix ? pf_in->q : (li == 0 ? qs_0 : w.qs);
+        if (!have_prefix) {
+        hipLaunchKernelGGL(token_self_attn_kernel, dim3(P), dim3(128), 0, cx.s, w.qs, ks_s, vs_s, Nt, w.attn_tok);
         CHECK(msam_check_launch("token_self_attn"));
         if (fuse_tok) {
             CHECK(gemm_ln_tok(cx, w.attn_tok, C, L.self_attn.o_w, M, C, L.self_attn.o_b, li == 0 ? nullptr : w.queries, L.n1_w, L.n1_b,
-                              w.queries, w.qpe, w.a, nullptr));
+                              n1_out, w.qpe, w.a, nullptr));
         } else {
         CHECK(gemm(cx, w.attn_tok, C, L.self_attn.o_w, M, C, C, L.self_attn.o_b, w.tmp, MSAM_F32, C, 0,
                    li == 0 ? nullptr : w.queries, li == 0 ? 0 : MSAM_F32, C));
-        LN(w.tmp, L.n1_w, L.n1_b, M, w.queries, MSAM_F32);
-        ADD_CAST(w.queries, w.qpe, w.a);
-        }
-        CHECK(gemm(cx, w.a, C, L.t2i.q_w, M, CI, C, L.t2i.q_b, w.qs, MSAM_D16, CI));
+        LN(w.tmp, L.n1_w, L.n1_b, M, n1_out, MSAM_F32);
+        ADD_CAST(n1_out, w.qpe, w.a);
+        }
+        CHECK(gemm(cx, w.a, C, L.t2i.q_w, M, CI, C, L.t2i.q_b, (u16*)qs_l, MSAM_D16, CI));
+        }
+        if (pf_out) return 0;
         if (li == 0 && !own_src) {
-            if (Nt <= 8)
-                hipLaunchKernelGGL(t2i_shared4_kernel, dim3(((P + 3) / 4) * 8), dim3(256), 0, cx.s, w.qs, im.k0, im.vT0, P, Nt,
-                                   w.attn_tok);
-            else
-                hipLaunchKernelGGL(t2i_attn_kernel, dim3(P * 8), dim3(256), 0, cx.s, w.qs, im.k0, im.vT0, 1, Nt, w.attn_tok);
+            if (Nt <= 8) {
+                const int G = g_tune_t2i_shared_group == 16 ? 16 : (g_tune_t2i_shared_group == 8 ? 8 : 4);
+                const dim3 grid(((P + G - 1) / G) * 8);
+                if (G == 4) hipLaunchKernelGGL(t2i_shared_kernel<4>, grid, dim3(256), 0, cx.s, qs_l, im.k0, im.vT0, P, Nt, w.attn_tok);
+                else if (G == 8) hipLaunchKernelGGL(t2i_shared_kernel<8>, grid, dim3(256), 0, cx.s, qs_l, im.k0, im.vT0, P, Nt, w.attn_tok);
+                else hipLaunchKernelGGL(t2i_shared_kernel<16>, grid, dim3(256), 0, cx.s, qs_l, im.k0, im.vT0, P, Nt, w.attn_tok);
+            } else {
+                hipLaunchKernelGGL(t2i_attn_kernel, dim3(P * 8), dim3(256), 0, cx.s, qs_l, im.k0, im.vT0, 1, Nt, w.attn_tok);
+            }
             CHECK(msam_check_launch("t2i_attn"));
         } else if (chain) {
             const msam_twoway_layer_t& L0 = dec->layer[0];
@@ -801,12 +872,12 @@
                 CHECK(msam_i2t0_t2i_fused(tables, oper0, L0.n4_w, L0.n4_b, 1e-5f, w.qs, P, Nt, L.t2i.k_w, L.t2i.v_w, L.t2i.v_b,
                                           w.attn_tok, w.vT, avail, cx.s));
         } else {
-            CHECK(t2i_stream(cx, w, c, li, L.t2i, P, Nt));
+            CHECK(t2i_stream(cx, w, c, li, L.t2i, P, Nt, false, qs_l));
         }
         if (fuse_tok) {
-            CHECK(gemm_ln_tok(cx, w.attn_tok, CI, L.t2i.o_w, M, CI, L.t2i.o_b, w.queries, L.n2_w, L.n2_b, w.queries, nullptr, w.a, nullptr));
+            CHECK(gemm_ln_tok(cx, w.attn_tok, CI, L.t2i.o_w, M, CI, L.t2i.o_b, n1_res, L.n2_w, L.n2_b, w.queries, nullptr, w.a, nullptr));
         } else {
-        CHECK(gemm(cx, w.attn_tok, CI, L.t2i.o_w, M, C, CI, L.t2i.o_b, w.tmp, MSAM_F32, C, 0, w.queries, MSAM_F32, C));
+        CHECK(gemm(cx, w.attn_tok, CI, L.t2i.o_w, M, C, CI, L.t2i.o_b, w.tmp, MSAM_F32, C, 0, n1_res, MSAM_F32, C));
         LN(w.tmp, L.n2_w, L.n2_b, M, w.queries, MSAM_F32);
         if (!(L.mlp1_ws != nullptr && L.mlp2_ws != nullptr)) ADD_CAST(w.queries, nullptr, w.a);
         }
@@ -837,9 +908,18 @@
         ADD_CAST2(w.queries, w.qpe, w.a, w.b);
         }
         {
-            const msam_gemm_t kv[2] = {mk_gemm(w.a, C, L.i2t.k_w, M, CI, C, L.i2t.k_b, w.ks, MSAM_D16, CI),
-                                       mk_gemm(w.b, C, L.i2t.v_w, M, CI, C, L.i2t.v_b, w.vs, MSAM_D16, CI)};
-            CHECK(msam_gemm_group_bf16(kv, 2, cx.s));
+            msam_gemm_t kv[5] = {mk_gemm(w.a, C, L.i2t.k_w, M, CI, C, L.i2t.k_b, w.ks, MSAM_D16, CI),
+                                 mk_gemm(w.b, C, L.i2t.v_w, M, CI, C, L.i2t.v_b, w.vs, MSAM_D16, CI)};
+            int nkv = 2;
+            if (merge && li == 0) {
+                const msam_attn_w_t& S = dec->layer[1].self_attn;
+                kv[nkv++] = mk_gemm(w.a, C, S.q_w, M, C, C, S.q_b, w.qs, MSAM_D16, C);
+                kv[nkv++] = mk_gemm(w.a, C, S.k_w, M, C, C, S.k_b, ks_1, MSAM_D16, C);
+                kv[nkv++] = mk_gemm(w.b, C, S.v_w, M, C, C, S.v_b, vs_1, MSAM_D16, C);
+            } else if (merge) {
+                kv[nkv++] = mk_gemm(w.a, C, dec->final_attn.q_w, M, CI, C, dec->final_attn.q_b, w.qs, MSAM_D16, CI);
+            }
+            CHECK(msam_gemm_group_bf16(kv, nkv, cx.s));
         }
         if (chain) {
             if (li == 0 && chain2)
@@ -868,9 +948,7 @@
         }
     }
     if (dbg) return 0;
-    if (!fuse_tok) ADD_CAST(w.queries, w.qpe, w.a);
-    CHECK(gemm(cx, w.a, C, dec->final_attn.q_w, M, CI, C, dec->final_attn.q_b, w.qs, MSAM_D16, CI));
-    CHECK(t2i_stream(cx, w, c, 2, dec->final_attn, P, Nt, chain));
+    CHECK(t2i_stream(cx, w, c, 2, dec->final_attn, P, Nt, chain, w.qs));
     if (fuse_tok) {
         CHECK(gemm_ln_tok(cx, w.attn_tok, CI, dec->final_attn.o_w, M, CI, dec->final_attn.o_b, w.queries, dec->nf_w, dec->nf_b, w.queries,
                           nullptr, w.a, nullptr));
diff --git a/micro_sam_amd/instance_segmentation.py b/micro_sam_amd/instance_segmentation.py
--- a/micro_sam_amd/instance_segmentation.py
+++ b/micro_sam_amd/instance_segmentation.py
@@ -7,7 +7,8 @@
 import numpy as np
 import torch
 
-from . import amg_utils, ops, util
+from . import _lib, amg_utils, ops, util
+from ._prompt_prefix import PromptPrefixCache
 from .predictor import SamPredictor
 
 
@@ -299,7 +300,7 @@
         import copy
         clone = copy.copy(self)
         clone._predictor = lane_predictor if lane_predictor is not None else SamPredictor(self._predictor.model.lane_view())
-        clone._prompt_cache = {}
+        clone._prompt_cache = PromptPrefixCache()
         clone._lanes = clone._post_stream = None
         clone.clear_state()
         return clone
@@ -336,22 +337,31 @@
         return lanes[:n]
 
     def _process_batch(self, points, im_size, crop_box, original_size):
-        key = (points.shape, tuple(im_size), float(points[0, 0]), float(points[-1, -1]))
-        cached = self._prompt_cache.get(key) if hasattr(self, "_prompt_cache") else None
-        if cached is None or cached[0].device != self._predictor.device or not np.array_equal(cached[2], points):
-            transformed_points = self._predictor.transform.apply_coords(points, im_size)
-            in_points = torch.as_tensor(transformed_points, device=self._predictor.device, dtype=torch.float)
+        predictor = self._predictor
+        model = predictor.model
+        with_prefix = not model.reference_formulation and _lib.tune_get("prompt_prefix") == 1
+        owner = model._prepare_decoder() if with_prefix else None
+        device = predictor.device
+
+        def make(pts_host):
+            transformed_points = predictor.transform.apply_coords(pts_host, im_size)
+            in_points = torch.as_tensor(transformed_points, device=device, dtype=torch.float)
             in_labels = torch.ones(in_points.shape[0], dtype=torch.int, device=in_points.device)
-            if not hasattr(self, "_prompt_cache"):
-                self._prompt_cache = {}
-            if len(self._prompt_cache) > 64:
-                self._prompt_cache.clear()
-            self._prompt_cache[key] = (in_points, in_labels, np.array(points, copy=True))
+            prefix = model.make_prompt_prefix(in_points[:, None, :], in_labels[:, None]) if with_prefix else None
+            return in_points, in_labels, prefix
+
+        if getattr(self, "_prompt_cache", None) is None:
+            self._prompt_cache = PromptPrefixCache()
+        key = (points.shape, tuple(im_size), float(points[0, 0]), float(points[-1, -1]), str(device), with_prefix)
+        in_points, in_labels, prefix = self._prompt_cache.get(key, points, owner, make)
+        if prefix is not None:
+            iou_preds, post = predictor.predict_masks_device(None, None, multimask_output=True,
+                                                             stability_score_offset=self._stability_score_offset,
+                                                             prompt_prefix=prefix)
         else:
-            in_points, in_labels = cached[0], cached[1]
-        iou_preds, post = self._predictor.predict_masks_device(
-            in_points[:, None, :], in_labels[:, None], multimask_output=True,
-            stability_score_offset=self._stability_score_offset)
+            iou_preds, post = predictor.predict_masks_device(
+                in_points[:, None, :], in_labels[:, None], multimask_output=True,
+                stability_score_offset=self._stability_score_offset)
         return self._to_mask_data_device(iou_preds, post, crop_box, original_size, points=points)
 
     def _process_crop(self, image, crop_box, crop_layer_idx, precomputed_embeddings, pbar_init=None, pbar_update=None):
diff --git a/micro_sam_amd/modeling.py b/micro_sam_amd/modeling.py
--- a/micro_sam_amd/modeling.py
+++ b/micro_sam_amd/modeling.py
@@ -691,10 +691,43 @@
         return low, iou
 
     @torch.no_grad()
+    def make_prompt_prefix(self, point_coords: Optional[torch.Tensor], point_labels: Optional[torch.Tensor],
+                           boxes: Optional[torch.Tensor] = None) -> "PromptPrefix":
+        if self.reference_formulation:
+            raise ValueError("micro_sam_amd: a prompt prefix belongs to the kernel path (precision 'default')")
+        if point_coords is None and boxes is None:
+            raise ValueError("micro_sam_amd: a prompt prefix needs points and / or boxes")
+        prepared = self._prepare_decoder()
+        p = prepared[0]
+        lib = _lib.load()
+        dev = self.device
+        pts = lbl = None
+        if point_coords is not None:
+            pts = point_coords.to(device=dev, dtype=torch.float32).contiguous()
+            lbl = point_labels.to(device=dev, dtype=torch.int32).contiguous()
+            P, Np = pts.shape[0], pts.shape[1]
+        else:
+            P, Np = boxes.reshape(-1, 4).shape[0], 0
+        bx = None if boxes is None else boxes.to(device=dev, dtype=torch.float32).reshape(-1, 4).contiguous()
+        Nt = 5 + Np + (2 if bx is not None else (1 if Np > 0 else 0))
+        block = torch.empty(lib.msam_decoder_prompt_prefix_bytes(P, Nt), dtype=torch.uint8, device=dev)
+        ws = self._workspace(P)
+        _lib.check(lib.msam_decoder_prompt_prefix(C.byref(p), _lib.ptr(pts), _lib.ptr(lbl), Np, _lib.ptr(bx), P, block.data_ptr(),
+                                                  ws.data_ptr(), ws.numel(), _lib.stream_ptr()), "msam_decoder_prompt_prefix")
+        return PromptPrefix(block, pts, lbl, bx, prepared)
+
+    @torch.no_grad()
     def decode(self, features: torch.Tensor, point_coords: Optional[torch.Tensor], point_labels: Optional[torch.Tensor],
                boxes: Optional[torch.Tensor] = None, mask_input: Optional[torch.Tensor] = None,
                multimask_output: bool = True, low_res_dtype: torch.dtype = torch.float32,
-               range_map: Union[bool, torch.Tensor] = False) -> Tuple[torch.Tensor, ...]:
+               range_map: Union[bool, torch.Tensor] = False,
+               prompt_prefix: Optional["PromptPrefix"] = None) -> Tuple[torch.Tensor, ...]:
+        if prompt_prefix is not None:
+            if self.reference_formulation:
+                raise ValueError("micro_sam_amd: a prompt prefix belongs to the kernel path (precision 'default')")
+            if point_coords is not None or point_labels is not None or boxes is not None:
+                raise ValueError("micro_sam_amd: with a prompt prefix the points, labels and boxes are the prefix's own")
+            point_coords, point_labels, boxes = prompt_prefix.points, prompt_prefix.labels, prompt_prefix.boxes
         want_range = range_map is not False and range_map is not None
         if want_range and (low_res_dtype != torch.float32 or self.reference_formulation or mask_input is not None):
             raise ValueError("range_map goes with float32 low-res logits of the kernel path, without a mask prompt")
@@ -712,6 +745,9 @@
             return (low if low_res_dtype == torch.float32 else low.to(low_res_dtype)), iou
         prepared = self._prepare_decoder()
         p, _, consts = prepared
+        if prompt_prefix is not None and (prompt_prefix.prepared is not prepared or prompt_prefix.block.device != self.device):
+            raise ValueError("micro_sam_amd: the prompt prefix was made for other decoder constants (new weights or settings) or "
+                             "another device; make it again")
         state = self._image_state(features, prepared)
         lib = _lib.load()
         dev = self.device
@@ -744,13 +780,26 @@
             msk = mask_input.to(device=dev, dtype=torch.float32).reshape(-1, 4 * GRID, 4 * GRID).contiguous()
             if msk.shape[0] != P:
                 raise ValueError(f"mask_input holds {msk.shape[0]} masks for {P} prompts")
-        _lib.check(lib.msam_decoder_forward_masks(
-            C.byref(p), C.byref(self._mask_params), consts.data_ptr(), state.data_ptr(), _lib.ptr(pts), _lib.ptr(lbl), Np,
-            _lib.ptr(bx), _lib.ptr(msk), P, 1 if multimask_output else 0, low.data_ptr(), iou.data_ptr(),
-            self._dec_ws.data_ptr(), self._dec_ws.numel(), _lib.stream_ptr()), "msam_decoder_forward")
+        if prompt_prefix is not None:
+            _lib.check(lib.msam_decoder_forward_masks_prefixed(
+                C.byref(p), C.byref(self._mask_params), consts.data_ptr(), state.data_ptr(), _lib.ptr(pts), _lib.ptr(lbl), Np,
+                _lib.ptr(bx), _lib.ptr(msk), prompt_prefix.block.data_ptr(), P, 1 if multimask_output else 0, low.data_ptr(),
+                iou.data_ptr(), self._dec_ws.data_ptr(), self._dec_ws.numel(), _lib.stream_ptr()), "msam_decoder_forward")
+        else:
+            _lib.check(lib.msam_decoder_forward_masks(
+                C.byref(p), C.byref(self._mask_params), consts.data_ptr(), state.data_ptr(), _lib.ptr(pts), _lib.ptr(lbl), Np,
+                _lib.ptr(bx), _lib.ptr(msk), P, 1 if multimask_output else 0, low.data_ptr(), iou.data_ptr(),
+                self._dec_ws.data_ptr(), self._dec_ws.numel(), _lib.stream_ptr()), "msam_decoder_forward")
         if want_range:
             return low, iou, rng
         return low, iou
+
+
+class PromptPrefix:
+    __slots__ = ("block", "points", "labels", "boxes", "prepared")
+
+    def __init__(self, block, points, labels, boxes, prepared):
+        self.block, self.points, self.labels, self.boxes, self.prepared = block, points, labels, boxes, prepared
 
 
 def build_sam(model_type: str = "vit_b", num_multimask_outputs: int = 3) -> Sam:
diff --git a/micro_sam_amd/predictor.py b/micro_sam_amd/predictor.py
--- a/micro_sam_amd/predictor.py
+++ b/micro_sam_amd/predictor.py
@@ -99,7 +99,7 @@
 
     @torch.no_grad()
     def predict_masks_device(self, point_coords, point_labels, boxes=None, multimask_output: bool = True,
-                             stability_score_offset: float = 1.0):
+                             stability_score_offset: float = 1.0, prompt_prefix=None):
         if not self.is_image_set:
             raise RuntimeError("An image must be set with .set_image(...) before mask prediction.")
         from . import _lib
@@ -108,7 +108,7 @@
                     and tuple(int(v) for v in self.input_size) == (1024, 1024)
                     and tuple(int(v) for v in self.original_size) == (1024, 1024) and _lib.tune_get("amg_range_map") == 1)
         out = self.model.decode(self.features, point_coords, point_labels, boxes, None, multimask_output, low_res_dtype=dt,
-                                range_map=with_map)
+                                range_map=with_map, prompt_prefix=prompt_prefix)
         low, iou = out[0], out[1]
         from .ops import postprocess_masks
         b, c = low.shape[:2]
```

Measured after the change: 188.0 tiles/s (median of 6 runs). 1.1% higher.
